# akashsengupta1997/STRAPS-3DHumanShapePose

Hardware: AMD Instinct MI355X
Metric: bodies/sec (higher is better)
Workload: dtype fp32 (encoder convolutions as exact bf16x3 operand splits (six bf16 products per term); in-step SMPL blend contraction and skinning as 3-product fp16 splits (fp16x3_lbs: 22-bit operands); fp32 accumulate throughout)

## Files before the change

include/straps_hip.h:

```cpp
#ifndef STRAPS_HIP_H
#define STRAPS_HIP_H

#include <stddef.h>
#include <stdint.h>

#ifdef __cplusplus
extern "C" {
#endif

#define STRAPS_ABI_VERSION 12

#define STRAPS_OK 0
#define STRAPS_EINVAL 1
#define STRAPS_EHIP 2
#define STRAPS_EUNSUPPORTED 3

int straps_abi_version(void);
int straps_selftest_mfma_peak(const float* seed512, float* out, int blocks, int iters, void* stream);
int straps_selftest_mfma_bf16(float* out, unsigned long long* clk2, int blocks, int iters, void* stream);
int straps_selftest_mfma_bf16_dense(float* out, unsigned long long* clk2, int blocks, int iters, int data, void* stream);
const char* straps_last_error(void);
int straps_device_count(void);
int straps_wall_clock_khz(void);
int straps_set_clock_accumulator(unsigned long long* acc2);


int straps_pack_conv_weight(const float* w_oihw, float* w_krsc, int cout, int cin, int kh, int kw,
                            void* stream);
int straps_pack_conv_weight_dgrad(const float* w_oihw, float* w_crsk, int cout, int cin, int kh,
                                  int kw, void* stream);
typedef struct {
    const float* src;
    float* dst_krsc;
    float* dst_crsk;
    int32_t o, c, r, s;
    long long first;
} straps_pack_desc_t;
int straps_pack_conv_weights_batched(const straps_pack_desc_t* descs, int n, long long total,
                                     void* stream);
int straps_pack_conv_weights_batched_x3(const straps_pack_desc_t* descs, int n, long long total,
                                        unsigned short* krsc_planes, unsigned short* crsk_planes,
                                        long long plane_stride, void* stream);

size_t straps_stem_weight_floats(int cin);
int straps_pack_stem_weight(const float* w_oihw, float* w_frag, int cin, void* stream);

int straps_bn_fold(const float* gamma, const float* beta, const float* mean, const float* var,
                   float eps, float* scale, float* shift, int c, void* stream);
int straps_bn_fold_stats(const float* gamma, const float* beta, const float* mean, const float* var,
                         float eps, float* scale, float* shift, float* save_mean, float* save_invstd,
                         int c, void* stream);

int straps_conv_trace_buffer(long long* trace);

int straps_stem_stat_blocks(int batch, int h, int w);
size_t straps_stem_nzmask_words(int batch, int cin, int h, int w);
int straps_stem_nzmask(const float* x_nchw, uint32_t* mask, int batch, int cin, int h, int w,
                       void* stream);
int straps_stem_fwd(const float* x_nchw, const float* w_frag, const float* scale,
                    const float* shift, int relu, float* y_nhwc, float* stats_partial,
                    const uint32_t* nzmask, int batch, int cin, int h, int w, void* stream);

int straps_conv_stat_blocks(int batch, int ho, int wo, int cout, int kdim , int tile_cfg);
int straps_conv_fwd(const float* x_nhwc, const float* w_krsc, const float* scale,
                    const float* shift, const float* residual, int relu, float* y_nhwc,
                    float* stats_partial, int batch, int h, int w, int cin, int cout, int kh,
                    int kw, int stride, int pad, int tile_cfg, void* stream);

int straps_maxpool_fwd(const float* x_nhwc, float* y_nhwc, int batch, int h, int w, int c,
                       void* stream);
int straps_gap_fwd(const float* x_nhwc, float* y, int batch, int hw, int c, void* stream);

int straps_bn_stats_finalize(const float* stats_partial, int nblocks, int c, long long count,
                             const float* gamma, const float* beta, float eps, float momentum,
                             float* running_mean, float* running_var, float* scale, float* shift,
                             float* save_mean, float* save_invstd, void* stream);
int straps_bn_apply(const float* x, const float* scale, const float* shift, const float* residual,
                    int relu, float* y, long long rows, int c, void* stream);

int straps_linear_fwd(const float* x, int ldx, const float* w, int ldw, const float* bias,
                      const float* addend, float* out, int ldo, int m, int n, int kdim, int relu,
                      void* stream);
int straps_broadcast_rows(const float* row, int cols, float* dst, int ld_dst, int m, void* stream);
int straps_ief_pack(const float* fc1_w, const float* fc3_w, float* w1f, float* w1e, float* w3, int f, int p,
                    int h1, int h2, int ld_e, void* stream);
#define STRAPS_GEMM_MULTI_MAX 8
typedef struct {
    const float* a; long long sam, sak;
    const float* b; long long sbk, sbn;
    float* c; int32_t ldc, accumulate;
    const float* addend; int32_t ldadd, reserved0;
    const float* mask; int32_t ldmask, reserved1;
    float* c2; int32_t ldc2, accumulate2;
    int32_t m, n, k, reserved2;
} straps_gemm_desc_t;
int straps_gemm_multi(const straps_gemm_desc_t* descs_host, int n, void* stream);

int straps_rot6d_fwd(const float* x6, long long ld, int per_row, float* rotmats, long long rows,
                     void* stream);
int straps_rodrigues_fwd(const float* aa, float* rotmats, long long n, void* stream);
int straps_rodrigues_bwd(const float* aa, const float* drotmats, float* daa, long long n, void* stream);
int straps_orthographic_project(const float* points, const float* cam, int ld_cam, float* out,
                                long long batch, int n, void* stream);
int straps_orthographic_project_bwd(const float* points, const float* cam, int ld_cam, const float* dout,
                                    float* dpoints, float* dcam, long long batch, int n, void* stream);
int straps_perspective_project(const float* points, const float* rotation, const float* translation,
                               const float* cam_k, int k_per_body, float* out, long long batch, int n,
                               void* stream);

#define STRAPS_SMPL_V 6890
#define STRAPS_SMPL_VPAD 6912
#define STRAPS_SMPL_TILES 216
#define STRAPS_SMPL_KP 224
#define STRAPS_SMPL_NJ 24
#define STRAPS_SMPL_NEXTRA 45
#define STRAPS_SMPL_NPICK 21
#define STRAPS_SMPL_NJOINTS_OUT 90

typedef struct {
    const float* blend_frag;
    const float* j_template;
    const float* j_shapedirs;
    const int32_t* parents;
    const int32_t* depth;
    int32_t max_depth;
    int32_t skin_k;
    const float* skin_w;
    const int32_t* skin_j;
    const int32_t* vj_ptr;
    int32_t n_tiles;
    int32_t reserved0;
    const int32_t* pick_ids;
    const float* blend_frag_t;
    const int32_t* children;
    const int32_t* jrt_ptr;
    const int32_t* jrt_code;
    const float* jrt_w;
    const int32_t* dj_ptr;
    const int32_t* dj_code;
    const float* dj_w;
    const void* blend_frag_h;
    float blend_h_unscale;
    int32_t reserved1;
    const void* skin_frag_p;
} straps_smpl_model_t;

#define STRAPS_SMPL_KERNEL_WIDE 0x100
#define STRAPS_SMPL_KERNEL_NARROW 0x200
#define STRAPS_SMPL_KERNEL_WIDE_BUILTIN 0x400
#define STRAPS_SMPL_EXACT_F32 0
#define STRAPS_SMPL_SPLIT_F16 1
#define STRAPS_SMPL_SPLIT_F16_LBS 2
#define STRAPS_SMPL_SPLIT_F16_LBS_PD16 3
#define STRAPS_SMPL_SPLIT_F16_LBS_P16 4

size_t straps_smpl_workspace_bytes(const straps_smpl_model_t* model, long long batch);
int straps_smpl_fwd(const straps_smpl_model_t* model, const float* betas, const float* rotmats,
                    float* verts, float* joints, void* workspace, long long batch, int chunks, int mode,
                    void* stream);

size_t straps_smpl_bwd_workspace_bytes(long long batch, int chunks);
int straps_smpl_bwd(const straps_smpl_model_t* model, const float* betas, const float* rotmats,
                    const float* dverts, const float* djoints, float* dbetas, float* drotmats,
                    void* workspace, long long batch, int chunks, void* stream);
int straps_smpl_bwd_aa(const straps_smpl_model_t* model, const float* betas, const float* rotmats,
                       const float* full_pose_aa, const float* dverts, const float* djoints, float* dbetas,
                       float* dfull_pose_aa, float* drotmats, void* workspace, long long batch, int chunks,
                       void* stream);

int straps_conv_dgrad(const float* dy_nhwc, const float* w_crsk, const float* addend,
                      float* dx_nhwc, int batch, int h, int w, int cin, int cout, int kh, int kw,
                      int stride, int pad, int tile_cfg, void* stream);

int straps_split3_bf16(const float* x, unsigned short* planes, long long n, long long plane_stride,
                       void* stream);
int straps_split3_bf16_cm(const float* x, unsigned short* planes, long long rows, int c,
                          long long plane_stride, void* stream);
int straps_conv_x3_stat_blocks(int batch, int h, int w, int cin, int cout, int kh, int kw, int stride,
                               int pad, int tile_cfg);

int straps_conv_x3f_supported(int cin, int cout, int kh, int kw, int stride, int pad);
int straps_conv_fwd_x3f(const float* x, const float* a_scale, const float* a_shift, int a_relu, const unsigned short* w3,
                        long long w_plane_stride, const float* scale, const float* shift, const float* residual, int relu,
                        float* y, float* stats_partial, int batch, int h, int w, int cin, int cout, int kh, int kw, int stride,
                        int pad, int tile_cfg, void* stream);
int straps_conv_x3f_stat_blocks(int batch, int h, int w, int cin, int cout, int kh, int kw, int stride, int pad, int tile_cfg);
int straps_conv_dgrad_x3f(const float* dy, const unsigned short* w3_crsk, long long w_plane_stride, const float* addend,
                          const unsigned* addend_bits, float* dx, int batch, int h, int w, int cin, int cout, int kh, int kw,
                          int stride, int pad, int tile_cfg, const float* bn_raw, const unsigned* bn_out_bits,
                          const float* bn_mask_scale, const float* bn_mask_shift, const float* bn_mean, const float* bn_invstd,
                          double* bn_partials, void* stream);
int straps_conv_dgrad_x3f_bn_blocks(int batch, int h, int w, int cin, int cout, int kh, int kw, int stride, int pad, int tile_cfg);
size_t straps_conv_wgrad_x3f_workspace_bytes(int batch, int h, int w, int cin, int cout, int kh, int kw, int stride, int pad);
int straps_conv_wgrad_x3f(const float* x, const float* a_scale, const float* a_shift, int a_relu, const float* dy, float* dw_oihw,
                          void* workspace, int batch, int h, int w, int cin, int cout, int kh, int kw, int stride, int pad,
                          int accumulate, void* stream);
int straps_conv_fwd_x3(const unsigned short* x3, long long x_plane_stride,
                       const unsigned short* w3_krsc, long long w_plane_stride, const float* scale,
                       const float* shift, const float* residual, int relu, float* y_nhwc,
                       float* stats_partial, int batch, int h, int w, int cin, int cout, int kh,
                       int kw, int stride, int pad, int tile_cfg, void* stream);
int straps_conv_fwd_x3p(const unsigned short* x3, long long x_plane_stride,
                        const unsigned short* w3_krsc, long long w_plane_stride, const float* scale,
                        const float* shift, const float* residual, int relu, float* y_nhwc,
                        unsigned short* y_planes, long long y_plane_stride, int batch, int h, int w,
                        int cin, int cout, int kh, int kw, int stride, int pad, int tile_cfg, void* stream);
int straps_split_bf16_cm(const float* x, unsigned short* plane, long long rows, int c, void* stream);
int straps_pack_conv_weight_bf16(const float* w_oihw, unsigned short* w_plane, int cout, int cin, int kh, int kw, void* stream);
int straps_conv_bf16_tile_choice(int batch, int h, int w, int cin, int cout, int kh, int kw, int stride, int pad);
int straps_conv_fwd_bf16(const unsigned short* x1, const unsigned short* w1_krsc, const float* scale, const float* shift,
                         const float* residual, int relu, float* y_nhwc, unsigned short* y_plane, int batch, int h, int w,
                         int cin, int cout, int kh, int kw, int stride, int pad, int tile_cfg, void* stream);
int straps_conv_dgrad_x3(const unsigned short* dy3, long long dy_plane_stride,
                         const unsigned short* w3_crsk, long long w_plane_stride,
                         const float* addend, float* dx_nhwc, int batch, int h, int w, int cin,
                         int cout, int kh, int kw, int stride, int pad, int tile_cfg, void* stream);
int straps_bn_apply_x3(const float* raw, const float* scale, const float* shift, const float* residual,
                       int relu, float* y, unsigned short* y_planes, long long plane_stride,
                       long long rows, int c, void* stream);
int straps_bn_relu_maxpool_fwd_x3(const float* raw, const float* scale, const float* shift,
                                  float* y_pool, uint8_t* idx, unsigned short* y_planes,
                                  long long plane_stride, int batch, int h, int w, int c, void* stream);
int straps_bn_bwd_x3(const float* dy, const float* yact, const float* raw, const float* save_mean,
                     const float* save_invstd, const float* gamma, const float* mask_scale,
                     const float* mask_shift, float* dgamma, float* dbeta, float* draw, float* dz_out,
                     unsigned short* draw_planes, long long plane_stride, void* workspace,
                     long long rows, int c, int accumulate, void* stream);
int straps_conv_dgrad_x3_bn_blocks(int batch, int h, int w, int cin, int cout, int kh, int kw, int stride,
                                   int pad, int tile_cfg);
int straps_conv_dgrad_x3_bn(const unsigned short* dy3, long long dy_plane_stride,
                            const unsigned short* w3_crsk, long long w_plane_stride, const float* addend,
                            float* dx_nhwc, int batch, int h, int w, int cin, int cout, int kh, int kw,
                            int stride, int pad, int tile_cfg, const float* bn_raw, const float* bn_out,
                            const float* bn_mask_scale, const float* bn_mask_shift, const float* bn_mean,
                            const float* bn_invstd, double* bn_partials, void* stream);
int straps_bn_bwd_finish_x3(const float* dy, const float* yact, const float* raw, const float* save_mean,
                            const float* save_invstd, const float* gamma, const float* mask_scale,
                            const float* mask_shift, float* dgamma, float* dbeta, float* draw, float* dz_out,
                            unsigned short* draw_planes, long long plane_stride, const double* partials,
                            int nblk, void* workspace, long long rows, int c, int accumulate, void* stream);
int straps_bn_apply_bits_x3(const float* raw, const float* scale, const float* shift, const float* residual, float* y,
                            unsigned short* y_planes, long long plane_stride, unsigned* relu_bits, long long rows,
                            int c, void* stream);
int straps_bn_bwd_bits_x3(const float* dy, const unsigned* relu_bits, const float* raw, const float* save_mean,
                          const float* save_invstd, const float* gamma, float* dgamma, float* dbeta, float* draw,
                          unsigned short* draw_planes, long long plane_stride, void* workspace, long long rows, int c,
                          int accumulate, void* stream);
int straps_bn_bwd_finish_bits_x3(const float* dy, const unsigned* relu_bits, const float* raw, const float* save_mean,
                                 const float* save_invstd, const float* gamma, float* dgamma, float* dbeta, float* draw,
                                 unsigned short* draw_planes, long long plane_stride, const double* partials, int nblk,
                                 void* workspace, long long rows, int c, int accumulate, void* stream);
int straps_conv_dgrad_x3_bits(const unsigned short* dy3, long long dy_plane_stride, const unsigned short* w3_crsk,
                              long long w_plane_stride, const float* addend, float* dx_nhwc, int batch, int h, int w,
                              int cin, int cout, int kh, int kw, int stride, int pad, int tile_cfg,
                              const unsigned* addend_bits, void* stream);
int straps_conv_dgrad_x3_bn_bits(const unsigned short* dy3, long long dy_plane_stride,
                                 const unsigned short* w3_crsk, long long w_plane_stride, const float* addend,
                                 float* dx_nhwc, int batch, int h, int w, int cin, int cout, int kh, int kw,
                                 int stride, int pad, int tile_cfg, const float* bn_raw, const float* bn_out,
                                 const float* bn_mask_scale, const float* bn_mask_shift, const float* bn_mean,
                                 const float* bn_invstd, double* bn_partials, const unsigned* addend_bits,
                                 const unsigned* bn_out_bits, void* stream);
int straps_conv_wgrad_x3_on_planes(int batch, int h, int w, int cin, int cout, int kh, int kw,
                                   int stride, int pad);
int straps_conv_wgrad_x3(const float* x_nhwc, const float* dy_nhwc, const unsigned short* x3,
                         long long x_plane_stride, const unsigned short* dy3, long long dy_plane_stride,
                         float* dw_oihw, void* workspace, int batch, int h, int w, int cin, int cout,
                         int kh, int kw, int stride, int pad, int accumulate, void* stream);


size_t straps_conv_wgrad_workspace_bytes(int batch, int h, int w, int cin, int cout, int kh,
                                         int kw, int stride, int pad);
int straps_conv_wgrad(const float* x_nhwc, const float* dy_nhwc, float* dw_oihw, void* workspace,
                      int batch, int h, int w, int cin, int cout, int kh, int kw, int stride,
                      int pad, int accumulate, void* stream);
size_t straps_stem_wgrad_workspace_bytes(int batch, int cin, int h, int w);
int straps_stem_wgrad(const float* x_nchw, const float* dy_nhwc, float* dw_oihw, void* workspace,
                      const uint32_t* nzmask , int batch, int cin,
                      int h, int w, int accumulate, void* stream);
#define STRAPS_STEM_DGRAD_MAX_CIN 64
size_t straps_stem_dgrad_weight_floats(int cin);
int straps_pack_stem_dgrad_weight(const float* w_oihw, float* w_pk, int cin, void* stream);
int straps_stem_dgrad(const float* dy_nhwc, const float* w_pk, float* dx_nchw, int batch, int cin, int h, int w,
                      int accumulate, void* stream);
int straps_bn_bwd_blocks(long long rows, int c);
size_t straps_bn_bwd_workspace_bytes(long long rows, int c);
int straps_bn_bwd(const float* dy, const float* yact, const float* raw, const float* save_mean,
                  const float* save_invstd, const float* gamma, const float* mask_scale,
                  const float* mask_shift, float* dgamma, float* dbeta, float* draw, float* dz_out,
                  void* workspace, long long rows, int c, int accumulate, void* stream);
int straps_bn_relu_maxpool_fwd(const float* raw_nhwc, const float* scale, const float* shift,
                               float* y_pool_nhwc, uint8_t* idx, int batch, int h, int w, int c,
                               void* stream);
int straps_bn_bwd_pooled(const float* dy_pool_nhwc, const uint8_t* idx, const float* raw,
                         const float* save_mean, const float* save_invstd, const float* gamma,
                         const float* mask_scale, const float* mask_shift, float* dgamma, float* dbeta,
                         float* draw, void* workspace, int batch, int h, int w, int c, int accumulate,
                         void* stream);
size_t straps_stem_tiles(int batch, int in_h, int in_w);
int straps_stem_tile_activity(const uint32_t* nzmask, uint8_t* tile_active, int batch, int cin, int in_h,
                              int in_w, void* stream);
int straps_bn_bwd_pooled_sparse(const float* dy_pool_nhwc, const uint8_t* idx, const float* raw,
                                const float* save_mean, const float* save_invstd, const float* gamma,
                                const float* mask_scale, const float* mask_shift, float* dgamma,
                                float* dbeta, float* draw, void* workspace, int batch, int h, int w, int c,
                                int accumulate, const uint8_t* tile_active, void* stream);
int straps_maxpool_fwd_idx(const float* x_nhwc, float* y_nhwc, uint8_t* idx, int batch, int h,
                           int w, int c, void* stream);
int straps_maxpool_bwd(const float* dy_nhwc, const uint8_t* idx, float* dx_nhwc, int batch, int h,
                       int w, int c, void* stream);
int straps_gap_bwd(const float* dfeat, float* dx_nhwc, int batch, int hw, int c, void* stream);
int straps_masked_copy(const float* x, int ldx, const float* mask, int ldmask, float* y, int ldy,
                       int m, int n, int accumulate, void* stream);
int straps_rot6d_bwd(const float* x6, long long ld, int per_row, const float* drot, float* dx6,
                     long long ldd, long long rows, void* stream);

int straps_build_proxy_input(const float* seg, const float* joints2d, float* out_nchw, int batch,
                             int nj, int wh, void* stream);
int straps_build_proxy_input_std(const float* seg, const float* joints2d, float* out_nchw, int batch,
                                 int nj, int wh, int std, void* stream);
int straps_build_proxy_input_nz(const float* seg, const float* joints2d, float* out_nchw, uint32_t* nzmask,
                                int batch, int nj, int wh, int std, void* stream);
size_t straps_loss_workspace_bytes(long long batch);
int straps_loss_fwd_bwd(const float* pred_verts, const float* pred_joints, const float* est,
                        int ld_est, const float* pred_rot, const float* tgt_verts,
                        const float* tgt_joints2d, const float* tgt_joints3d,
                        const float* tgt_shape, const float* tgt_rot, const float* log_vars,
                        float* loss_out, float* dverts, float* djoints, float* dest, float* drot,
                        float* dlogvar, void* workspace, long long batch, int img_wh, void* stream);
int straps_loss_fwd_bwd_gm(const float* pred_verts, const float* pred_joints, const float* est, int ld_est,
                           const float* pred_rot, const float* tgt_verts, const float* tgt_joints2d,
                           const float* tgt_joints3d, const float* tgt_shape, const float* tgt_rot,
                           const float* log_vars, float* loss_out, float* dverts, float* djoints, float* dest,
                           float* drot, float* dlogvar, void* workspace, long long batch, int img_wh,
                           const float* j2d_count_global, float count_scale, void* stream);
int straps_count_visible(const float* tgt_joints2d, float* out_count, long long batch, int nj, int img_wh,
                         void* stream);
int straps_mse_fwd(const float* pred, const float* tgt, const uint8_t* row_mask, long long rows,
                   int cols, float tgt_scale, float tgt_shift, float* out3, void* workspace,
                   void* stream);
int straps_mse_bwd(const float* pred, const float* tgt, const uint8_t* row_mask, long long rows,
                   int cols, float tgt_scale, float tgt_shift, const float* coef, float* grad,
                   void* stream);
int straps_augment_seg(const float* seg, const float* uniforms, const float* remove_prob,
                       float occlude_prob, int box_dim, float* out, int batch, int wh, void* stream);
int straps_philox_fill(unsigned long long seed, const long long* step_dev, long long step_host,
                       unsigned substream, float* out, long long n, int kind, void* stream);
int straps_counter_add(long long* counters, int n, long long delta, void* stream);
int straps_gather_f32(const float* src, const int* index, float* dst, int n, void* stream);
int straps_memset_zero(void* ptr, size_t bytes, void* stream);
int straps_augment_smpl(const float* pose_rows, long long n_rows, const float* u_index,
                        const float* orig_shape, const float* mean_shape, const float* shape_draws,
                        int shape_mode, const float* std_vector, double range_lo, double range_hi,
                        float* out_shape, float* out_rotmats, float* out_pose, long long batch,
                        void* stream);
int straps_augment_cam_t(const float* mean_cam_t, const float* normals_xy, const float* uniform_z,
                         double xy_std, double z_lo, double z_hi, float* out_cam_t, long long batch,
                         void* stream);
int straps_deviate_joints2d(const float* joints2d, const float* uniforms, double lo, double hi,
                            double hip_lo, double hip_hi, float* out, long long batch, void* stream);
int straps_deviate_verts2d(const float* verts, const float* uniforms, double lo, double hi, float* out,
                           long long nverts_total, void* stream);
int straps_project_targets(const float* joints, const float* cam_t, float fx, float fy, float cx,
                           float cy, float* joints2d, float* joints3d, long long batch, void* stream);
size_t straps_rasterize_workspace_bytes(long long batch, int nverts, int wh);
int straps_rasterize_parts(const float* verts, const int32_t* faces, const uint8_t* face_parts,
                           const float* cam_K, const float* cam_R, const float* cam_t, float* parts,
                           float* depth, void* workspace, long long batch, int nverts, int nfaces, int wh,
                           int cam_per_body, float near, float far, const float* vert_noise_u, double noise_lo,
                           double noise_hi, void* stream);
int straps_crop_resize(const float* seg, const float* joints2d, const float* uniforms,
                       double orig_scale_factor, double delta_scale_lo, double delta_scale_hi,
                       double delta_centre_lo, double delta_centre_hi, float* out_seg,
                       float* out_joints2d, int* boxes, int batch, int wh, int out_wh, int nj,
                       void* stream);
int straps_point_metrics(const float* pred, const float* target, float* out3, long long batch,
                         int npoints, void* stream);
int straps_adam_step(float* params, const float* grads, float* exp_avg, float* exp_avg_sq,
                     long long n, int step, float lr, float beta1, float beta2, float eps,
                     float grad_scale, const long long* step_dev, void* stream);

typedef struct {
    int layers;
    int in_channels;
    int ief_iters;
    int precision;
} straps_regressor_desc_t;
size_t straps_regressor_param_floats(const straps_regressor_desc_t* desc);
size_t straps_regressor_prepared_bytes(const straps_regressor_desc_t* desc);
int straps_regressor_prepare(const straps_regressor_desc_t* desc, const float* params, void* prepared, void* stream);
size_t straps_regressor_workspace_bytes(const straps_regressor_desc_t* desc, int batch, int h, int w);
int straps_regressor_fwd_infer(const straps_regressor_desc_t* desc, const void* prepared, const float* x, int batch, int h, int w,
                               float* est, int ld_est, float* rotmats, void* workspace, size_t workspace_bytes, void* stream);

size_t straps_regressor_train_param_floats(const straps_regressor_desc_t* desc);
size_t straps_regressor_bn_state_floats(const straps_regressor_desc_t* desc);
size_t straps_regressor_train_workspace_bytes(const straps_regressor_desc_t* desc, int batch, int h, int w);
int straps_regressor_fwd_train(const straps_regressor_desc_t* desc, const float* params, float* bn_state, const float* init_est,
                               const float* x, int batch, int h, int w, float* est, int ld_est,
                               void* workspace, size_t workspace_bytes, void* stream);
int straps_regressor_bwd(const straps_regressor_desc_t* desc, const float* params, const float* x, int batch, int h, int w,
                         const float* dest, int ld_dest, float* grads, float* dx,
                         void* workspace, size_t workspace_bytes, void* stream);
int straps_regressor_export_infer_params(const straps_regressor_desc_t* desc, const float* params, const float* bn_state,
                                         const float* init_est, float* infer_params, void* stream);

#define STRAPS_COMM_ID_BYTES 128
int straps_comm_unique_id(void* id128);
int straps_comm_init_rank(const void* id128, int nranks, int rank, void** comm);
int straps_comm_destroy(void* comm);
int straps_comm_size(void* comm);
const char* straps_comm_library(void);
int straps_allreduce_grads(float* flat_g, long long n, void* comm, void* stream);

#ifdef __cplusplus
}
#endif
#endif
```

straps-3dhumanshapepose_amd/csrc/common.h:

```cpp
#pragma once
#include <hip/hip_runtime.h>
#include <stdint.h>
#include <stdio.h>

#include "../../include/straps_hip.h"

typedef float f32x4 __attribute__((ext_vector_type(4)));
typedef float f32x16 __attribute__((ext_vector_type(16)));
typedef float f32x2 __attribute__((ext_vector_type(2)));

void straps_set_error(const char* fmt, ...);
unsigned long long* straps_clk_acc_current();

#define STRAPS_REQUIRE(cond, ...)             \
    do {                                      \
        if (!(cond)) {                        \
            straps_set_error(__VA_ARGS__);    \
            return STRAPS_EINVAL;             \
        }                                     \
    } while (0)

#define STRAPS_CHECK_LAUNCH(name)                                                        \
    do {                                                                                 \
        hipError_t e__ = hipGetLastError();                                              \
        if (e__ != hipSuccess) {                                                         \
            straps_set_error("%s: launch failed: %s", name, hipGetErrorString(e__));     \
            return STRAPS_EHIP;                                                          \
        }                                                                                \
    } while (0)

#if defined(__HIP_DEVICE_COMPILE__) && !(defined(STRAPS_TOOLS) && defined(STRAPS_ALLOW_PACKED_FP32))
#define STRAPS_NO_PACKED_FP32 __attribute__((target("no-packed-fp32-ops")))
#else
#define STRAPS_NO_PACKED_FP32
#endif

inline hipError_t straps_raise_dynamic_lds(const void* fn, size_t bytes, unsigned long long& done) {
    int dev = 0;
    hipError_t e = hipGetDevice(&dev);
    if (e != hipSuccess) return e;
    const unsigned long long bit = 1ull << (dev & 63);
    if (done & bit) return hipSuccess;
    e = hipFuncSetAttribute(fn, hipFuncAttributeMaxDynamicSharedMemorySize, (int)bytes);
    if (e == hipSuccess) done |= bit;
    return e;
}
#define STRAPS_RAISE_LDS(fn, bytes, name)                                                                  \
    do {                                                                                                   \
        static unsigned long long done__ = 0;                                                              \
        hipError_t e__ = straps_raise_dynamic_lds((const void*)(fn), (size_t)(bytes), done__);             \
        if (e__ != hipSuccess) {                                                                           \
            straps_set_error("%s: cannot raise dynamic LDS to %zu: %s", name, (size_t)(bytes), hipGetErrorString(e__)); \
            return STRAPS_EHIP;                                                                            \
        }                                                                                                  \
    } while (0)

__device__ __forceinline__ f32x16 mfma32(float a, float b, f32x16 c) {
    return __builtin_amdgcn_mfma_f32_32x32x2f32(a, b, c, 0, 0, 0);
}
__device__ __forceinline__ int mfma_row(int r, int lane) { return (r & 3) + 8 * (r >> 2) + 4 * (lane >> 5); }

__device__ __forceinline__ int xcd_remap(int bid, int nblk) {
    const int q = nblk >> 3, r = nblk & 7, xcd = bid & 7;
    return (xcd < r ? xcd * (q + 1) : r * (q + 1) + (xcd - r) * q) + (bid >> 3);
}

template <typename T>
__device__ __forceinline__ bool bn_partials_sum4(const T* __restrict__ part, int nblocks, int C, double& s1, double& s2, int& c) {
    __shared__ double red[256][2];
    const int cl = threadIdx.x & 3, pl = threadIdx.x >> 2;
    c = blockIdx.x * 4 + cl;
    double a1 = 0.0, a2 = 0.0;
    if (c < C) {
        int k = pl;
        for (; k + 15 * 64 < nblocks; k += 16 * 64) {
            T v0[16], v1[16];
#pragma unroll
            for (int q = 0; q < 16; ++q) {
                const T* v = part + ((long long)(k + q * 64) * C + c) * 2;
                v0[q] = v[0];
                v1[q] = v[1];
            }
#pragma unroll
            for (int q = 0; q < 16; ++q) { a1 += (double)v0[q]; a2 += (double)v1[q]; }
        }
#pragma unroll 8
        for (; k < nblocks; k += 64) {
            const T* v = part + ((long long)k * C + c) * 2;
            a1 += (double)v[0];
            a2 += (double)v[1];
        }
    }
    red[threadIdx.x][0] = a1;
    red[threadIdx.x][1] = a2;
    __syncthreads();
    if (pl != 0 || c >= C) return false;
    s1 = 0.0; s2 = 0.0;
    for (int q = 0; q < 64; ++q) { s1 += red[q * 4 + cl][0]; s2 += red[q * 4 + cl][1]; }
    return true;
}

typedef unsigned short u16;
typedef u16 u16x4 __attribute__((ext_vector_type(4)));
__device__ __forceinline__ u16 bf16_rn(float x) {
    unsigned u = __float_as_uint(x);
    u += 0x7FFFu + ((u >> 16) & 1u);
    return (u16)(u >> 16);
}
__device__ __forceinline__ void split3(float x, u16& b1, u16& b2, u16& b3) {
    b1 = bf16_rn(x);
    const float r1 = (__float_as_uint(x) & 0x7fffffffu) == 0x7f800000u ? 0.f : x - __uint_as_float((unsigned)b1 << 16);
    b2 = bf16_rn(r1);
    const float r2 = r1 - __uint_as_float((unsigned)b2 << 16);
    b3 = bf16_rn(r2);
}
__device__ __forceinline__ void store_planes4(u16* __restrict__ planes, long long ps, long long i, const f32x4& v) {
    u16x4 q1, q2, q3;
#pragma unroll
    for (int e = 0; e < 4; ++e) {
        u16 b1, b2, b3;
        split3(v[e], b1, b2, b3);
        q1[e] = b1; q2[e] = b2; q3[e] = b3;
    }
    *reinterpret_cast<u16x4*>(planes + i) = q1;
    *reinterpret_cast<u16x4*>(planes + ps + i) = q2;
    *reinterpret_cast<u16x4*>(planes + 2 * ps + i) = q3;
}

__device__ __forceinline__ long long cm_index(long long r, int c, long long rows) { return ((long long)(c >> 5) * rows + r) * 32 + (c & 31); }
__device__ __forceinline__ void store_planes4_cm(u16* __restrict__ planes, long long ps, long long r, int c, long long rows, const f32x4& v) {
    store_planes4(planes, ps, cm_index(r, c, rows), v);
}

#ifdef STRAPS_TOOLS
#include <stdlib.h>
#define STRAPS_TOOL_ENV_INT(name, dflt) (getenv(name) ? atoi(getenv(name)) : (dflt))
#else
#define STRAPS_TOOL_ENV_INT(name, dflt) (dflt)
#endif

static inline int cdiv(long long a, long long b) { return (int)((a + b - 1) / b); }

static inline unsigned straps_grid256(long long n) {
    const long long g = (n + 255) / 256;
    return (unsigned)(g > 256 * 16 ? 256 * 16 : (g < 1 ? 1 : g));
}
static inline unsigned straps_grid256_rows(long long n, int C4) {
    unsigned g = straps_grid256(n);
    if (C4 > 0 && (256 % C4) != 0) {
        long long a = C4, b = 256;
        while (b) { const long long t = a % b; a = b; b = t; }
        const long long m = C4 / a;
        if (m <= 256 * 16) { const long long up = ((g + m - 1) / m) * m; g = (unsigned)(up > 256 * 16 ? (256 * 16 / m) * m : up); }
    }
    return g;
}
static inline int straps_bn_tiled(long long rows, int C4) {
    static const int mode = STRAPS_TOOL_ENV_INT("STRAPS_BN_TILED", 1);
    if (!mode || (C4 & 15)) return 0;
    const int ncg = C4 >> 4;
    if (!(ncg == 1 || ncg == 2 || (ncg & 3) == 0) || (mode == 1 && ncg < 4)) return 0;
    const int wcg = ncg < 4 ? ncg : 4;
    return (rows % (16 / wcg)) == 0 ? wcg : 0;
}
static inline unsigned straps_bn_tiled_grid(long long rows, int C4, int wcg) {
    const long long ncb = (C4 >> 4) / wcg, tiles = rows / (16 / wcg) * ncb;
    long long g = tiles < 256 * 16 ? tiles : 256 * 16;
    g = g / ncb * ncb;
    return (unsigned)(g < ncb ? ncb : g);
}
```

straps-3dhumanshapepose_amd/csrc/smpl_bwd.hip:

```cpp
#include "common.h"
#include "rodrigues.h"

namespace {

constexpr int KP = STRAPS_SMPL_KP, KG = KP / 8, NT = STRAPS_SMPL_TILES, NV = STRAPS_SMPL_V, NROUNDS = NT / 4;
constexpr int BT = 32, AS = 292, SS = 193;
constexpr int NJS = STRAPS_SMPL_NPICK + STRAPS_SMPL_NEXTRA;

__global__ __launch_bounds__(256, 1) STRAPS_NO_PACKED_FP32 void smpl_verts_bwd_kernel(straps_smpl_model_t m, const float* __restrict__ F,
                                                                const float* __restrict__ Amat, const float* __restrict__ dverts,
                                                                const float* __restrict__ djoints, float* __restrict__ dFp,
                                                                float* __restrict__ dAp, long long B, int rounds_per_chunk) {
    extern __shared__ __attribute__((aligned(16))) float smem[];
    float* As_ = smem;
    float* stage = As_ + BT * AS;

    const int tid = threadIdx.x, lane = tid & 63, wave = tid >> 6;
    const int h = lane >> 5, bl = lane & 31;
    const int chunk = blockIdx.x;
    const long long b0 = (long long)blockIdx.y * BT;
    const int nb = (int)((B - b0) < BT ? (B - b0) : BT);

    for (int i = tid; i < BT * 72; i += 256) {
        const int b = i / 72, q = i % 72;
        f32x4 v = {0.f, 0.f, 0.f, 0.f};
        if (b < nb) v = *reinterpret_cast<const f32x4*>(Amat + (b0 + b) * 288 + q * 4);
        *reinterpret_cast<f32x4*>(As_ + b * AS + q * 4) = v;
    }
    __syncthreads();

    const int round0 = chunk * rounds_per_chunk;
    const int round1 = min(round0 + rounds_per_chunk, NROUNDS);
    const f32x4* __restrict__ blend = reinterpret_cast<const f32x4*>(m.blend_frag);
    const f32x4* __restrict__ blend_t = reinterpret_cast<const f32x4*>(m.blend_frag_t);
    float* mystage = stage + wave * BT * SS;
    const int KW = m.skin_k;
    const bool vbody = bl < nb;

    float dacc[3][12];
#pragma unroll
    for (int i = 0; i < 3; ++i)
#pragma unroll
        for (int e = 0; e < 12; ++e) dacc[i][e] = 0.f;
    f32x16 accF[7];
#pragma unroll
    for (int f = 0; f < 7; ++f)
#pragma unroll
        for (int q = 0; q < 16; ++q) accF[f][q] = 0.f;

    for (int rd = round0; rd < round1; ++rd) {
        const int tile = rd * 4 + wave;
        f32x16 ax, ay, az;
#pragma unroll
        for (int r = 0; r < 16; ++r) { ax[r] = 0.f; ay[r] = 0.f; az[r] = 0.f; }
        {
            const f32x4* px = blend + ((long long)(tile * 3 + 0) * KG) * 64 + lane;
            const f32x4* py = px + KG * 64;
            const f32x4* pz = py + KG * 64;
            const float* frow = F + (b0 + (vbody ? bl : 0)) * KP + 4 * h;
            f32x4 cx0 = px[0], cy0 = py[0], cz0 = pz[0];
            f32x4 fn = *reinterpret_cast<const f32x4*>(frow);
#pragma unroll 2
            for (int g = 0; g < KG; ++g) {
                f32x4 nx0 = cx0, ny0 = cy0, nz0 = cz0;
                const f32x4 f0 = vbody ? fn : f32x4{0.f, 0.f, 0.f, 0.f};
                if (g + 1 < KG) {
                    nx0 = px[(g + 1) * 64]; ny0 = py[(g + 1) * 64]; nz0 = pz[(g + 1) * 64];
                    fn = *reinterpret_cast<const f32x4*>(frow + 8 * (g + 1));
                }
#pragma unroll
                for (int e = 0; e < 4; ++e) {
                    ax = mfma32(cx0[e], f0[e], ax);
                    ay = mfma32(cy0[e], f0[e], ay);
                    az = mfma32(cz0[e], f0[e], az);
                }
                cx0 = nx0; cy0 = ny0; cz0 = nz0;
            }
        }
        {
            const int ncol = min(96, (NV - tile * 32) * 3);
            for (int i = lane; i < BT * 96; i += 64) {
                const int b = i / 96, c = i - b * 96;
                float v = 0.f;
                if (dverts && b < nb && c < ncol) v = dverts[(b0 + b) * (long long)(NV * 3) + tile * 96 + c];
                mystage[b * SS + (c / 3) * 6 + (c % 3)] = v;
            }
        }
        __syncthreads();
        if (djoints && h == 0 && vbody) {
            const float* dj = djoints + (b0 + bl) * (STRAPS_SMPL_NJOINTS_OUT * 3) + 72;
            const int e0 = m.jrt_ptr[tile], e1 = m.jrt_ptr[tile + 1];
            for (int e = e0; e < e1; ++e) {
                const int code = m.jrt_code[e];
                const float w = m.jrt_w[e];
                float* sv = mystage + bl * SS + (code >> 8) * 6;
                const float* g = dj + (code & 255) * 3;
                sv[0] = fmaf(w, g[0], sv[0]); sv[1] = fmaf(w, g[1], sv[1]); sv[2] = fmaf(w, g[2], sv[2]);
            }
        }
        __syncthreads();
        {
            const float* Ab = As_ + bl * AS;
#pragma unroll
            for (int r = 0; r < 16; ++r) {
                const int vrow = (r & 3) + 8 * (r >> 2) + 4 * h;
                const int v = tile * 32 + vrow;
                float* sv = mystage + bl * SS + vrow * 6;
                const float gx = sv[0], gy = sv[1], gz = sv[2];
                sv[3] = ax[r]; sv[4] = ay[r]; sv[5] = az[r];
                float t00 = 0.f, t01 = 0.f, t02 = 0.f, t10 = 0.f, t11 = 0.f, t12 = 0.f, t20 = 0.f, t21 = 0.f, t22 = 0.f;
                for (int k = 0; k < KW; ++k) {
                    const float w = m.skin_w[v * KW + k];
                    const int jo = m.skin_j[v * KW + k] * 12;
                    const f32x4 a0 = *reinterpret_cast<const f32x4*>(Ab + jo);
                    const f32x4 a1 = *reinterpret_cast<const f32x4*>(Ab + jo + 4);
                    const f32x4 a2 = *reinterpret_cast<const f32x4*>(Ab + jo + 8);
                    t00 += w * a0[0]; t01 += w * a0[1]; t02 += w * a0[2];
                    t10 += w * a1[0]; t11 += w * a1[1]; t12 += w * a1[2];
                    t20 += w * a2[0]; t21 += w * a2[1]; t22 += w * a2[2];
                }
                ax[r] = t00 * gx + t10 * gy + t20 * gz;
                ay[r] = t01 * gx + t11 * gy + t21 * gz;
                az[r] = t02 * gx + t12 * gy + t22 * gz;
            }
        }
        __syncthreads();
#pragma unroll
        for (int i = 0; i < 3; ++i) {
            const int j = wave + 4 * (2 * i + h);
            const int e0 = m.dj_ptr[rd * 24 + j], e1 = m.dj_ptr[rd * 24 + j + 1];
            for (int e = e0; e < e1; ++e) {
                const int code = m.dj_code[e];
                const float w = m.dj_w[e];
                const float* sv = stage + ((code >> 5) * BT + bl) * SS + (code & 31) * 6;
                const float wx = w * sv[0], wy = w * sv[1], wz = w * sv[2];
                const float x = sv[3], y = sv[4], z = sv[5];
                dacc[i][0] = fmaf(wx, x, dacc[i][0]); dacc[i][1] = fmaf(wx, y, dacc[i][1]); dacc[i][2] = fmaf(wx, z, dacc[i][2]); dacc[i][3] += wx;
                dacc[i][4] = fmaf(wy, x, dacc[i][4]); dacc[i][5] = fmaf(wy, y, dacc[i][5]); dacc[i][6] = fmaf(wy, z, dacc[i][6]); dacc[i][7] += wy;
                dacc[i][8] = fmaf(wz, x, dacc[i][8]); dacc[i][9] = fmaf(wz, y, dacc[i][9]); dacc[i][10] = fmaf(wz, z, dacc[i][10]); dacc[i][11] += wz;
            }
        }
        {
            const f32x4* pt = blend_t + ((long long)tile * 3 * 7 * 4) * 64 + lane;
#pragma unroll
            for (int c = 0; c < 3; ++c) {
#pragma unroll
                for (int f = 0; f < 7; ++f) {
#pragma unroll
                    for (int rq = 0; rq < 4; ++rq) {
                        const f32x4 a = pt[((c * 7 + f) * 4 + rq) * 64];
#pragma unroll
                        for (int e = 0; e < 4; ++e) {
                            const float g = c == 0 ? ax[rq * 4 + e] : (c == 1 ? ay[rq * 4 + e] : az[rq * 4 + e]);
                            accF[f] = mfma32(a[e], g, accF[f]);
                        }
                    }
                }
            }
        }
        __syncthreads();
    }
    {
        __syncthreads();
        float* red = smem;
        if (wave >= 2) {
#pragma unroll
            for (int f = 0; f < 7; ++f)
#pragma unroll
                for (int q = 0; q < 16; ++q) red[(wave - 2) * 7168 + (f * 16 + q) * 64 + lane] = accF[f][q];
        }
        __syncthreads();
        if (wave < 2) {
#pragma unroll
            for (int f = 0; f < 7; ++f)
#pragma unroll
                for (int q = 0; q < 16; ++q) accF[f][q] += red[wave * 7168 + (f * 16 + q) * 64 + lane];
        }
        __syncthreads();
        if (wave == 1) {
#pragma unroll
            for (int f = 0; f < 7; ++f)
#pragma unroll
                for (int q = 0; q < 16; ++q) red[(f * 16 + q) * 64 + lane] = accF[f][q];
        }
        __syncthreads();
        if (wave == 0) {
#pragma unroll
            for (int f = 0; f < 7; ++f)
#pragma unroll
                for (int q = 0; q < 16; ++q) accF[f][q] += red[(f * 16 + q) * 64 + lane];
        }
    }
    if (vbody && wave == 0) {
        float* o = dFp + ((long long)chunk * B + b0 + bl) * KP;
#pragma unroll
        for (int f = 0; f < 7; ++f)
#pragma unroll
            for (int q = 0; q < 16; ++q) o[f * 32 + mfma_row(q, lane)] = accF[f][q];
    }
    if (vbody) {
        float* o = dAp + ((long long)chunk * B + b0 + bl) * 288;
#pragma unroll
        for (int i = 0; i < 3; ++i) {
            const int j = wave + 4 * (2 * i + h);
#pragma unroll
            for (int e = 0; e < 12; ++e) o[j * 12 + e] = dacc[i][e];
        }
    }
}

__device__ __forceinline__ float lane_get(float value, int src) { return __shfl(value, src, 64); }
template <bool AA>
__global__ __launch_bounds__(256) STRAPS_NO_PACKED_FP32 void smpl_pose_bwd_kernel(straps_smpl_model_t m, const float* __restrict__ betas,
                                                            const float* __restrict__ rotmats, const float* __restrict__ dFp,
                                                            const float* __restrict__ dAp, const float* __restrict__ djoints,
                                                            float* __restrict__ dbetas, float* __restrict__ drot, long long B,
                                                            int chunks, const float* __restrict__ aa, float* __restrict__ daa) {
    const int lane = threadIdx.x & 63;
    const int j = lane & 31;
    const int base = lane & 32;
    const long long body = ((long long)blockIdx.x * 256 + threadIdx.x) >> 5;
    const bool vb = body < B;
    const bool vj = j < 24;
    const long long bb = vb ? body : 0;
    const int jj = vj ? j : 0;

    float beta[10];
#pragma unroll
    for (int l = 0; l < 10; ++l) beta[l] = betas[bb * 10 + l];
    float R[9];
#pragma unroll
    for (int e = 0; e < 9; ++e) R[e] = rotmats[(bb * 24 + jj) * 9 + e];
    float J[3];
#pragma unroll
    for (int c = 0; c < 3; ++c) {
        float s = m.j_template[jj * 3 + c];
#pragma unroll
        for (int l = 0; l < 10; ++l) s = fmaf(m.j_shapedirs[(jj * 3 + c) * 10 + l], beta[l], s);
        J[c] = s;
    }
    const int par = m.parents[jj];
    const int dep = vj ? m.depth[jj] : -1;
    const int src = base + (par < 0 ? 0 : par);
    float rel[3];
#pragma unroll
    for (int c = 0; c < 3; ++c) {
        const float jp = lane_get(J[c], src);
        rel[c] = (jj > 0) ? J[c] - jp : J[c];
    }
    float G[12], PR[9];
#pragma unroll
    for (int r = 0; r < 3; ++r) {
        G[r * 4 + 0] = R[r * 3 + 0]; G[r * 4 + 1] = R[r * 3 + 1]; G[r * 4 + 2] = R[r * 3 + 2]; G[r * 4 + 3] = rel[r];
    }
#pragma unroll
    for (int e = 0; e < 9; ++e) PR[e] = (e == 0 || e == 4 || e == 8) ? 1.f : 0.f;
    for (int d = 1; d <= m.max_depth; ++d) {
        float P[12];
#pragma unroll
        for (int e = 0; e < 12; ++e) P[e] = lane_get(G[e], src);
        if (dep == d) {
#pragma unroll
            for (int r = 0; r < 3; ++r) {
                const float p0 = P[r * 4 + 0], p1 = P[r * 4 + 1], p2 = P[r * 4 + 2];
                PR[r * 3 + 0] = p0; PR[r * 3 + 1] = p1; PR[r * 3 + 2] = p2;
                G[r * 4 + 0] = p0 * R[0] + p1 * R[3] + p2 * R[6];
                G[r * 4 + 1] = p0 * R[1] + p1 * R[4] + p2 * R[7];
                G[r * 4 + 2] = p0 * R[2] + p1 * R[5] + p2 * R[8];
                G[r * 4 + 3] = p0 * rel[0] + p1 * rel[1] + p2 * rel[2] + P[r * 4 + 3];
            }
        }
    }
    float gA[12];
#pragma unroll
    for (int e = 0; e < 12; ++e) gA[e] = 0.f;
    if (vb && vj)
        for (int c = 0; c < chunks; ++c) {
            const float* p = dAp + (((long long)c * B + body) * 24 + j) * 12;
#pragma unroll
            for (int e = 0; e < 12; ++e) gA[e] += p[e];
        }
    float gGR[9], gGt[3], gJ[3];
#pragma unroll
    for (int r = 0; r < 3; ++r) {
        const float gat = gA[r * 4 + 3];
        gGR[r * 3 + 0] = gA[r * 4 + 0] - gat * J[0];
        gGR[r * 3 + 1] = gA[r * 4 + 1] - gat * J[1];
        gGR[r * 3 + 2] = gA[r * 4 + 2] - gat * J[2];
        gGt[r] = gat + ((vb && vj && djoints) ? djoints[(body * STRAPS_SMPL_NJOINTS_OUT + j) * 3 + r] : 0.f);
    }
#pragma unroll
    for (int c = 0; c < 3; ++c) gJ[c] = -(G[0 * 4 + c] * gA[3] + G[1 * 4 + c] * gA[7] + G[2 * 4 + c] * gA[11]);

    int child[3];
#pragma unroll
    for (int c = 0; c < 3; ++c) child[c] = m.children[jj * 3 + c];
    float gR[9];
#pragma unroll
    for (int e = 0; e < 9; ++e) gR[e] = 0.f;
    for (int d = m.max_depth; d >= 1; --d) {
        float M[15];
        const bool mine = (dep == d);
        float grel[3];
#pragma unroll
        for (int c = 0; c < 3; ++c) grel[c] = PR[0 * 3 + c] * gGt[0] + PR[1 * 3 + c] * gGt[1] + PR[2 * 3 + c] * gGt[2];
#pragma unroll
        for (int r = 0; r < 3; ++r)
#pragma unroll
            for (int c = 0; c < 3; ++c)
                M[r * 3 + c] = mine ? (gGR[r * 3 + 0] * R[c * 3 + 0] + gGR[r * 3 + 1] * R[c * 3 + 1] + gGR[r * 3 + 2] * R[c * 3 + 2] + gGt[r] * rel[c]) : 0.f;
#pragma unroll
        for (int c = 0; c < 3; ++c) { M[9 + c] = mine ? gGt[c] : 0.f; M[12 + c] = mine ? -grel[c] : 0.f; }
        if (mine) {
#pragma unroll
            for (int r = 0; r < 3; ++r)
#pragma unroll
                for (int c = 0; c < 3; ++c)
                    gR[r * 3 + c] = PR[0 * 3 + r] * gGR[0 * 3 + c] + PR[1 * 3 + r] * gGR[1 * 3 + c] + PR[2 * 3 + r] * gGR[2 * 3 + c];
#pragma unroll
            for (int c = 0; c < 3; ++c) gJ[c] += grel[c];
        }
#pragma unroll
        for (int cc = 0; cc < 3; ++cc) {
            const int ch = child[cc];
            const int cs = base + (ch < 0 ? 0 : ch);
            float in[15];
#pragma unroll
            for (int e = 0; e < 15; ++e) in[e] = lane_get(M[e], cs);
            if (vj && ch >= 0) {
#pragma unroll
                for (int e = 0; e < 9; ++e) gGR[e] += in[e];
#pragma unroll
                for (int c = 0; c < 3; ++c) { gGt[c] += in[9 + c]; gJ[c] += in[12 + c]; }
            }
        }
    }
    if (j == 0) {
#pragma unroll
        for (int e = 0; e < 9; ++e) gR[e] = gGR[e];
#pragma unroll
        for (int c = 0; c < 3; ++c) gJ[c] += gGt[c];
    }
    float gbeta_direct = 0.f;
    if (vb && vj) {
        for (int c = 0; c < chunks; ++c) {
            const float* p = dFp + ((long long)c * B + body) * KP;
            if (j >= 1) {
#pragma unroll
                for (int e = 0; e < 9; ++e) gR[e] += p[11 + (j - 1) * 9 + e];
            }
            if (j < 10) gbeta_direct += p[1 + j];
        }
        if (!AA || drot) {
#pragma unroll
            for (int e = 0; e < 9; ++e) drot[(body * 24 + j) * 9 + e] = gR[e];
        }
        if constexpr (AA) {
            float ox, oy, oz;
            const float* r = aa + (body * 24 + j) * 3;
            straps_rodrigues_bwd_one(r[0], r[1], r[2], gR, ox, oy, oz);
            float* o = daa + (body * 24 + j) * 3;
            o[0] = ox; o[1] = oy; o[2] = oz;
        }
    }
#pragma unroll
    for (int l = 0; l < 10; ++l) {
        float s = vj ? (m.j_shapedirs[(jj * 3 + 0) * 10 + l] * gJ[0] + m.j_shapedirs[(jj * 3 + 1) * 10 + l] * gJ[1] +
                        m.j_shapedirs[(jj * 3 + 2) * 10 + l] * gJ[2]) : 0.f;
#pragma unroll
        for (int o = 16; o > 0; o >>= 1) s += __shfl_xor(s, o, 64);
        const float direct = lane_get(gbeta_direct, base + l);
        if (vb && j == l) dbetas[body * 10 + l] = s + direct;
    }
}

inline int resolve_rpc(long long batch, int chunks) {
    if (chunks <= 0) chunks = (batch >= 1024) ? 8 : 54;
    if (chunks > NROUNDS) chunks = NROUNDS;
    return (NROUNDS + chunks - 1) / chunks;
}

}

int straps_smpl_launch_pose(const straps_smpl_model_t* model, const float* betas, const float* rotmats, float* F, float* Amat,
                            float* joints, long long batch, hipStream_t st);

extern "C" size_t straps_smpl_bwd_workspace_bytes(long long batch, int chunks) {
    const int rpc = resolve_rpc(batch, chunks);
    const int nch = (NROUNDS + rpc - 1) / rpc;
    return (size_t)batch * (size_t)(KP + 288 + nch * (KP + 288)) * sizeof(float);
}

namespace {
template <bool AA>
int smpl_bwd_launch(const straps_smpl_model_t* model, const float* betas, const float* rotmats, const float* aa, const float* dverts,
                    const float* djoints, float* dbetas, float* drotmats, float* daa, void* workspace, long long batch, int chunks,
                    void* stream) {
    hipStream_t st = (hipStream_t)stream;
    const int rpc = resolve_rpc(batch, chunks);
    const int nch = (NROUNDS + rpc - 1) / rpc;
    float* F = (float*)workspace;
    float* Amat = F + batch * KP;
    float* dFp = Amat + batch * 288;
    float* dAp = dFp + (long long)nch * batch * KP;
    int rc = straps_smpl_launch_pose(model, betas, rotmats, F, Amat, nullptr, batch, st);
    if (rc != STRAPS_OK) return rc;
    const size_t lds = (size_t)(BT * AS + 4 * BT * SS) * sizeof(float);
    STRAPS_RAISE_LDS((smpl_verts_bwd_kernel), lds, "smpl_verts_bwd_kernel");
    const long long btiles = (batch + BT - 1) / BT;
    if (btiles > 65535) { straps_set_error("straps_smpl_bwd: batch %lld exceeds one launch; split it", batch); return STRAPS_EUNSUPPORTED; }
    hipLaunchKernelGGL(smpl_verts_bwd_kernel, dim3(nch, (unsigned)btiles), dim3(256), lds, st, *model, F, Amat, dverts, djoints, dFp, dAp, batch, rpc);
    STRAPS_CHECK_LAUNCH("smpl_verts_bwd_kernel");
    hipLaunchKernelGGL(smpl_pose_bwd_kernel<AA>, dim3((unsigned)((batch * 32 + 255) / 256)), dim3(256), 0, st, *model, betas, rotmats, dFp, dAp,
                       djoints, dbetas, drotmats, batch, nch, aa, daa);
    STRAPS_CHECK_LAUNCH("smpl_pose_bwd_kernel");
    return STRAPS_OK;
}
}

extern "C" int straps_smpl_bwd(const straps_smpl_model_t* model, const float* betas, const float* rotmats, const float* dverts,
                               const float* djoints, float* dbetas, float* drotmats, void* workspace, long long batch, int chunks,
                               void* stream) {
    STRAPS_REQUIRE(model && betas && rotmats && dbetas && drotmats && workspace, "straps_smpl_bwd: null pointer");
    STRAPS_REQUIRE(model->blend_frag_t && model->children && model->jrt_ptr && model->dj_ptr && model->dj_code && model->dj_w,
                   "straps_smpl_bwd: model lacks the backward tables");
    STRAPS_REQUIRE(batch > 0, "straps_smpl_bwd: batch must be positive");
    return smpl_bwd_launch<false>(model, betas, rotmats, nullptr, dverts, djoints, dbetas, drotmats, nullptr, workspace, batch, chunks, stream);
}

extern "C" int straps_smpl_bwd_aa(const straps_smpl_model_t* model, const float* betas, const float* rotmats, const float* full_pose_aa,
                                  const float* dverts, const float* djoints, float* dbetas, float* dfull_pose_aa, float* drotmats,
                                  void* workspace, long long batch, int chunks, void* stream) {
    STRAPS_REQUIRE(model && betas && rotmats && full_pose_aa && dbetas && dfull_pose_aa && workspace, "straps_smpl_bwd_aa: null pointer");
    STRAPS_REQUIRE(model->blend_frag_t && model->children && model->jrt_ptr && model->dj_ptr && model->dj_code && model->dj_w,
                   "straps_smpl_bwd_aa: model lacks the backward tables");
    STRAPS_REQUIRE(batch > 0, "straps_smpl_bwd_aa: batch must be positive");
    return smpl_bwd_launch<true>(model, betas, rotmats, full_pose_aa, dverts, djoints, dbetas, drotmats, dfull_pose_aa, workspace, batch, chunks,
                                 stream);
}
```

straps-3dhumanshapepose_amd/csrc/train.hip:

```cpp
#include <math.h>

#include "common.h"

namespace {

__constant__ int c_coco[17] = {24, 26, 25, 28, 27, 16, 17, 18, 19, 20, 21, 1, 2, 4, 5, 7, 8};
__constant__ int c_h36m14[14] = {73 + 6, 73 + 5, 73 + 4, 73 + 1, 73 + 2, 73 + 3, 73 + 16, 73 + 15, 73 + 14, 73 + 11, 73 + 12, 73 + 13, 73 + 8, 73 + 10};

__device__ __forceinline__ float heat_value(int x, int y, int jx, int jy, int WH, int size, float step, float two_var) {
    if (!(jx > -size && jy > -size && jx < WH - 1 + size && jy < WH - 1 + size)) return 0.f;
    const int hx0 = max(0, jx - size), hx1 = min(WH - 1, jx + size);
    const int hy0 = max(0, jy - size), hy1 = min(WH - 1, jy + size);
    if (!(x >= hx0 && x < hx1 && y >= hy0 && y < hy1)) return 0.f;
    const int gx = x - hx0 + max(0, size - jx), gy = y - hy0 + max(0, size - jy);
    const float fs = (float)size;
    const float lx = gx < size ? -fs + step * gx : fs - step * (2 * size - 1 - gx);
    const float ly = gy < size ? -fs + step * gy : fs - step * (2 * size - 1 - gy);
    const float d = sqrtf(lx * lx + ly * ly);
    return expf(-(d * d / two_var));
}

__global__ __launch_bounds__(256) void build_proxy_kernel(const float* __restrict__ seg, const float* __restrict__ j2d,
                                                          float* __restrict__ out, int B, int NJ, int WH, int size, float step, float two_var) {
    const int plane = blockIdx.y;
    const int b = plane / (NJ + 1), ch = plane - b * (NJ + 1);
    const int npix = WH * WH;
    float* o = out + (long long)plane * npix;
    int jx = 0, jy = 0;
    if (ch > 0) {
        jx = (int)j2d[((long long)b * NJ + ch - 1) * 2 + 0];
        jy = (int)j2d[((long long)b * NJ + ch - 1) * 2 + 1];
    }
    const float* s = seg + (long long)b * npix;
    const bool vec = (WH & 3) == 0;
    for (int p = (blockIdx.x * 256 + threadIdx.x) * 4; p < npix; p += gridDim.x * 1024) {
        float v[4];
#pragma unroll
        for (int e = 0; e < 4; ++e) {
            const int q = p + e;
            v[e] = 0.f;
            if (q < npix) {
                if (ch == 0) v[e] = s[q] != 0.f ? 1.f : 0.f;
                else {
                    const int y = q / WH, x = q - y * WH;
                    v[e] = heat_value(x, y, jx, jy, WH, size, step, two_var);
                }
            }
        }
        if (vec) *reinterpret_cast<f32x4*>(o + p) = f32x4{v[0], v[1], v[2], v[3]};
        else
            for (int e = 0; e < 4; ++e)
                if (p + e < npix) o[p + e] = v[e];
    }
}

__global__ __launch_bounds__(256) void build_proxy_nz_kernel(const float* __restrict__ seg, const float* __restrict__ j2d, float* __restrict__ out,
                                                             unsigned* __restrict__ mask, long long nwords, int NJ, int WH, int size, float step,
                                                             float two_var) {
    const int lane = threadIdx.x & 63;
    const long long word = (long long)blockIdx.x * 4 + (threadIdx.x >> 6);
    if (word >= nwords) return;
    const int HC = (WH + 3) >> 2, WW = (WH + 255) >> 8;
    const int ww = (int)(word % WW);
    const long long t = word / WW;
    const int hc = (int)(t % HC);
    const int plane = (int)(t / HC);
    const int b = plane / (NJ + 1), ch = plane - b * (NJ + 1);
    const int x0 = ww * 256 + (lane & 31) * 8 + (lane >> 5) * 4, y0 = hc * 4;
    const int npix = WH * WH;
    float* o = out + (long long)plane * npix;
    bool nz = false;
    if (x0 < WH) {
        f32x4 v[4];
#pragma unroll
        for (int r = 0; r < 4; ++r) v[r] = f32x4{0.f, 0.f, 0.f, 0.f};
        if (ch == 0) {
            const float* s = seg + (long long)b * npix;
#pragma unroll
            for (int r = 0; r < 4; ++r)
                if (y0 + r < WH) {
                    const f32x4 a = *reinterpret_cast<const f32x4*>(s + (y0 + r) * WH + x0);
#pragma unroll
                    for (int e = 0; e < 4; ++e) v[r][e] = a[e] != 0.f ? 1.f : 0.f;
                }
        } else {
            const int jx = (int)j2d[((long long)b * NJ + ch - 1) * 2 + 0];
            const int jy = (int)j2d[((long long)b * NJ + ch - 1) * 2 + 1];
            if (x0 + 3 >= jx - size && x0 < jx + size && y0 + 3 >= jy - size && y0 < jy + size) {
#pragma unroll
                for (int r = 0; r < 4; ++r)
                    if (y0 + r < WH)
#pragma unroll
                        for (int e = 0; e < 4; ++e) v[r][e] = heat_value(x0 + e, y0 + r, jx, jy, WH, size, step, two_var);
            }
        }
#pragma unroll
        for (int r = 0; r < 4; ++r)
            if (y0 + r < WH) {
                *reinterpret_cast<f32x4*>(o + (y0 + r) * WH + x0) = v[r];
                nz = nz || v[r][0] != 0.f || v[r][1] != 0.f || v[r][2] != 0.f || v[r][3] != 0.f;
            }
    }
    const unsigned long long m = __ballot(nz);
    if (lane == 0) mask[word] = (unsigned)(m | (m >> 32));
}

constexpr int NVB = 1024;

__global__ __launch_bounds__(256) void loss_verts_partial_kernel(const float* __restrict__ p, const float* __restrict__ t, long long n,
                                                                 float* __restrict__ part) {
    __shared__ float red[4];
    float s = 0.f;
    for (long long i = (long long)blockIdx.x * 256 + threadIdx.x; i < n; i += (long long)gridDim.x * 256) {
        const float d = p[i] - t[i];
        s = fmaf(d, d, s);
    }
#pragma unroll
    for (int o = 32; o > 0; o >>= 1) s += __shfl_xor(s, o, 64);
    if ((threadIdx.x & 63) == 0) red[threadIdx.x >> 6] = s;
    __syncthreads();
    if (threadIdx.x == 0) part[blockIdx.x] = (red[0] + red[1]) + (red[2] + red[3]);
}

__device__ __forceinline__ bool joint_visible(float x, float y, float wh) { return !(x > wh || y > wh || x < 0.f || y < 0.f); }

__global__ __launch_bounds__(256) void loss_heads_kernel(const float* __restrict__ joints, const float* __restrict__ est, int ld_est,
                                                         const float* __restrict__ prot, const float* __restrict__ tj2d,
                                                         const float* __restrict__ tj3d, const float* __restrict__ tshape,
                                                         const float* __restrict__ trot, float* __restrict__ body_sums, long long B,
                                                         float wh) {
    const long long b = (long long)blockIdx.x * 256 + threadIdx.x;
    if (b >= B) return;
    const float* J = joints + b * 270;
    const float* e = est + b * ld_est;
    const float s = e[0], tx = e[1], ty = e[2];
    float sq2 = 0.f, nvis = 0.f, sq3 = 0.f, sqs = 0.f, sqr = 0.f;
    for (int k = 0; k < 17; ++k) {
        const float lx = tj2d[(b * 17 + k) * 2 + 0], ly = tj2d[(b * 17 + k) * 2 + 1];
        if (joint_visible(lx, ly, wh)) {
            const float* pj = J + c_coco[k] * 3;
            const float u = s * (pj[0] + tx), v = s * (pj[1] + ty);
            const float du = u - ((2.0f * lx) / wh - 1.0f), dv = v - ((2.0f * ly) / wh - 1.0f);
            sq2 += du * du + dv * dv;
            nvis += 1.f;
        }
    }
    for (int k = 0; k < 14; ++k) {
        const float* pj = J + c_h36m14[k] * 3;
        const float* tj = tj3d + (b * 14 + k) * 3;
        for (int c = 0; c < 3; ++c) { const float d = pj[c] - tj[c]; sq3 += d * d; }
    }
    for (int l = 0; l < 10; ++l) { const float d = e[147 + l] - tshape[b * 10 + l]; sqs += d * d; }
    for (int q = 0; q < 216; ++q) { const float d = prot[b * 216 + q] - trot[b * 216 + q]; sqr += d * d; }
    float* o = body_sums + b * 8;
    o[0] = sq2; o[1] = nvis; o[2] = sq3; o[3] = sqs; o[4] = sqr;
}

__global__ __launch_bounds__(256) void loss_finalize_kernel(const float* __restrict__ vpart, const float* __restrict__ body_sums,
                                                            const float* __restrict__ log_vars, float* __restrict__ loss_out,
                                                            float* __restrict__ dlogvar, float* __restrict__ coef, long long B,
                                                            const float* __restrict__ j2d_count, float count_scale) {
    __shared__ double red[256][6];
    double a[6] = {0, 0, 0, 0, 0, 0};
    for (int i = threadIdx.x; i < NVB; i += 256) a[0] += (double)vpart[i];
    for (long long b = threadIdx.x; b < B; b += 256) {
        const float* o = body_sums + b * 8;
        a[1] += o[0]; a[2] += o[1]; a[3] += o[2]; a[4] += o[3]; a[5] += o[4];
    }
    for (int q = 0; q < 6; ++q) red[threadIdx.x][q] = a[q];
    __syncthreads();
    if (threadIdx.x == 0) {
        double t[6] = {0, 0, 0, 0, 0, 0};
        for (int i = 0; i < 256; ++i)
            for (int q = 0; q < 6; ++q) t[q] += red[i][q];
        const double nvis = t[2];
        const double n2 = j2d_count ? (double)j2d_count[0] * (double)count_scale : nvis;
        const double cnt[5] = {(double)B * 20670.0, n2 * 2.0, (double)B * 42.0, (double)B * 10.0, (double)B * 216.0};
        const double sq[5] = {t[0], t[1], t[3], t[4], t[5]};
        double total = 0.0;
        for (int k = 0; k < 5; ++k) {
            const double mse = sq[k] / cnt[k];
            const double s = (double)log_vars[k];
            const double w = exp(-s);
            loss_out[1 + k] = (float)(mse * w);
            loss_out[6 + k] = (float)mse;
            total += mse * w + s;
            dlogvar[k] = (float)(-mse * w + 1.0);
            coef[k] = (float)(2.0 * w / cnt[k]);
        }
        loss_out[0] = (float)total;
        loss_out[11] = (float)nvis;
    }
}

__global__ __launch_bounds__(256) void loss_grad_verts_kernel(const float* __restrict__ p, const float* __restrict__ t,
                                                              const float* __restrict__ coef, float* __restrict__ g, long long n) {
    const float c = coef[0];
    for (long long i = (long long)blockIdx.x * 256 + threadIdx.x; i < n; i += (long long)gridDim.x * 256) g[i] = c * (p[i] - t[i]);
}

__global__ __launch_bounds__(64) STRAPS_NO_PACKED_FP32 void loss_grad_heads_kernel(const float* __restrict__ joints, const float* __restrict__ est, int ld_est,
                                                             const float* __restrict__ prot, const float* __restrict__ tj2d,
                                                             const float* __restrict__ tj3d, const float* __restrict__ tshape,
                                                             const float* __restrict__ trot, const float* __restrict__ coef,
                                                             float* __restrict__ djoints, float* __restrict__ dest,
                                                             float* __restrict__ drot, long long B, float wh) {
    const long long b = blockIdx.x;
    const int lane = threadIdx.x;
    const float* J = joints + b * 270;
    const float* e = est + b * ld_est;
    float* dJ = djoints + b * 270;
    float* dE = dest + b * ld_est;
    const float c2 = coef[1], c3 = coef[2], cs = coef[3], cr = coef[4];
    for (int i = lane; i < 270; i += 64) dJ[i] = 0.f;
    for (int i = lane; i < ld_est; i += 64) dE[i] = (i >= 147 && i < 157) ? cs * (e[i] - tshape[b * 10 + i - 147]) : 0.f;
    for (int i = lane; i < 216; i += 64) drot[b * 216 + i] = cr * (prot[b * 216 + i] - trot[b * 216 + i]);
    __builtin_amdgcn_s_waitcnt(0);
    __syncthreads();
    const float s = e[0], tx = e[1], ty = e[2];
    float gs = 0.f, gtx = 0.f, gty = 0.f;
    if (lane < 17) {
        const float lx = tj2d[(b * 17 + lane) * 2 + 0], ly = tj2d[(b * 17 + lane) * 2 + 1];
        if (joint_visible(lx, ly, wh)) {
            const float* pj = J + c_coco[lane] * 3;
            const float u = s * (pj[0] + tx), v = s * (pj[1] + ty);
            const float du = c2 * (u - ((2.0f * lx) / wh - 1.0f)), dv = c2 * (v - ((2.0f * ly) / wh - 1.0f));
            dJ[c_coco[lane] * 3 + 0] = du * s;
            dJ[c_coco[lane] * 3 + 1] = dv * s;
            gs = du * (pj[0] + tx) + dv * (pj[1] + ty);
            gtx = du * s;
            gty = dv * s;
        }
    } else if (lane >= 32 && lane < 46) {
        const int k = lane - 32;
        const float* pj = J + c_h36m14[k] * 3;
        const float* tj = tj3d + (b * 14 + k) * 3;
        for (int c = 0; c < 3; ++c) dJ[c_h36m14[k] * 3 + c] = c3 * (pj[c] - tj[c]);
    }
#pragma unroll
    for (int o = 16; o > 0; o >>= 1) {
        gs += __shfl_xor(gs, o, 64);
        gtx += __shfl_xor(gtx, o, 64);
        gty += __shfl_xor(gty, o, 64);
    }
    if (lane == 0) { dE[0] = gs; dE[1] = gtx; dE[2] = gty; }
}

__global__ __launch_bounds__(256) void adam_kernel(float* __restrict__ p, const float* __restrict__ g, float* __restrict__ m,
                                                   float* __restrict__ v, long long n, float b1, float b2, float eps, float step_size,
                                                   float inv_sqrt_bc2, float gscale, float lr, const long long* __restrict__ step_dev) {
    if (step_dev) {
        const double t = (double)step_dev[0];
        step_size = (float)((double)lr / (1.0 - pow((double)b1, t)));
        inv_sqrt_bc2 = (float)(1.0 / sqrt(1.0 - pow((double)b2, t)));
    }
    for (long long i = (long long)blockIdx.x * 256 + threadIdx.x; i < n; i += (long long)gridDim.x * 256) {
        const float gi = g[i] * gscale;
        const float mi = b1 * m[i] + (1.f - b1) * gi;
        const float vi = b2 * v[i] + (1.f - b2) * gi * gi;
        m[i] = mi;
        v[i] = vi;
        p[i] -= step_size * mi / (sqrtf(vi) * inv_sqrt_bc2 + eps);
    }
}

inline unsigned capped_grid(long long n, int cap = 4096) {
    long long g = (n + 255) / 256;
    return (unsigned)(g > cap ? cap : (g < 1 ? 1 : g));
}

}

extern "C" int straps_build_proxy_input_std(const float* seg, const float* joints2d, float* out_nchw, int batch, int nj, int wh, int std,
                                            void* stream) {
    STRAPS_REQUIRE(seg && joints2d && out_nchw && batch > 0 && nj > 0 && wh > 16, "straps_build_proxy_input: bad arguments");
    STRAPS_REQUIRE(std >= 1 && 4 * std <= wh, "straps_build_proxy_input: std must be an integer in [1, wh / 4] (got %d)", std);
    STRAPS_REQUIRE((long long)batch * (nj + 1) <= 65535 && wh <= 16384, "straps_build_proxy_input: batch*(nj+1) must be <= 65535 per call");
    const int gx = (wh * wh / 4 + 255) / 256;
    const int size = 2 * std;
    const float step = (float)(2 * size) / (float)(2 * size - 1);
    const float two_var = (float)(2.0 * std * std);
    hipLaunchKernelGGL(build_proxy_kernel, dim3(gx < 64 ? gx : 64, batch * (nj + 1)), dim3(256), 0, (hipStream_t)stream, seg, joints2d, out_nchw, batch, nj, wh,
                       size, step, two_var);
    STRAPS_CHECK_LAUNCH("build_proxy_kernel");
    return STRAPS_OK;
}

extern "C" int straps_build_proxy_input_nz(const float* seg, const float* joints2d, float* out_nchw, uint32_t* nzmask, int batch, int nj, int wh,
                                           int std, void* stream) {
    STRAPS_REQUIRE(seg && joints2d && out_nchw && nzmask && batch > 0 && nj > 0 && wh > 16, "straps_build_proxy_input_nz: bad arguments");
    STRAPS_REQUIRE(std >= 1 && 4 * std <= wh, "straps_build_proxy_input_nz: std must be an integer in [1, wh / 4] (got %d)", std);
    STRAPS_REQUIRE((wh & 7) == 0 && wh <= 16384, "straps_build_proxy_input_nz: wh must be a multiple of 8 (got %d)", wh);
    const long long nwords = (long long)batch * (nj + 1) * ((wh + 3) / 4) * ((wh + 255) / 256);
    STRAPS_REQUIRE((nwords + 3) / 4 < (1LL << 31) && (long long)batch * (nj + 1) * wh * wh < (1LL << 40), "straps_build_proxy_input_nz: input too large for one launch");
    const int size = 2 * std;
    const float step = (float)(2 * size) / (float)(2 * size - 1);
    const float two_var = (float)(2.0 * std * std);
    hipLaunchKernelGGL(build_proxy_nz_kernel, dim3((unsigned)((nwords + 3) / 4)), dim3(256), 0, (hipStream_t)stream, seg, joints2d, out_nchw, nzmask, nwords, nj,
                       wh, size, step, two_var);
    STRAPS_CHECK_LAUNCH("build_proxy_nz_kernel");
    return STRAPS_OK;
}

extern "C" int straps_build_proxy_input(const float* seg, const float* joints2d, float* out_nchw, int batch, int nj, int wh,
                                        void* stream) {
    return straps_build_proxy_input_std(seg, joints2d, out_nchw, batch, nj, wh, 4, stream);
}

extern "C" size_t straps_loss_workspace_bytes(long long batch) { return (size_t)(NVB + batch * 8 + 16) * sizeof(float); }

__global__ __launch_bounds__(256) void count_visible_kernel(const float* __restrict__ tj2d, float* __restrict__ out, long long n, float wh) {
    __shared__ int red[4];
    int c = 0;
    for (long long i = threadIdx.x; i < n; i += 256) c += joint_visible(tj2d[i * 2], tj2d[i * 2 + 1], wh) ? 1 : 0;
#pragma unroll
    for (int o = 32; o > 0; o >>= 1) c += __shfl_xor(c, o, 64);
    if ((threadIdx.x & 63) == 0) red[threadIdx.x >> 6] = c;
    __syncthreads();
    if (threadIdx.x == 0) out[0] = (float)(red[0] + red[1] + red[2] + red[3]);
}

extern "C" int straps_count_visible(const float* tgt_joints2d, float* out_count, long long batch, int nj, int img_wh, void* stream) {
    STRAPS_REQUIRE(tgt_joints2d && out_count && batch > 0 && nj > 0, "straps_count_visible: bad arguments");
    hipLaunchKernelGGL(count_visible_kernel, dim3(1), dim3(256), 0, (hipStream_t)stream, tgt_joints2d, out_count, batch * nj, (float)img_wh);
    STRAPS_CHECK_LAUNCH("count_visible_kernel");
    return STRAPS_OK;
}

extern "C" int straps_loss_fwd_bwd(const float* pred_verts, const float* pred_joints, const float* est, int ld_est, const float* pred_rot,
                                   const float* tgt_verts, const float* tgt_joints2d, const float* tgt_joints3d, const float* tgt_shape,
                                   const float* tgt_rot, const float* log_vars, float* loss_out, float* dverts, float* djoints,
                                   float* dest, float* drot, float* dlogvar, void* workspace, long long batch, int img_wh, void* stream) {
    return straps_loss_fwd_bwd_gm(pred_verts, pred_joints, est, ld_est, pred_rot, tgt_verts, tgt_joints2d, tgt_joints3d, tgt_shape, tgt_rot, log_vars, loss_out,
                                  dverts, djoints, dest, drot, dlogvar, workspace, batch, img_wh, nullptr, 1.0f, stream);
}

extern "C" int straps_loss_fwd_bwd_gm(const float* pred_verts, const float* pred_joints, const float* est, int ld_est, const float* pred_rot,
                                      const float* tgt_verts, const float* tgt_joints2d, const float* tgt_joints3d, const float* tgt_shape,
                                      const float* tgt_rot, const float* log_vars, float* loss_out, float* dverts, float* djoints,
                                      float* dest, float* drot, float* dlogvar, void* workspace, long long batch, int img_wh,
                                      const float* j2d_count_global, float count_scale, void* stream) {
    STRAPS_REQUIRE(pred_verts && pred_joints && est && pred_rot && tgt_verts && tgt_joints2d && tgt_joints3d && tgt_shape && tgt_rot &&
                       log_vars && loss_out && workspace,
                   "straps_loss_fwd_bwd: null pointer");
    STRAPS_REQUIRE(batch > 0 && ld_est >= 157, "straps_loss_fwd_bwd: bad shape batch=%lld ld_est=%d", batch, ld_est);
    const bool want_grad = dverts || djoints || dest || drot || dlogvar;
    STRAPS_REQUIRE(!want_grad || (dverts && djoints && dest && drot && dlogvar), "straps_loss_fwd_bwd: give all gradient outputs or none");
    hipStream_t st = (hipStream_t)stream;
    float* vpart = (float*)workspace;
    float* body = vpart + NVB;
    float* coef = body + batch * 8;
    float* dlv = dlogvar ? dlogvar : coef + 8;
    const long long nv = batch * 20670LL;
    hipLaunchKernelGGL(loss_verts_partial_kernel, dim3(NVB), dim3(256), 0, st, pred_verts, tgt_verts, nv, vpart);
    STRAPS_CHECK_LAUNCH("loss_verts_partial_kernel");
    hipLaunchKernelGGL(loss_heads_kernel, dim3((unsigned)((batch + 255) / 256)), dim3(256), 0, st, pred_joints, est, ld_est, pred_rot,
                       tgt_joints2d, tgt_joints3d, tgt_shape, tgt_rot, body, batch, (float)img_wh);
    STRAPS_CHECK_LAUNCH("loss_heads_kernel");
    hipLaunchKernelGGL(loss_finalize_kernel, dim3(1), dim3(256), 0, st, vpart, body, log_vars, loss_out, dlv, coef, batch, j2d_count_global, count_scale);
    STRAPS_CHECK_LAUNCH("loss_finalize_kernel");
    if (want_grad) {
        hipLaunchKernelGGL(loss_grad_verts_kernel, dim3(capped_grid(nv)), dim3(256), 0, st, pred_verts, tgt_verts, coef, dverts, nv);
        STRAPS_CHECK_LAUNCH("loss_grad_verts_kernel");
        hipLaunchKernelGGL(loss_grad_heads_kernel, dim3((unsigned)batch), dim3(64), 0, st, pred_joints, est, ld_est, pred_rot, tgt_joints2d,
                           tgt_joints3d, tgt_shape, tgt_rot, coef, djoints, dest, drot, batch, (float)img_wh);
        STRAPS_CHECK_LAUNCH("loss_grad_heads_kernel");
    }
    return STRAPS_OK;
}

extern "C" int straps_adam_step(float* params, const float* grads, float* exp_avg, float* exp_avg_sq, long long n, int step, float lr,
                                float beta1, float beta2, float eps, float grad_scale, const long long* step_dev, void* stream) {
    STRAPS_REQUIRE(params && grads && exp_avg && exp_avg_sq && n > 0 && (step >= 1 || step_dev), "straps_adam_step: bad arguments");
    if (step < 1) step = 1;
    const double bc1 = 1.0 - pow((double)beta1, (double)step);
    const double bc2 = 1.0 - pow((double)beta2, (double)step);
    hipLaunchKernelGGL(adam_kernel, dim3(capped_grid(n)), dim3(256), 0, (hipStream_t)stream, params, grads, exp_avg, exp_avg_sq, n, beta1, beta2,
                       eps, (float)((double)lr / bc1), (float)(1.0 / sqrt(bc2)), grad_scale, lr, step_dev);
    STRAPS_CHECK_LAUNCH("adam_kernel");
    return STRAPS_OK;
}

namespace {

__global__ __launch_bounds__(256) void mse_sum_kernel(const float* __restrict__ p, const float* __restrict__ t, const uint8_t* __restrict__ mask,
                                                      long long rows, int cols, float ts, float tb, float* __restrict__ part) {
    __shared__ float red[4][2];
    float s = 0.f, c = 0.f;
    const long long n = rows * cols;
    for (long long i = (long long)blockIdx.x * 256 + threadIdx.x; i < n; i += (long long)gridDim.x * 256) {
        if (mask && !mask[i / cols]) continue;
        const float d = p[i] - (t[i] * ts + tb);
        s = fmaf(d, d, s);
        c += 1.f;
    }
#pragma unroll
    for (int o = 32; o > 0; o >>= 1) { s += __shfl_xor(s, o, 64); c += __shfl_xor(c, o, 64); }
    if ((threadIdx.x & 63) == 0) { red[threadIdx.x >> 6][0] = s; red[threadIdx.x >> 6][1] = c; }
    __syncthreads();
    if (threadIdx.x == 0) {
        part[blockIdx.x * 2 + 0] = (red[0][0] + red[1][0]) + (red[2][0] + red[3][0]);
        part[blockIdx.x * 2 + 1] = (red[0][1] + red[1][1]) + (red[2][1] + red[3][1]);
    }
}

__global__ __launch_bounds__(64) void mse_finalize_kernel(const float* __restrict__ part, int nblk, float* __restrict__ out) {
    double s = 0.0, c = 0.0;
    for (int i = threadIdx.x; i < nblk; i += 64) { s += part[i * 2]; c += part[i * 2 + 1]; }
#pragma unroll
    for (int o = 32; o > 0; o >>= 1) { s += __shfl_xor(s, o, 64); c += __shfl_xor(c, o, 64); }
    if (threadIdx.x == 0) { out[0] = (float)s; out[1] = (float)c; out[2] = (float)(s / c); }
}

__global__ __launch_bounds__(256) void mse_grad_kernel(const float* __restrict__ p, const float* __restrict__ t, const uint8_t* __restrict__ mask,
                                                       long long rows, int cols, float ts, float tb, const float* __restrict__ coef,
                                                       float* __restrict__ g) {
    const long long n = rows * cols;
    const float c = coef[0];
    for (long long i = (long long)blockIdx.x * 256 + threadIdx.x; i < n; i += (long long)gridDim.x * 256)
        g[i] = (mask && !mask[i / cols]) ? 0.f : c * (p[i] - (t[i] * ts + tb));
}

}

extern "C" int straps_mse_fwd(const float* pred, const float* tgt, const uint8_t* row_mask, long long rows, int cols, float tgt_scale,
                              float tgt_shift, float* out3, void* workspace, void* stream) {
    STRAPS_REQUIRE(pred && tgt && out3 && workspace && rows > 0 && cols > 0, "straps_mse_fwd: bad arguments");
    float* part = (float*)workspace;
    hipLaunchKernelGGL(mse_sum_kernel, dim3(256), dim3(256), 0, (hipStream_t)stream, pred, tgt, row_mask, rows, cols, tgt_scale, tgt_shift, part);
    STRAPS_CHECK_LAUNCH("mse_sum_kernel");
    hipLaunchKernelGGL(mse_finalize_kernel, dim3(1), dim3(64), 0, (hipStream_t)stream, part, 256, out3);
    STRAPS_CHECK_LAUNCH("mse_finalize_kernel");
    return STRAPS_OK;
}

extern "C" int straps_mse_bwd(const float* pred, const float* tgt, const uint8_t* row_mask, long long rows, int cols, float tgt_scale,
                              float tgt_shift, const float* coef, float* grad, void* stream) {
    STRAPS_REQUIRE(pred && tgt && coef && grad && rows > 0 && cols > 0, "straps_mse_bwd: bad arguments");
    hipLaunchKernelGGL(mse_grad_kernel, dim3(capped_grid(rows * cols)), dim3(256), 0, (hipStream_t)stream, pred, tgt, row_mask, rows, cols,
                       tgt_scale, tgt_shift, coef, grad);
    STRAPS_CHECK_LAUNCH("mse_grad_kernel");
    return STRAPS_OK;
}

namespace {
__global__ __launch_bounds__(256) void project_targets_kernel(const float* __restrict__ joints, const float* __restrict__ cam_t, float fx,
                                                              float fy, float cx, float cy, float* __restrict__ j2d,
                                                              float* __restrict__ j3d, long long B) {
    const long long i = (long long)blockIdx.x * 256 + threadIdx.x;
    if (i >= B * 31) return;
    const long long b = i / 31;
    const int k = (int)(i - b * 31);
    const float* J = joints + b * 270;
    if (k < 17) {
        const float* p = J + c_coco[k] * 3;
        const float x = p[0] + cam_t[b * 3 + 0], y = p[1] + cam_t[b * 3 + 1], z = p[2] + cam_t[b * 3 + 2];
        j2d[(b * 17 + k) * 2 + 0] = fx * (x / z) + cx;
        j2d[(b * 17 + k) * 2 + 1] = fy * (y / z) + cy;
    } else {
        const float* p = J + c_h36m14[k - 17] * 3;
        float* o = j3d + (b * 14 + (k - 17)) * 3;
        o[0] = p[0]; o[1] = p[1]; o[2] = p[2];
    }
}
}

extern "C" int straps_project_targets(const float* joints, const float* cam_t, float fx, float fy, float cx, float cy, float* joints2d,
                                      float* joints3d, long long batch, void* stream) {
    STRAPS_REQUIRE(joints && cam_t && joints2d && joints3d && batch > 0, "straps_project_targets: bad arguments");
    hipLaunchKernelGGL(project_targets_kernel, dim3((unsigned)((batch * 31 + 255) / 256)), dim3(256), 0, (hipStream_t)stream, joints, cam_t, fx,
                       fy, cx, cy, joints2d, joints3d, batch);
    STRAPS_CHECK_LAUNCH("project_targets_kernel");
    return STRAPS_OK;
}
```

straps-3dhumanshapepose_amd/hipabi.py:

```python
import ctypes as C
import os
import subprocess

_HERE = os.path.dirname(os.path.abspath(__file__))
CSRC = os.path.join(_HERE, 'csrc')
LIB_PATH = os.path.join(CSRC, 'libstraps_hip.so')
HEADER = os.path.join(os.path.dirname(_HERE), 'include', 'straps_hip.h')
SOURCES = ['abi.hip', 'augment.hip', 'pose.hip', 'ief.hip', 'elementwise.hip', 'conv.hip', 'conv_x3.hip', 'conv_x3_lean.hip', 'conv_bf16.hip', 'conv_x3f.hip', 'conv_wgrad_x3f.hip', 'stem.hip', 'stem_dgrad.hip', 'smpl.hip',
           'smpl_bwd.hip', 'backward.hip', 'train.hip', 'metrics.hip', 'image.hip', 'raster.hip', 'exchange.hip',
           'regressor.hip', 'regressor_train.hip']

_lib = None
LINK_LIBS = ['-ldl']
EXTRA_FLAGS = {'smpl.hip': ['-fno-slp-vectorize']}


def _existing_sources():
    return [os.path.join(CSRC, s) for s in SOURCES if os.path.isfile(os.path.join(CSRC, s))]


TOOLS_LIB_PATH = os.path.join(os.path.dirname(_HERE), 'tools', 'bin', 'libstraps_hip_tools.so')


def build(force=False, verbose=False, tools=False):
    srcs = _existing_sources()
    lib_path = TOOLS_LIB_PATH if tools else LIB_PATH
    if tools and not force and os.environ.get('STRAPS_TOOLS_NO_BUILD') == '1' and os.path.isfile(lib_path):
        import sys
        import time
        print('hipabi.build(tools=True): STRAPS_TOOLS_NO_BUILD=1 -- reusing %s (built %s)' % (lib_path, time.strftime('%Y-%m-%d %H:%M:%S', time.localtime(os.path.getmtime(lib_path)))),
              file=sys.stderr)
        return lib_path
    import glob
    hdrs = sorted(glob.glob(os.path.join(CSRC, '*.h'))) + [HEADER]
    deps = srcs + hdrs
    if not force and os.path.isfile(lib_path) and all(os.path.getmtime(lib_path) > os.path.getmtime(d) for d in deps):
        if not tools:
            _audit(lib_path, 'hipabi.build (library up to date)')
        return lib_path
    hipcc = os.environ.get('HIPCC', '/opt/rocm/bin/hipcc')
    flags = ['--offload-arch=gfx950', '-O3', '-std=c++17', '-fPIC'] + (['-DSTRAPS_TOOLS'] if tools else [])
    extra = dict(EXTRA_FLAGS)
    if tools and os.environ.get('STRAPS_TOOLS_SMPL_FLAGS'):
        extra['smpl.hip'] = extra.get('smpl.hip', []) + os.environ['STRAPS_TOOLS_SMPL_FLAGS'].split()
    if tools and os.environ.get('STRAPS_TOOLS_SMPL_BWD_FLAGS'):
        extra['smpl_bwd.hip'] = extra.get('smpl_bwd.hip', []) + os.environ['STRAPS_TOOLS_SMPL_BWD_FLAGS'].split()
    if tools and os.environ.get('STRAPS_TOOLS_RASTER_FLAGS'):
        extra['raster.hip'] = extra.get('raster.hip', []) + os.environ['STRAPS_TOOLS_RASTER_FLAGS'].split()
    objdir = os.path.join(os.path.dirname(TOOLS_LIB_PATH), 'build') if tools else os.path.join(CSRC, 'build')
    os.makedirs(objdir, exist_ok=True)
    jobs = []
    for s in srcs:
        o = os.path.join(objdir, os.path.basename(s)[:-4] + '.o')
        if force or not os.path.isfile(o) or any(os.path.getmtime(o) <= os.path.getmtime(d) for d in [s] + hdrs):
            cmd = [hipcc] + flags + extra.get(os.path.basename(s), []) + ['-c', s, '-o', o]
            if verbose:
                print(' '.join(cmd))
            jobs.append((cmd, subprocess.Popen(cmd, cwd=CSRC)))
    for cmd, p in jobs:
        if p.wait() != 0:
            raise subprocess.CalledProcessError(p.returncode, cmd)
    objs = [os.path.join(objdir, os.path.basename(s)[:-4] + '.o') for s in srcs]
    cmd = [hipcc, '--offload-arch=gfx950', '-fPIC', '-shared', '-o', lib_path] + objs + LINK_LIBS
    if verbose:
        print(' '.join(cmd))
    subprocess.run(cmd, check=True, cwd=CSRC)
    if not tools:
        _audit(lib_path, 'hipabi.build', fresh=True)
    return lib_path


def _audit(lib_path, what, fresh=False):
    from . import isa_audit
    if not fresh and isa_audit.stamp_ok(lib_path):
        return
    if not isa_audit.enforce(lib_path, what):
        import warnings
        warnings.warn('%s: llvm-objdump not found under %s -- the packed-operand-select audit of %s (DESIGN section 1: wrong results in lanes 48..63 on '
                      'MI355X) did NOT run; set STRAPS_LLVM_BIN or audit the library where it was built (tools/audit_packed_fp32.py)'
                      % (what, isa_audit.LLVM_BIN, lib_path), RuntimeWarning, stacklevel=3)


class SmplModelStruct(C.Structure):
    _fields_ = [('blend_frag', C.c_void_p), ('j_template', C.c_void_p), ('j_shapedirs', C.c_void_p),
                ('parents', C.c_void_p), ('depth', C.c_void_p), ('max_depth', C.c_int32), ('skin_k', C.c_int32),
                ('skin_w', C.c_void_p), ('skin_j', C.c_void_p), ('vj_ptr', C.c_void_p), ('n_tiles', C.c_int32),
                ('reserved0', C.c_int32), ('pick_ids', C.c_void_p), ('blend_frag_t', C.c_void_p), ('children', C.c_void_p),
                ('jrt_ptr', C.c_void_p), ('jrt_code', C.c_void_p), ('jrt_w', C.c_void_p), ('dj_ptr', C.c_void_p), ('dj_code', C.c_void_p),
                ('dj_w', C.c_void_p), ('blend_frag_h', C.c_void_p), ('blend_h_unscale', C.c_float), ('reserved1', C.c_int32), ('skin_frag_p', C.c_void_p)]


class PackDesc(C.Structure):
    _fields_ = [('src', C.c_void_p), ('dst_krsc', C.c_void_p), ('dst_crsk', C.c_void_p), ('o', C.c_int32), ('c', C.c_int32),
                ('r', C.c_int32), ('s', C.c_int32), ('first', C.c_longlong)]


class GemmDesc(C.Structure):
    _fields_ = [('a', C.c_void_p), ('sam', C.c_longlong), ('sak', C.c_longlong), ('b', C.c_void_p), ('sbk', C.c_longlong), ('sbn', C.c_longlong),
                ('c', C.c_void_p), ('ldc', C.c_int32), ('accumulate', C.c_int32), ('addend', C.c_void_p), ('ldadd', C.c_int32), ('reserved0', C.c_int32),
                ('mask', C.c_void_p), ('ldmask', C.c_int32), ('reserved1', C.c_int32), ('c2', C.c_void_p), ('ldc2', C.c_int32), ('accumulate2', C.c_int32),
                ('m', C.c_int32), ('n', C.c_int32), ('k', C.c_int32), ('reserved2', C.c_int32)]


def gemm_desc(a, sam, sak, b, sbk, sbn, c, ldc, m, n, k, accumulate=0, addend=None, ldadd=0, mask=None, ldmask=0, c2=None, ldc2=0, accumulate2=0):
    adr = lambda t: None if t is None else (t if isinstance(t, int) else t.data_ptr())
    return GemmDesc(adr(a), sam, sak, adr(b), sbk, sbn, adr(c), ldc, accumulate, adr(addend), ldadd, 0, adr(mask), ldmask, 0, adr(c2), ldc2, accumulate2,
                    m, n, k, 0)


def gemm_multi(descs):
    arr = (GemmDesc * len(descs))(*descs)
    check(lib().straps_gemm_multi(arr, len(descs), stream_ptr()), 'straps_gemm_multi')


class RegressorDesc(C.Structure):
    _fields_ = [('layers', C.c_int32), ('in_channels', C.c_int32), ('ief_iters', C.c_int32), ('precision', C.c_int32)]


_P, _I, _L, _F, _Z, _D = C.c_void_p, C.c_int, C.c_longlong, C.c_float, C.c_size_t, C.c_double

ABI_VERSION = 12
SIGNATURES = {
    'straps_abi_version': (_I, []),
    'straps_last_error': (C.c_char_p, []),
    'straps_device_count': (_I, []),
    'straps_wall_clock_khz': (_I, []),
    'straps_set_clock_accumulator': (_I, [_P]),
    'straps_selftest_mfma_peak': (_I, [_P, _P, _I, _I, _P]),
    'straps_selftest_mfma_bf16': (_I, [_P, _P, _I, _I, _P]),
    'straps_selftest_mfma_bf16_dense': (_I, [_P, _P, _I, _I, _I, _P]),
    'straps_pack_conv_weight': (_I, [_P, _P, _I, _I, _I, _I, _P]),
    'straps_pack_conv_weight_dgrad': (_I, [_P, _P, _I, _I, _I, _I, _P]),
    'straps_pack_conv_weights_batched': (_I, [_P, _I, _L, _P]),
    'straps_pack_conv_weights_batched_x3': (_I, [_P, _I, _L, _P, _P, _L, _P]),
    'straps_stem_weight_floats': (_Z, [_I]),
    'straps_pack_stem_weight': (_I, [_P, _P, _I, _P]),
    'straps_bn_fold': (_I, [_P, _P, _P, _P, _F, _P, _P, _I, _P]),
    'straps_bn_fold_stats': (_I, [_P, _P, _P, _P, _F, _P, _P, _P, _P, _I, _P]),
    'straps_stem_stat_blocks': (_I, [_I, _I, _I]),
    'straps_stem_nzmask_words': (_Z, [_I, _I, _I, _I]),
    'straps_stem_nzmask': (_I, [_P, _P, _I, _I, _I, _I, _P]),
    'straps_stem_fwd': (_I, [_P, _P, _P, _P, _I, _P, _P, _P, _I, _I, _I, _I, _P]),
    'straps_conv_trace_buffer': (_I, [_P]),
    'straps_split3_bf16': (_I, [_P, _P, _L, _L, _P]),
    'straps_split3_bf16_cm': (_I, [_P, _P, _L, _I, _L, _P]),
    'straps_conv_fwd_x3': (_I, [_P, _L, _P, _L, _P, _P, _P, _I, _P, _P, _I, _I, _I, _I, _I, _I, _I, _I, _I, _I, _P]),
    'straps_conv_fwd_x3p': (_I, [_P, _L, _P, _L, _P, _P, _P, _I, _P, _P, _L, _I, _I, _I, _I, _I, _I, _I, _I, _I, _I, _P]),
    'straps_conv_dgrad_x3': (_I, [_P, _L, _P, _L, _P, _P, _I, _I, _I, _I, _I, _I, _I, _I, _I, _I, _P]),
    'straps_split_bf16_cm': (_I, [_P, _P, _L, _I, _P]),
    'straps_pack_conv_weight_bf16': (_I, [_P, _P, _I, _I, _I, _I, _P]),
    'straps_conv_bf16_tile_choice': (_I, [_I] * 9),
    'straps_conv_fwd_bf16': (_I, [_P, _P, _P, _P, _P, _I, _P, _P] + [_I] * 10 + [_P]),
    'straps_conv_x3_stat_blocks': (_I, [_I] * 10),
    'straps_conv_x3f_supported': (_I, [_I] * 6),
    'straps_conv_fwd_x3f': (_I, [_P, _P, _P, _I, _P, _L, _P, _P, _P, _I, _P, _P] + [_I] * 10 + [_P]),
    'straps_conv_x3f_stat_blocks': (_I, [_I] * 10),
    'straps_conv_dgrad_x3f': (_I, [_P, _P, _L, _P, _P, _P] + [_I] * 10 + [_P] * 8),
    'straps_conv_dgrad_x3f_bn_blocks': (_I, [_I] * 10),
    'straps_conv_wgrad_x3f_workspace_bytes': (_Z, [_I] * 9),
    'straps_conv_wgrad_x3f': (_I, [_P, _P, _P, _I, _P, _P, _P] + [_I] * 10 + [_P]),
    'straps_bn_apply_x3': (_I, [_P, _P, _P, _P, _I, _P, _P, _L, _L, _I, _P]),
    'straps_bn_relu_maxpool_fwd_x3': (_I, [_P, _P, _P, _P, _P, _P, _L, _I, _I, _I, _I, _P]),
    'straps_conv_wgrad_x3_on_planes': (_I, [_I] * 9),
    'straps_conv_dgrad_x3_bn_blocks': (_I, [_I] * 10),
    'straps_conv_dgrad_x3_bn': (_I, [_P, _L, _P, _L, _P, _P, _I, _I, _I, _I, _I, _I, _I, _I, _I, _I, _P, _P, _P, _P, _P, _P, _P, _P]),
    'straps_bn_bwd_finish_x3': (_I, [_P] * 13 + [_L, _P, _I, _P, _L, _I, _I, _P]),
    'straps_conv_wgrad_x3': (_I, [_P, _P, _P, _L, _P, _L, _P, _P, _I, _I, _I, _I, _I, _I, _I, _I, _I, _I, _P]),
    'straps_bn_bwd_x3': (_I, [_P] * 13 + [_L, _P, _L, _I, _I, _P]),
    'straps_bn_apply_bits_x3': (_I, [_P, _P, _P, _P, _P, _P, _L, _P, _L, _I, _P]),
    'straps_bn_bwd_bits_x3': (_I, [_P] * 10 + [_L, _P, _L, _I, _I, _P]),
    'straps_bn_bwd_finish_bits_x3': (_I, [_P] * 10 + [_L, _P, _I, _P, _L, _I, _I, _P]),
    'straps_conv_dgrad_x3_bits': (_I, [_P, _L, _P, _L, _P, _P, _I, _I, _I, _I, _I, _I, _I, _I, _I, _I, _P, _P]),
    'straps_conv_dgrad_x3_bn_bits': (_I, [_P, _L, _P, _L, _P, _P, _I, _I, _I, _I, _I, _I, _I, _I, _I, _I, _P, _P, _P, _P, _P, _P, _P, _P, _P, _P]),
    'straps_conv_stat_blocks': (_I, [_I, _I, _I, _I, _I, _I]),
    'straps_conv_fwd': (_I, [_P, _P, _P, _P, _P, _I, _P, _P, _I, _I, _I, _I, _I, _I, _I, _I, _I, _I, _P]),
    'straps_maxpool_fwd': (_I, [_P, _P, _I, _I, _I, _I, _P]),
    'straps_gap_fwd': (_I, [_P, _P, _I, _I, _I, _P]),
    'straps_bn_stats_finalize': (_I, [_P, _I, _I, _L, _P, _P, _F, _F, _P, _P, _P, _P, _P, _P, _P]),
    'straps_bn_apply': (_I, [_P, _P, _P, _P, _I, _P, _L, _I, _P]),
    'straps_linear_fwd': (_I, [_P, _I, _P, _I, _P, _P, _P, _I, _I, _I, _I, _I, _P]),
    'straps_broadcast_rows': (_I, [_P, _I, _P, _I, _I, _P]),
    'straps_ief_pack': (_I, [_P, _P, _P, _P, _P, _I, _I, _I, _I, _I, _P]),
    'straps_gemm_multi': (_I, [C.POINTER(GemmDesc), _I, _P]),
    'straps_rot6d_fwd': (_I, [_P, _L, _I, _P, _L, _P]),
    'straps_rodrigues_fwd': (_I, [_P, _P, _L, _P]),
    'straps_rodrigues_bwd': (_I, [_P, _P, _P, _L, _P]),
    'straps_orthographic_project': (_I, [_P, _P, _I, _P, _L, _I, _P]),
    'straps_orthographic_project_bwd': (_I, [_P, _P, _I, _P, _P, _P, _L, _I, _P]),
    'straps_perspective_project': (_I, [_P, _P, _P, _P, _I, _P, _L, _I, _P]),
    'straps_smpl_workspace_bytes': (_Z, [C.POINTER(SmplModelStruct), _L]),
    'straps_smpl_fwd': (_I, [C.POINTER(SmplModelStruct), _P, _P, _P, _P, _P, _L, _I, _I, _P]),
    'straps_smpl_bwd_workspace_bytes': (_Z, [_L, _I]),
    'straps_smpl_bwd': (_I, [C.POINTER(SmplModelStruct), _P, _P, _P, _P, _P, _P, _P, _L, _I, _P]),
    'straps_smpl_bwd_aa': (_I, [C.POINTER(SmplModelStruct), _P, _P, _P, _P, _P, _P, _P, _P, _P, _L, _I, _P]),
    'straps_conv_dgrad': (_I, [_P, _P, _P, _P, _I, _I, _I, _I, _I, _I, _I, _I, _I, _I, _P]),
    'straps_conv_wgrad_workspace_bytes': (_Z, [_I, _I, _I, _I, _I, _I, _I, _I, _I]),
    'straps_conv_wgrad': (_I, [_P, _P, _P, _P, _I, _I, _I, _I, _I, _I, _I, _I, _I, _I, _P]),
    'straps_stem_wgrad_workspace_bytes': (_Z, [_I, _I, _I, _I]),
    'straps_stem_wgrad': (_I, [_P, _P, _P, _P, _P, _I, _I, _I, _I, _I, _P]),
    'straps_stem_dgrad_weight_floats': (_Z, [_I]),
    'straps_pack_stem_dgrad_weight': (_I, [_P, _P, _I, _P]),
    'straps_stem_dgrad': (_I, [_P, _P, _P, _I, _I, _I, _I, _I, _P]),
    'straps_bn_bwd_blocks': (_I, [_L, _I]),
    'straps_bn_bwd_workspace_bytes': (_Z, [_L, _I]),
    'straps_bn_bwd': (_I, [_P, _P, _P, _P, _P, _P, _P, _P, _P, _P, _P, _P, _P, _L, _I, _I, _P]),
    'straps_bn_relu_maxpool_fwd': (_I, [_P, _P, _P, _P, _P, _I, _I, _I, _I, _P]),
    'straps_bn_bwd_pooled': (_I, [_P, _P, _P, _P, _P, _P, _P, _P, _P, _P, _P, _P, _I, _I, _I, _I, _I, _P]),
    'straps_bn_bwd_pooled_sparse': (_I, [_P, _P, _P, _P, _P, _P, _P, _P, _P, _P, _P, _P, _I, _I, _I, _I, _I, _P, _P]),
    'straps_stem_tiles': (_Z, [_I, _I, _I]),
    'straps_stem_tile_activity': (_I, [_P, _P, _I, _I, _I, _I, _P]),
    'straps_maxpool_fwd_idx': (_I, [_P, _P, _P, _I, _I, _I, _I, _P]),
    'straps_maxpool_bwd': (_I, [_P, _P, _P, _I, _I, _I, _I, _P]),
    'straps_gap_bwd': (_I, [_P, _P, _I, _I, _I, _P]),
    'straps_masked_copy': (_I, [_P, _I, _P, _I, _P, _I, _I, _I, _I, _P]),
    'straps_rot6d_bwd': (_I, [_P, _L, _I, _P, _P, _L, _L, _P]),
    'straps_build_proxy_input': (_I, [_P, _P, _P, _I, _I, _I, _P]),
    'straps_build_proxy_input_std': (_I, [_P, _P, _P, _I, _I, _I, _I, _P]),
    'straps_build_proxy_input_nz': (_I, [_P, _P, _P, _P, _I, _I, _I, _I, _P]),
    'straps_loss_workspace_bytes': (_Z, [_L]),
    'straps_loss_fwd_bwd': (_I, [_P, _P, _P, _I, _P, _P, _P, _P, _P, _P, _P, _P, _P, _P, _P, _P, _P, _P, _L, _I, _P]),
    'straps_loss_fwd_bwd_gm': (_I, [_P, _P, _P, _I, _P, _P, _P, _P, _P, _P, _P, _P, _P, _P, _P, _P, _P, _P, _L, _I, _P, _F, _P]),
    'straps_count_visible': (_I, [_P, _P, _L, _I, _I, _P]),
    'straps_adam_step': (_I, [_P, _P, _P, _P, _L, _I, _F, _F, _F, _F, _F, _P, _P]),
    'straps_mse_fwd': (_I, [_P, _P, _P, _L, _I, _F, _F, _P, _P, _P]),
    'straps_mse_bwd': (_I, [_P, _P, _P, _L, _I, _F, _F, _P, _P, _P]),
    'straps_augment_seg': (_I, [_P, _P, _P, _F, _I, _P, _I, _I, _P]),
    'straps_rasterize_workspace_bytes': (_Z, [_L, _I, _I]),
    'straps_rasterize_parts': (_I, [_P, _P, _P, _P, _P, _P, _P, _P, _P, _L, _I, _I, _I, _I, _F, _F, _P, _D, _D, _P]),
    'straps_philox_fill': (_I, [C.c_ulonglong, _P, _L, C.c_uint, _P, _L, _I, _P]),
    'straps_counter_add': (_I, [_P, _I, _L, _P]),
    'straps_gather_f32': (_I, [_P, _P, _P, _I, _P]),
    'straps_memset_zero': (_I, [_P, _Z, _P]),
    'straps_augment_smpl': (_I, [_P, _L, _P, _P, _P, _P, _I, _P, _D, _D, _P, _P, _P, _L, _P]),
    'straps_augment_cam_t': (_I, [_P, _P, _P, _D, _D, _D, _P, _L, _P]),
    'straps_deviate_verts2d': (_I, [_P, _P, _D, _D, _P, _L, _P]),
    'straps_deviate_joints2d': (_I, [_P, _P, _D, _D, _D, _D, _P, _L, _P]),
    'straps_project_targets': (_I, [_P, _P, _F, _F, _F, _F, _P, _P, _L, _P]),
    'straps_point_metrics': (_I, [_P, _P, _P, _L, _I, _P]),
    'straps_crop_resize': (_I, [_P, _P, _P, _D, _D, _D, _D, _D, _P, _P, _P, _I, _I, _I, _I, _P]),
    'straps_comm_unique_id': (_I, [_P]),
    'straps_comm_init_rank': (_I, [_P, _I, _I, C.POINTER(C.c_void_p)]),
    'straps_comm_destroy': (_I, [_P]),
    'straps_comm_size': (_I, [_P]),
    'straps_comm_library': (C.c_char_p, []),
    'straps_allreduce_grads': (_I, [_P, _L, _P, _P]),
    'straps_regressor_param_floats': (_Z, [C.POINTER(RegressorDesc)]),
    'straps_regressor_prepared_bytes': (_Z, [C.POINTER(RegressorDesc)]),
    'straps_regressor_prepare': (_I, [C.POINTER(RegressorDesc), _P, _P, _P]),
    'straps_regressor_workspace_bytes': (_Z, [C.POINTER(RegressorDesc), _I, _I, _I]),
    'straps_regressor_fwd_infer': (_I, [C.POINTER(RegressorDesc), _P, _P, _I, _I, _I, _P, _I, _P, _P, _Z, _P]),
    'straps_regressor_train_param_floats': (_Z, [C.POINTER(RegressorDesc)]),
    'straps_regressor_bn_state_floats': (_Z, [C.POINTER(RegressorDesc)]),
    'straps_regressor_train_workspace_bytes': (_Z, [C.POINTER(RegressorDesc), _I, _I, _I]),
    'straps_regressor_fwd_train': (_I, [C.POINTER(RegressorDesc), _P, _P, _P, _P, _I, _I, _I, _P, _I, _P, _Z, _P]),
    'straps_regressor_bwd': (_I, [C.POINTER(RegressorDesc), _P, _P, _I, _I, _I, _P, _I, _P, _P, _P, _Z, _P]),
    'straps_regressor_export_infer_params': (_I, [C.POINTER(RegressorDesc), _P, _P, _P, _P, _P]),
}


def load(path=None):
    global _lib
    if _lib is not None and path is None:
        return _lib
    p = path or LIB_PATH
    if not os.path.isfile(p):
        raise RuntimeError('libstraps_hip.so is not built (%s missing): run `python -c "import __graft_entry__ as g; '
                           'g.build()"` -- this package has no CPU fallback' % p)
    if os.path.abspath(p) != os.path.abspath(TOOLS_LIB_PATH):
        _audit(p, 'hipabi.load')
    lib = C.CDLL(p)
    if hasattr(lib, 'straps_abi_version'):
        lib.straps_abi_version.restype = C.c_int
        got = lib.straps_abi_version()
        if got != ABI_VERSION:
            raise RuntimeError('%s is ABI version %d, this package binds version %d: rebuild it (`python -c "import __graft_entry__ as g; g.build()"`)'
                               % (p, got, ABI_VERSION))
    for name, (res, args) in SIGNATURES.items():
        if not hasattr(lib, name):
            continue
        fn = getattr(lib, name)
        fn.restype = res
        fn.argtypes = args
    if path is None:
        _lib = lib
    return lib


def lib():
    return load()


def use_library(path):
    global _lib
    _lib = load(path)
    return _lib


_TRACE = os.environ.get('STRAPS_TRACE_CALLS')
_trace_fh = None


def check(rc, what):
    if rc != 0:
        raise RuntimeError('%s failed (code %d): %s' % (what, rc, lib().straps_last_error().decode()))
    if _TRACE:
        import torch
        global _trace_fh
        if _trace_fh is None:
            _trace_fh = open(_TRACE, 'a', buffering=1)
        if not torch.cuda.is_current_stream_capturing():
            _trace_fh.write(what + '\n')
            _trace_fh.flush()
            os.fsync(_trace_fh.fileno())
            torch.cuda.synchronize()


def stream_ptr():
    import torch
    return C.c_void_p(torch.cuda.current_stream().cuda_stream)


def _first_cuda_tensor(values):
    import torch
    for v in values:
        if isinstance(v, torch.Tensor):
            if v.is_cuda:
                return v
        elif isinstance(v, dict):
            t = _first_cuda_tensor(v.values())
            if t is not None:
                return t
    return None


def on_tensor_device(fn):
    import functools

    @functools.wraps(fn)
    def wrapper(*a, **k):
        import torch
        t = _first_cuda_tensor(list(a) + list(k.values()))
        if t is None or t.device.index == torch.cuda.current_device():
            return fn(*a, **k)
        with torch.cuda.device(t.device):
            return fn(*a, **k)
    return wrapper


def ptr(t):
    return C.c_void_p(0 if t is None else t.data_ptr())


def require_gpu_tensor(t, name, dtype=None):
    import torch
    if not isinstance(t, torch.Tensor) or not t.is_cuda:
        raise RuntimeError('%s must be a GPU tensor: the STRAPS hot path runs only through the HIP library '
                           '(no CPU fallback)' % name)
    if dtype is not None and t.dtype != dtype:
        raise RuntimeError('%s must have dtype %s (got %s)' % (name, dtype, t.dtype))
    if t.device.index != torch.cuda.current_device():
        raise RuntimeError('%s lives on %s but the current device is cuda:%d: kernels are launched on the current device\'s '
                           'stream -- call torch.cuda.set_device(%d) or wrap the call in `with torch.cuda.device(...)`'
                           % (name, t.device, torch.cuda.current_device(), t.device.index))
    return t
```

straps-3dhumanshapepose_amd/smpl.py:

```python
import ctypes as C
from collections import namedtuple

import numpy as np
import torch
import torch.nn as nn

from . import hipabi
from .synthetic_smpl import load_smpl_model

ModelOutput = namedtuple('ModelOutput', ['vertices', 'joints', 'full_pose', 'betas', 'global_orient', 'body_pose'])
ModelOutput.__new__.__defaults__ = (None,) * len(ModelOutput._fields)

V, VPAD, TILES, KP = 6890, 6912, 216, 224
PRECISIONS = {'fp32': 0, 'fp16x3': 1, 'fp16x3_lbs': 2, 'fp16x3_lbs_pd16': 3, 'fp16x3_lbs_p16': 4}
KERNELS = {'auto': 0, 'wide': 0x100, 'narrow': 0x200, 'wide_builtin': 0x100 | 0x400}


def pack_smpl_model(model):
    vt = np.asarray(model['v_template'], np.float64)
    sd = np.asarray(model['shapedirs'], np.float64)
    pd = np.asarray(model['posedirs'], np.float64)
    Jr = np.asarray(model['J_regressor'], np.float64)
    W = np.asarray(model['weights'], np.float32)
    assert vt.shape == (V, 3) and sd.shape == (V, 3, 10) and pd.shape == (207, V * 3) and W.shape == (V, 24)
    D = np.zeros((KP, VPAD, 3), np.float32)
    D[0, :V] = vt
    D[1:11, :V] = np.transpose(sd, (2, 0, 1))
    D[11:218, :V] = pd.reshape(207, V, 3)
    R45 = np.concatenate([np.asarray(model[n], np.float64) for n in
                          ('J_regressor_extra', 'J_regressor_cocoplus', 'J_regressor_h36m')], axis=0)
    assert R45.shape == (45, V)
    D64 = np.zeros((V, 218, 3), np.float64)
    D64[:, 0] = vt
    D64[:, 1:11] = np.transpose(sd, (0, 2, 1))
    D64[:, 11:] = pd.reshape(207, V, 3).transpose(1, 0, 2)
    D64 = D64.reshape(V, 218 * 3)
    W64 = W.astype(np.float64)
    vdirs, vs_, vk_, vjn = [], [], [], np.zeros(45, np.int64)
    for j in range(45):
        cols = np.nonzero(R45[j])[0]
        if cols.size == 0:
            continue
        Cj = R45[j, cols, None] * W64[cols]
        for kb in np.nonzero(np.any(Cj != 0, axis=0))[0]:
            c = Cj[:, kb]
            parts = [c] if abs(c.sum()) >= 0.25 * np.abs(c).sum() else [np.where(c > 0, c, 0.0), np.where(c < 0, c, 0.0)]
            for cp in parts:
                s_ = cp.sum()
                if s_ == 0:
                    continue
                vdirs.append((cp @ D64[cols]) / s_)
                vs_.append(s_)
                vk_.append(kb)
                vjn[j] += 1
    nvirt = len(vs_)
    vj_ptr = np.concatenate([[0], np.cumsum(vjn)]).astype(np.int32)
    n_tiles = ((TILES + (nvirt + 31) // 32 + 7) // 8) * 8
    Dall = np.zeros((KP, n_tiles * 32, 3), np.float32)
    Dall[:, :VPAD] = D
    if nvirt:
        Dall[:218, VPAD:VPAD + nvirt] = np.asarray(vdirs).reshape(nvirt, 218, 3).transpose(1, 0, 2)
    frag = Dall.reshape(28, 2, 4, n_tiles, 32, 3).transpose(3, 5, 0, 1, 4, 2).copy()
    dmax = float(np.abs(Dall).max())
    sd_exp = 14 if dmax == 0 else int(min(14, np.floor(np.log2(32768.0 / dmax))))
    Ds = Dall.astype(np.float32) * np.float32(2.0 ** sd_exp)
    Dh = Ds.astype(np.float16)
    Dl = (Ds - Dh.astype(np.float32)).astype(np.float16)
    assert np.isfinite(Dh.astype(np.float32)).all()
    frag_h = np.stack([Dh, Dl], axis=0).reshape(2, KP // 16, 2, 8, n_tiles, 32, 3).transpose(4, 1, 6, 0, 2, 5, 3).copy()
    parents = np.asarray(model['parents'], np.int32).copy()
    depth = np.zeros(24, np.int32)
    for j in range(1, 24):
        assert 0 <= parents[j] < j, 'parents must be topologically ordered'
        depth[j] = depth[parents[j]] + 1
    nnz = (W != 0).sum(1)
    k = int(max(1, nnz.max()))
    order = np.argsort(-(W != 0).astype(np.int8), axis=1, kind='stable')[:, :k]
    sw = np.zeros((n_tiles * 32, k), np.float32)
    sj = np.zeros((n_tiles * 32, k), np.int32)
    sw[:V] = np.take_along_axis(W, order, axis=1)
    sj[:V] = np.where(sw[:V] != 0, order, 0)
    if nvirt:
        sw[VPAD:VPAD + nvirt, 0] = np.asarray(vs_, np.float32)
        sj[VPAD:VPAD + nvirt, 0] = np.asarray(vk_, np.int32)
    Wd = np.zeros((n_tiles * 32, 32), np.float32)
    np.add.at(Wd, (np.repeat(np.arange(n_tiles * 32), k), sj.reshape(-1)), sw.reshape(-1))
    assert float(np.abs(Wd).max()) < 3.9, 'skinning weight too large for the fp16 split (|w| * 2^14 must stay below 65504)'
    Ws = Wd * np.float32(2.0 ** 14)
    Wh = Ws.astype(np.float16)
    Wl = (Ws - Wh.astype(np.float32)).astype(np.float16)
    Wp = np.concatenate([Wh[:, :24], Wh[:, :24], Wl[:, :24], np.zeros((n_tiles * 32, 8), np.float16)], axis=1)
    skin_frag_p = Wp.reshape(n_tiles, 32, 5, 2, 8).transpose(0, 2, 3, 1, 4).copy()
    jj, vv = np.nonzero(R45)
    o = np.lexsort((vv, jj))
    jj, vv = jj[o], vv[o]
    r_ = np.arange(16)
    rows = (r_[None, :] & 3) + 8 * (r_[None, :] >> 2) + 4 * np.arange(2)[:, None]
    Dk = D.reshape(7, 32, TILES, 32, 3)
    Dt = Dk[:, :, :, rows, :]
    frag_t = Dt.reshape(7, 32, TILES, 2, 4, 4, 3).transpose(2, 6, 0, 4, 3, 1, 5).copy()
    children = -np.ones((24, 3), np.int32)
    for j in range(1, 24):
        slot = int((children[parents[j]] >= 0).sum())
        assert slot < 3, 'a joint with more than 3 children is not supported'
        children[parents[j], slot] = j
    pj = np.arange(21)
    pv = np.asarray(model['extra_vertex_ids'], np.int64)
    src = np.concatenate([pj, 21 + jj])
    vs = np.concatenate([pv, vv])
    ws = np.concatenate([np.ones(21, np.float32), R45[jj, vv].astype(np.float32)])
    o2 = np.lexsort((src, vs))
    src, vs, ws = src[o2], vs[o2], ws[o2]
    jrt_ptr = np.zeros(TILES + 1, np.int32)
    np.add.at(jrt_ptr, vs // 32 + 1, 1)
    jrt_ptr = np.cumsum(jrt_ptr).astype(np.int32)
    dv, dk = np.nonzero(sw[:VPAD])
    dj, dw = sj[:VPAD][dv, dk], sw[:VPAD][dv, dk]
    o3 = np.lexsort((dv, dj, dv // 128))
    dv, dj, dw = dv[o3], dj[o3], dw[o3]
    dj_ptr = np.zeros(54 * 24 + 1, np.int32)
    np.add.at(dj_ptr, (dv // 128) * 24 + dj + 1, 1)
    dj_ptr = np.cumsum(dj_ptr).astype(np.int32)
    dj_code = ((((dv % 128) // 32) << 5) | (dv % 32)).astype(np.int32)
    return {
        'dj_ptr': dj_ptr, 'dj_code': dj_code, 'dj_w': dw.astype(np.float32),
        'blend_frag_t': frag_t.reshape(-1), 'children': children,
        'jrt_ptr': jrt_ptr, 'jrt_code': (((vs % 32) << 8) | src).astype(np.int32), 'jrt_w': ws,
        'blend_frag': frag.reshape(-1),
        'blend_frag_h': frag_h.reshape(-1), 'blend_h_unscale': float(2.0 ** -(sd_exp + 6)),         'skin_frag_p': skin_frag_p.reshape(-1),
        'j_template': (Jr @ vt).astype(np.float32),
        'j_shapedirs': np.einsum('jv,vcl->jcl', Jr, sd).astype(np.float32),
        'parents': parents, 'depth': depth, 'max_depth': int(depth.max()), 'skin_k': k,
        'skin_w': sw, 'skin_j': sj,
        'vj_ptr': vj_ptr, 'n_tiles': int(n_tiles),
        'pick_ids': np.asarray(model['extra_vertex_ids'], np.int32),
    }


class SMPL(nn.Module):

    NUM_BODY_JOINTS = 23

    def __init__(self, model_path, batch_size=1, gender='neutral', extra_regressor_paths=None, **kwargs):
        super().__init__()
        model = model_path if isinstance(model_path, dict) else load_smpl_model(model_path, gender, extra_regressor_paths)
        self.batch_size = batch_size
        self.faces = None if model.get('faces') is None else np.asarray(model['faces'])
        self.face_parts = None if model.get('face_parts') is None else np.asarray(model['face_parts'])
        packed = pack_smpl_model(model)
        self.max_depth, self.skin_k, self.n_tiles = packed.pop('max_depth'), packed.pop('skin_k'), packed.pop('n_tiles')
        self.blend_h_unscale = packed.pop('blend_h_unscale')
        precision = kwargs.pop('precision', 'fp32')
        if precision not in PRECISIONS:
            raise ValueError("SMPL: precision must be one of %s" % (sorted(PRECISIONS),))
        self.precision = precision
        for name, arr in packed.items():
            self.register_buffer('_k_' + name, torch.from_numpy(np.ascontiguousarray(arr)), persistent=False)
        self.register_buffer('v_template', torch.tensor(model['v_template'], dtype=torch.float32))
        self.register_buffer('shapedirs', torch.tensor(model['shapedirs'], dtype=torch.float32))
        self.register_buffer('posedirs', torch.tensor(model['posedirs'], dtype=torch.float32))
        self.register_buffer('J_regressor', torch.tensor(model['J_regressor'], dtype=torch.float32))
        self.register_buffer('lbs_weights', torch.tensor(model['weights'], dtype=torch.float32))
        self.register_buffer('parents', torch.tensor(model['parents'], dtype=torch.long))
        self.register_buffer('J_regressor_extra', torch.tensor(model['J_regressor_extra'], dtype=torch.float32))
        self.register_buffer('J_regressor_cocoplus', torch.tensor(model['J_regressor_cocoplus'], dtype=torch.float32))
        self.register_buffer('J_regressor_h36m', torch.tensor(model['J_regressor_h36m'], dtype=torch.float32))
        self.betas = nn.Parameter(torch.zeros(batch_size, 10))
        self.global_orient = nn.Parameter(torch.zeros(batch_size, 3))
        self.body_pose = nn.Parameter(torch.zeros(batch_size, self.NUM_BODY_JOINTS * 3))
        self.transl = nn.Parameter(torch.zeros(batch_size, 3))
        self._struct = None
        self._struct_key = None

    def _model_struct(self):
        key = self._k_blend_frag.data_ptr()
        if self._struct_key != key:
            s = hipabi.SmplModelStruct()
            for f in ('blend_frag', 'blend_frag_h', 'skin_frag_p', 'j_template', 'j_shapedirs', 'parents', 'depth', 'skin_w', 'skin_j', 'vj_ptr',
                      'pick_ids', 'blend_frag_t', 'children', 'jrt_ptr', 'jrt_code', 'jrt_w', 'dj_ptr', 'dj_code', 'dj_w'):
                setattr(s, f, getattr(self, '_k_' + f).data_ptr())
            s.max_depth, s.skin_k, s.n_tiles = self.max_depth, self.skin_k, self.n_tiles
            s.blend_h_unscale = self.blend_h_unscale
            self._struct, self._struct_key = s, key
        return self._struct

    @hipabi.on_tensor_device
    def forward_arrays(self, betas, rotmats, want_joints=True, chunks=0, out_verts=None, out_joints=None, precision=None, kernel='auto'):
        if kernel not in KERNELS:
            raise ValueError("SMPL.forward_arrays: kernel must be one of %s" % (sorted(KERNELS),))
        hipabi.require_gpu_tensor(betas, 'betas', torch.float32)
        hipabi.require_gpu_tensor(rotmats, 'rotmats', torch.float32)
        hipabi.require_gpu_tensor(self._k_blend_frag, 'SMPL model buffers (call .to(device))')
        B = betas.shape[0]
        if tuple(betas.shape) != (B, 10) or tuple(rotmats.shape) != (B, 24, 3, 3):
            raise RuntimeError('SMPL: expected betas [B,10] and rotmats [B,24,3,3], got %s and %s'
                               % (tuple(betas.shape), tuple(rotmats.shape)))
        betas, rotmats = betas.contiguous(), rotmats.contiguous()
        L = hipabi.lib()
        verts = torch.empty(B, V, 3, device=betas.device, dtype=torch.float32) if out_verts is None else out_verts
        joints = None
        if want_joints:
            joints = torch.empty(B, 90, 3, device=betas.device, dtype=torch.float32) if out_joints is None else out_joints
        for t, shp, nm in ((verts, (B, V, 3), 'out_verts'), (joints, (B, 90, 3), 'out_joints')):
            if t is not None and (tuple(t.shape) != shp or not t.is_contiguous() or t.dtype != torch.float32 or t.device != betas.device):
                raise RuntimeError('SMPL: %s must be a contiguous fp32 %s tensor on %s' % (nm, shp, betas.device))
        ws = torch.empty(L.straps_smpl_workspace_bytes(C.byref(self._model_struct()), B) // 4, device=betas.device, dtype=torch.float32)
        hipabi.check(L.straps_smpl_fwd(C.byref(self._model_struct()), hipabi.ptr(betas), hipabi.ptr(rotmats),
                                       hipabi.ptr(verts), hipabi.ptr(joints), hipabi.ptr(ws), B, chunks,
                                       PRECISIONS[self.precision if precision is None else precision] | KERNELS[kernel], hipabi.stream_ptr()), 'straps_smpl_fwd')
        return verts, joints

    @hipabi.on_tensor_device
    def forward(self, betas=None, body_pose=None, global_orient=None, transl=None, pose2rot=True, **kwargs):
        from .rigid_transform_utils import batch_rodrigues
        betas = self.betas if betas is None else betas
        body_pose = self.body_pose if body_pose is None else body_pose
        global_orient = self.global_orient if global_orient is None else global_orient
        B = max(betas.shape[0], body_pose.shape[0], global_orient.shape[0])
        if betas.shape[0] != B:
            betas = betas.expand(B, -1)
        if pose2rot:
            full_pose = torch.cat([global_orient.reshape(-1, 3).expand(B, -1) if global_orient.shape[0] != B
                                   else global_orient.reshape(B, 3), body_pose.reshape(body_pose.shape[0], -1).expand(B, -1)],
                                  dim=1)
            if torch.is_grad_enabled() and (betas.requires_grad or full_pose.requires_grad):
                from .autograd_ops import smpl_aa_forward_autograd
                verts, joints = smpl_aa_forward_autograd(self, betas, full_pose)
            else:
                rotmats = batch_rodrigues(full_pose.detach().reshape(-1, 3)).view(B, 24, 3, 3)
                verts, joints = self.forward_arrays(betas.detach().float(), rotmats)
        else:
            full_pose = torch.cat([global_orient.reshape(-1, 1, 3, 3), body_pose.reshape(-1, 23, 3, 3)], dim=1)
            rotmats = full_pose
            if torch.is_grad_enabled() and (betas.requires_grad or rotmats.requires_grad):
                from .autograd_ops import smpl_forward_autograd
                verts, joints = smpl_forward_autograd(self, betas, rotmats)
            else:
                verts, joints = self.forward_arrays(betas.detach().float(), rotmats.detach().float())
        tr = self.transl if transl is None else transl
        if transl is not None:
            verts = verts + tr[:, None]
            joints = joints + tr[:, None]
        return ModelOutput(vertices=verts, joints=joints, full_pose=full_pose if pose2rot else None, betas=betas,
                           global_orient=global_orient, body_pose=body_pose)
```

straps-3dhumanshapepose_amd/train_step.py:

```python
import ctypes as C
import sys

import numpy as np
import torch

from . import config, hipabi
from .autograd_ops import encoder_backward, ief_backward
from .encoder_exec import encoder_forward
from .ief_module import EST_LD
from .multi_task_loss import TASKS

SMPL_AUGMENT_PARAMS = {'augment_shape': True, 'delta_betas_distribution': 'normal', 'delta_betas_std_vector': [1.5] * 10,
                       'delta_betas_range': [-3., 3.]}
CAM_AUGMENT_PARAMS = {'xy_std': 0.05, 'delta_z_range': [-5, 5]}
BBOX_AUGMENT_PARAMS = {'crop_input': True, 'mean_scale_factor': 1.2, 'delta_scale_range': [-0.2, 0.2], 'delta_centre_range': [-5, 5]}
PROXY_REP_AUGMENT_PARAMS = {'remove_appendages': True, 'deviate_joints2D': True, 'deviate_verts2D': True, 'occlude_seg': True,
                            'remove_appendages_classes': [1, 2, 3, 4, 5, 6],
                            'remove_appendages_probabilities': [0.1, 0.1, 0.1, 0.1, 0.05, 0.05],
                            'delta_j2d_dev_range': [-8, 8], 'delta_j2d_hip_dev_range': [-8, 8], 'delta_verts2d_dev_range': [-0.01, 0.01],
                            'occlude_probability': 0.5, 'occlude_box_dim': 48}
H36M14 = [73 + i for i in config.H36M_TO_J14]


def flatten_parameters(params, device):
    total = sum(p.numel() for p in params)
    flat_p = torch.empty(total, device=device, dtype=torch.float32)
    flat_g = torch.zeros(total, device=device, dtype=torch.float32)
    views, off = {}, 0
    for p in params:
        n = p.numel()
        flat_p[off:off + n].copy_(p.detach().reshape(-1))
        p.data = flat_p[off:off + n].view(p.shape)
        views[p] = flat_g[off:off + n].view(p.shape)
        off += n
    return flat_p, flat_g, views


def allreduce_gradients(flat_g, world_size, group=None):
    if world_size > 1:
        import torch.distributed as dist
        dist.all_reduce(flat_g, op=dist.ReduceOp.SUM, group=group)
    return 1.0 / world_size


def allreduce_visible_count(count, world_size, group=None, async_op=False):
    if world_size > 1:
        import torch.distributed as dist
        return dist.all_reduce(count, op=dist.ReduceOp.SUM, group=group, async_op=async_op)
    return None


_FUSED_PROXY_NZ = True

class GradientExchange:

    def __init__(self, flat_g, split_off, world_size, group=None, force=False, backend='torch', rank=0):
        self.flat_g, self.split_off, self.world, self.group = flat_g, int(split_off), world_size, group
        self.active = world_size > 1 or bool(force)
        self.backend = backend
        self._work = None
        self._comm, self._stream, self._started = None, None, False
        if backend not in ('torch', 'rccl'):
            raise ValueError("GradientExchange: backend must be 'torch' or 'rccl' (got %r)" % (backend,))
        if self.active and backend == 'rccl':
            self._init_rccl(rank)

    def _init_rccl(self, rank):
        if not self.flat_g.is_cuda:
            raise RuntimeError("GradientExchange(backend='rccl') needs the gradient buffer on a GPU")
        L = hipabi.lib()
        grank = rank
        if self.world > 1:
            import torch.distributed as dist
            grank = dist.get_rank(self.group)
            if grank < 0:
                raise RuntimeError("GradientExchange(backend='rccl'): this process is not a member of the group it was given")
            if dist.get_world_size(self.group) != self.world:
                raise RuntimeError("GradientExchange(backend='rccl'): world_size %d != size of the process group %d" % (self.world, dist.get_world_size(self.group)))
        idbuf = (C.c_char * 128)()
        if grank == 0:
            hipabi.check(L.straps_comm_unique_id(idbuf), 'straps_comm_unique_id')
        if self.world > 1:
            box = [bytes(idbuf) if grank == 0 else None]
            dist.broadcast_object_list(box, src=dist.get_global_rank(self.group, 0) if self.group is not None else 0, group=self.group)
            idbuf = (C.c_char * 128).from_buffer_copy(box[0])
        comm = C.c_void_p()
        with torch.cuda.device(self.flat_g.device):
            hipabi.check(L.straps_comm_init_rank(idbuf, self.world, grank, C.byref(comm)), 'straps_comm_init_rank')
            self._stream = torch.cuda.Stream(device=self.flat_g.device)
        self._comm = comm
        if L.straps_comm_size(comm) != self.world:
            n = L.straps_comm_size(comm)
            self.close()
            raise RuntimeError("GradientExchange(backend='rccl'): the communicator reports %d ranks, expected %d" % (n, self.world))

    def close(self):
        if self._comm is not None:
            comm, self._comm = self._comm, None
            torch.cuda.synchronize(self.flat_g.device)
            hipabi.check(hipabi.lib().straps_comm_destroy(comm), 'straps_comm_destroy')

    def __del__(self):
        if sys is None or sys.is_finalizing():
            return
        try:
            self.close()
        except Exception:
            pass

    def _rccl_allreduce(self, lo, hi):
        cur = torch.cuda.current_stream(self.flat_g.device)
        self._stream.wait_stream(cur)
        hipabi.check(hipabi.lib().straps_allreduce_grads(C.c_void_p(self.flat_g.data_ptr() + 4 * lo), hi - lo, self._comm,
                                                          C.c_void_p(self._stream.cuda_stream)), 'straps_allreduce_grads')

    def start_tail(self):
        if not self.active:
            return
        if self.backend == 'rccl':
            if not self._started:
                self._rccl_allreduce(self.split_off, self.flat_g.numel())
                self._started = True
        elif self._work is None:
            import torch.distributed as dist
            self._work = dist.all_reduce(self.flat_g[self.split_off:], op=dist.ReduceOp.SUM, group=self.group, async_op=True)

    def finish(self):
        if self.active:
            self.start_tail()
            if self.backend == 'rccl':
                if self.split_off > 0:
                    self._rccl_allreduce(0, self.split_off)
                torch.cuda.current_stream(self.flat_g.device).wait_stream(self._stream)
                self._started = False
            else:
                import torch.distributed as dist
                self._work.wait()
                self._work = None
                if self.split_off > 0:
                    dist.all_reduce(self.flat_g[:self.split_off], op=dist.ReduceOp.SUM, group=self.group)
        return 1.0 / self.world


class TrainStep:
    def __init__(self, regressor, smpl, criterion, batch_size, lr=1e-4, rank=0, world_size=1, seed=1234, group=None,
                 mean_shape=None, mean_cam_t=(0., 0.2, 42.), pose_pool=None, use_graph=False, overlap_wgrad=False,
                 renderer=None, track_metrics=False, comm_overlap=None, pipeline_data=True, smpl_augment_params=None,
                 cam_augment_params=None, bbox_augment_params=None, proxy_rep_augment_params=None, global_masked_mean=False,
                 force_exchange=False, exchange_backend='torch'):
        if getattr(regressor.image_encoder, 'conv_precision', 'fp32') == 'bf16':
            raise RuntimeError("TrainStep: conv_precision='bf16' is an inference-only route (no gradients): train on 'bf16x3' or 'fp32'")
        p0 = next(regressor.parameters())
        if not (isinstance(p0, torch.Tensor) and p0.is_cuda):
            raise RuntimeError('TrainStep: regressor parameters must be GPU tensors (call .to(device) first): the STRAPS hot path runs only '
                               'through the HIP library (no CPU fallback)')
        self.dev = p0.device
        self._force_exchange, self._exchange_backend = bool(force_exchange), exchange_backend
        with torch.cuda.device(self.dev):
            self._init(regressor, smpl, criterion, batch_size, lr, rank, world_size, seed, group, mean_shape, mean_cam_t, pose_pool, use_graph,
                       overlap_wgrad, renderer, track_metrics, comm_overlap, pipeline_data, smpl_augment_params, cam_augment_params,
                       bbox_augment_params, proxy_rep_augment_params)
            self.global_masked_mean = bool(global_masked_mean) and world_size > 1
            self._vis_work = {}
            if self.global_masked_mean and use_graph and not pipeline_data:
                raise NotImplementedError('global_masked_mean with hipGraph capture needs the data pipeline (the count exchange cannot sit inside a captured graph)')

    def _init(self, regressor, smpl, criterion, batch_size, lr, rank, world_size, seed, group, mean_shape, mean_cam_t, pose_pool, use_graph,
              overlap_wgrad, renderer, track_metrics, comm_overlap, pipeline_data, smpl_augment_params, cam_augment_params, bbox_augment_params,
              proxy_rep_augment_params):
        self.reg, self.smpl, self.crit = regressor, smpl, criterion
        if getattr(criterion, 'reduction', 'mean') != 'mean':
            raise NotImplementedError("TrainStep: the fused loss kernel implements reduction='mean' (run_train.py:196); use the criterion "
                                      "module with autograd for 'sum'")
        self.B, self.lr, self.rank, self.world, self.group = batch_size, lr, rank, world_size, group
        self.params = list(regressor.parameters()) + list(criterion.parameters())
        self.flat_p, self.flat_g, self.gviews = flatten_parameters(self.params, self.dev)
        self.exp_avg = torch.zeros_like(self.flat_p)
        self.exp_avg_sq = torch.zeros_like(self.flat_p)
        self.steps = 0
        self.n_reg = sum(p.numel() for p in regressor.parameters())
        if comm_overlap is None:
            import os
            comm_overlap = (world_size > 1 or self._force_exchange) and os.environ.get('STRAPS_NO_COMM_OVERLAP', '0') != '1'
        self.comm_overlap = bool(comm_overlap)
        split_off, off = 0, 0
        for n_, p_ in regressor.named_parameters():
            if n_.startswith('image_encoder.layer3.'):
                split_off = off
                break
            off += p_.numel()
        self.tail_offset = split_off
        self.exchange = GradientExchange(self.flat_g, split_off if self.comm_overlap else 0, world_size, group, force=self._force_exchange,
                                         backend=self._exchange_backend, rank=rank)
        self.time_exchange, self.exchange_events = False, []
        self.logvar_params = [getattr(criterion, n + '_log_var') for n in TASKS]
        self._lv_index = None
        if all(p.requires_grad and p in self.gviews for p in self.logvar_params):
            offs = [(self.gviews[p].data_ptr() - self.flat_g.data_ptr()) // 4 for p in self.logvar_params]
            base = min(offs)
            if sorted(o - base for o in offs) == list(range(5)):
                rel = [o - base for o in offs]
                inv = [rel.index(i) for i in range(5)]
                self._lv_index = torch.tensor(rel, dtype=torch.int32, device=self.dev)
                self._lv_index_inv = torch.tensor(inv, dtype=torch.int32, device=self.dev)
                self._lv_params_flat = self.flat_p[base:base + 5]
                self._lv_grads_flat = self.flat_g[base:base + 5]
        from .device_rng import DeviceDraws
        self.draws = DeviceDraws(seed + rank, self.dev)
        self.smpl_augment_params = dict(SMPL_AUGMENT_PARAMS if smpl_augment_params is None else smpl_augment_params)
        self.cam_augment_params = dict(CAM_AUGMENT_PARAMS if cam_augment_params is None else cam_augment_params)
        self.bbox_augment_params = dict(BBOX_AUGMENT_PARAMS if bbox_augment_params is None else bbox_augment_params)
        self.proxy_rep_augment_params = dict(PROXY_REP_AUGMENT_PARAMS if proxy_rep_augment_params is None else proxy_rep_augment_params)
        assert self.smpl_augment_params['delta_betas_distribution'] in ['uniform', 'normal']
        self.step_t = torch.zeros(1, dtype=torch.int64, device=self.dev)
        self.use_graph, self.graph, self.graph_tail, self._warm, self._g_loss = use_graph, None, None, 0, None
        self.side_stream = torch.cuda.Stream(device=self.dev) if overlap_wgrad else None
        d = self.dev
        self.mean_shape = torch.zeros(10, device=d) if mean_shape is None else torch.as_tensor(mean_shape, dtype=torch.float32, device=d)
        self.mean_cam_t = torch.tensor(mean_cam_t, device=d).expand(batch_size, 3).contiguous()
        self._eye = torch.eye(3, device=d).expand(batch_size, 24, 3, 3).contiguous()
        K = np.array([[config.FOCAL_LENGTH, 0., config.REGRESSOR_IMG_WH / 2.0], [0., config.FOCAL_LENGTH, config.REGRESSOR_IMG_WH / 2.0],
                      [0., 0., 1.]], dtype=np.float32)
        self.cam_K = torch.from_numpy(K).to(d)
        from .augmentation import remove_probabilities
        self.remove_prob = remove_probabilities(self.proxy_rep_augment_params, d)
        std = self.smpl_augment_params.get('delta_betas_std_vector')
        self._std_vector = None if std is None else torch.as_tensor(std, dtype=torch.float32, device=d).expand(10).contiguous()
        self.pool_shape = self.mean_shape[None].expand(batch_size, 10).contiguous()
        if renderer is None:
            if smpl.faces is None or smpl.face_parts is None:
                raise RuntimeError('TrainStep: the SMPL model carries no faces / face_parts; pass renderer=NMRRenderer(...)')
            from .nmr_renderer import NMRRenderer
            renderer = NMRRenderer(batch_size, self.cam_K.cpu(), torch.eye(3), config.REGRESSOR_IMG_WH, rend_parts_seg=True,
                                   faces=smpl.faces, face_parts=smpl.face_parts).to(d)
        self.renderer = renderer
        self.metrics = None
        if track_metrics:
            from .metrics import BatchMetrics
            self.metrics = BatchMetrics(self.dev)
        self._coco = torch.tensor(config.ALL_JOINTS_TO_COCO_MAP, device=d)
        self._h36m14 = torch.tensor([config.ALL_JOINTS_TO_H36M_MAP[k] for k in config.H36M_TO_J14], device=d)
        bns = [m for m in regressor.image_encoder.modules() if isinstance(m, torch.nn.BatchNorm2d) and m.track_running_stats
               and m.num_batches_tracked is not None]
        self.nbt_flat = torch.stack([m.num_batches_tracked.detach().to(d) for m in bns]) if bns else None
        for k, m in enumerate(bns):
            m.num_batches_tracked = self.nbt_flat[k]
        regressor.image_encoder._nbt_flat = self.nbt_flat
        if pose_pool is None:
            g = torch.Generator().manual_seed(seed)
            pose_pool = torch.randn(4096, 72, generator=g) * 0.2
            pose_pool[:, :3] = 0
            pose_pool[:, 1] = (torch.rand(4096, generator=g) * 2 - 1) * np.pi * 0.5
        self.pose_pool = pose_pool.to(d)
        self.last = {}
        self.pipeline = bool(pipeline_data)
        self.data_stream = torch.cuda.Stream(device=d) if self.pipeline else None
        self._bufs = [self._new_buffers() for _ in range(2)] if self.pipeline else None
        self._cur, self._primed = 0, False
        self._last_by_parity = {}

    def _new_buffers(self):
        d, B = self.dev, self.B
        return dict(input=torch.empty(B, 18, 256, 256, device=d), verts=torch.empty(B, 6890, 3, device=d),
                    joints2d=torch.empty(B, 17, 2, device=d), joints3d=torch.empty(B, 14, 3, device=d),
                    shape=torch.empty(B, 10, device=d), rot=torch.empty(B, 24, 3, 3, device=d),
                    reposed=torch.empty(B, 6890, 3, device=d), cam_t=torch.empty(B, 3, device=d), vis_count=torch.zeros(1, device=d),
                    nzmask=torch.empty(hipabi.lib().straps_stem_nzmask_words(B, 18, 256, 256), device=d, dtype=torch.int32))

    def draw_layout(self):
        B = self.B
        u, off = {}, 0
        for name, n in (('pose_index', B), ('cam_z', B), ('crop', 3 * B), ('seg', 9 * B), ('joints2d', 34 * B), ('shape_uniform', 10 * B),
                        ('verts2d', 2 * 6890 * B)):
            u[name] = (off, n)
            off += (n + 3) // 4 * 4
        n_shape = (10 * B + 3) // 4 * 4
        return {'uniform': u, 'n_uniform': off, 'normal': {'shape': (0, 10 * B), 'cam_xy': (n_shape, 2 * B)}, 'n_normal': n_shape + 2 * B}

    def make_batch(self, out=None, keep=None):
        L, st, d, B = hipabi.lib(), hipabi.stream_ptr(), self.dev, self.B
        out = self._new_buffers() if out is None else out
        lay = self.draw_layout()
        U = self.draws.fill(torch.empty(lay['n_uniform'], device=d), 0, 0)
        N = self.draws.fill(torch.empty(lay['n_normal'], device=d), 1, 1)
        self.draws.advance()

        def useg(name):
            o, n = lay['uniform'][name]
            return U[o:o + n]

        def nseg(name):
            o, n = lay['normal'][name]
            return N[o:o + n]
        sp, cp, bp, pp = self.smpl_augment_params, self.cam_augment_params, self.bbox_augment_params, self.proxy_rep_augment_params
        mode = 0
        if sp['augment_shape']:
            mode = 1 if sp['delta_betas_distribution'] == 'normal' else 2
        sdraws = nseg('shape') if mode == 1 else useg('shape_uniform')
        rng = sp['delta_betas_range'] if mode == 2 else (0.0, 0.0)
        tgt_shape, tgt_rot = out['shape'], out['rot']
        hipabi.check(L.straps_augment_smpl(hipabi.ptr(self.pose_pool), self.pose_pool.shape[0], hipabi.ptr(useg('pose_index')),
                                           hipabi.ptr(self.pool_shape), hipabi.ptr(self.mean_shape), hipabi.ptr(sdraws), mode, hipabi.ptr(self._std_vector),
                                           float(rng[0]), float(rng[1]), hipabi.ptr(tgt_shape), hipabi.ptr(tgt_rot), None, B, st),
                     'straps_augment_smpl')
        cam_t = out['cam_t']
        hipabi.check(L.straps_augment_cam_t(hipabi.ptr(self.mean_cam_t), hipabi.ptr(nseg('cam_xy')), hipabi.ptr(useg('cam_z')), float(cp['xy_std']),
                                            float(cp['delta_z_range'][0]), float(cp['delta_z_range'][1]), hipabi.ptr(cam_t), B, st),
                     'straps_augment_cam_t')
        tgt_verts, tgt_joints = self.smpl.forward_arrays(tgt_shape, tgt_rot, out_verts=out['verts'])
        self.smpl.forward_arrays(tgt_shape, self._eye, want_joints=False, out_verts=out['reposed'])
        j2d_full = torch.empty(B, 17, 2, device=d)
        wh = float(config.REGRESSOR_IMG_WH)
        hipabi.check(L.straps_project_targets(hipabi.ptr(tgt_joints), hipabi.ptr(cam_t), config.FOCAL_LENGTH, config.FOCAL_LENGTH, wh / 2, wh / 2,
                                              hipabi.ptr(j2d_full), hipabi.ptr(out['joints3d']), B, st), 'straps_project_targets')
        noise = useg('verts2d') if pp['deviate_verts2D'] else None
        seg = self.renderer.render_arrays(tgt_verts, cam_t, vert_noise_u=noise, noise_range=pp['delta_verts2d_dev_range'])
        if bp['crop_input']:
            from .image_utils import batch_crop_and_resize
            seg_c, tgt_j2d, boxes = batch_crop_and_resize(seg, j2d_full, config.REGRESSOR_IMG_WH, bp['mean_scale_factor'], bp['delta_scale_range'],
                                                          bp['delta_centre_range'], uniforms=useg('crop'), jout=out['joints2d'])
        else:
            seg_c, boxes = seg, None
            tgt_j2d = out['joints2d']
            hipabi.check(L.straps_masked_copy(hipabi.ptr(j2d_full), 34, None, 0, hipabi.ptr(tgt_j2d), 34, B, 34, 0, st), 'joints2d copy')
        seg_aug = torch.empty_like(seg_c)
        hipabi.check(L.straps_augment_seg(hipabi.ptr(seg_c), hipabi.ptr(useg('seg')), hipabi.ptr(self.remove_prob),
                                          float(pp['occlude_probability']) if pp['occlude_seg'] else 0.0, int(pp['occlude_box_dim']),
                                          hipabi.ptr(seg_aug), B, 256, st), 'straps_augment_seg')
        j2d_in = tgt_j2d
        if pp['deviate_joints2D']:
            j2d_in = torch.empty(B, 17, 2, device=d)
            r, hr = pp['delta_j2d_dev_range'], pp['delta_j2d_hip_dev_range']
            hipabi.check(L.straps_deviate_joints2d(hipabi.ptr(tgt_j2d), hipabi.ptr(useg('joints2d')), float(r[0]), float(r[1]), float(hr[0]),
                                                   float(hr[1]), hipabi.ptr(j2d_in), B, st), 'straps_deviate_joints2d')
        x = out['input']
        if _FUSED_PROXY_NZ:
            hipabi.check(L.straps_build_proxy_input_nz(hipabi.ptr(seg_aug), hipabi.ptr(j2d_in), hipabi.ptr(x), hipabi.ptr(out['nzmask']), B, 17, 256, 4, st),
                         'straps_build_proxy_input_nz')
        else:
            hipabi.check(L.straps_build_proxy_input(hipabi.ptr(seg_aug), hipabi.ptr(j2d_in), hipabi.ptr(x), B, 17, 256, st), 'straps_build_proxy_input')
            hipabi.check(L.straps_stem_nzmask(hipabi.ptr(x), hipabi.ptr(out['nzmask']), B, 18, 256, 256, st), 'straps_stem_nzmask')
        hipabi.check(L.straps_count_visible(hipabi.ptr(tgt_j2d), hipabi.ptr(out['vis_count']), B, 17, config.REGRESSOR_IMG_WH, st), 'straps_count_visible')
        if keep is not None:
            keep.update(uniforms=U, normals=N, joints=tgt_joints, joints2d_uncropped=j2d_full, seg=seg, seg_cropped=seg_c, boxes=boxes,
                        seg_aug=seg_aug, joints2d_input=j2d_in)
        return out

    def forward_backward(self, batch, after_layer3=None):
        L, st, d, B = hipabi.lib(), hipabi.stream_ptr(), self.dev, self.B
        reg, smpl = self.reg, self.smpl
        assert reg.training, 'TrainStep needs the regressor in .train() mode'
        hipabi.check(L.straps_memset_zero(hipabi.ptr(self.flat_g), self.flat_g.numel() * 4, st), 'straps_memset_zero(flat gradient)')
        enc_tape, ief_tape = {}, []
        reg.image_encoder.prepack(with_dgrad=True)
        if self.nbt_flat is not None:
            hipabi.check(L.straps_counter_add(hipabi.ptr(self.nbt_flat), self.nbt_flat.numel(), 1, st), 'straps_counter_add(num_batches_tracked)')
        feat = encoder_forward(reg.image_encoder, batch['input'], enc_tape, nzmask=batch.get('nzmask'))
        est = reg.ief_module.forward_estimate(feat, ief_tape)
        pose6d = est[:, 3:147]
        R = torch.empty(B, 24, 3, 3, device=d)
        hipabi.check(L.straps_rot6d_fwd(hipabi.ptr(pose6d), EST_LD, 24, hipabi.ptr(R), B, st), 'straps_rot6d_fwd')
        pred_shape = torch.empty(B, 10, device=d)
        hipabi.check(L.straps_masked_copy(C.c_void_p(est.data_ptr() + 4 * 147), EST_LD, None, 0, hipabi.ptr(pred_shape), 10, B, 10, 0, st), 'pred_shape')
        verts, joints = smpl.forward_arrays(pred_shape, R)
        eye = self._eye
        reposed, _ = smpl.forward_arrays(pred_shape, eye, want_joints=False)
        if self._lv_index is not None:
            lv = torch.empty(5, device=d)
            hipabi.check(L.straps_gather_f32(hipabi.ptr(self._lv_params_flat), hipabi.ptr(self._lv_index), hipabi.ptr(lv), 5, st), 'log-var gather')
        else:
            lv = self.crit.log_var_vector()
        loss = torch.empty(12, device=d)
        dverts, djoints = torch.empty_like(verts), torch.empty_like(joints)
        dest, drot = torch.empty(B, EST_LD, device=d), torch.empty(B, 24, 3, 3, device=d)
        dlv = torch.empty(5, device=d)
        ws = torch.empty(L.straps_loss_workspace_bytes(B) // 4, device=d)
        gm = getattr(self, 'global_masked_mean', False)
        hipabi.check(L.straps_loss_fwd_bwd_gm(hipabi.ptr(verts), hipabi.ptr(joints), hipabi.ptr(est), EST_LD, hipabi.ptr(R), hipabi.ptr(batch['verts']),
                                              hipabi.ptr(batch['joints2d']), hipabi.ptr(batch['joints3d']), hipabi.ptr(batch['shape']),
                                              hipabi.ptr(batch['rot']), hipabi.ptr(lv), hipabi.ptr(loss), hipabi.ptr(dverts), hipabi.ptr(djoints),
                                              hipabi.ptr(dest), hipabi.ptr(drot), hipabi.ptr(dlv), hipabi.ptr(ws), B, config.REGRESSOR_IMG_WH,
                                              hipabi.ptr(batch['vis_count'] if gm else None), 1.0 / self.world, st),
                     'straps_loss_fwd_bwd')
        dbetas, drot2 = torch.empty(B, 10, device=d), torch.empty(B, 24, 3, 3, device=d)
        ws2 = torch.empty(L.straps_smpl_bwd_workspace_bytes(B, 0) // 4, device=d)
        hipabi.check(L.straps_smpl_bwd(C.byref(smpl._model_struct()), hipabi.ptr(pred_shape), hipabi.ptr(R), hipabi.ptr(dverts), hipabi.ptr(djoints),
                                       hipabi.ptr(dbetas), hipabi.ptr(drot2), hipabi.ptr(ws2), B, 0, st), 'straps_smpl_bwd')
        hipabi.check(L.straps_masked_copy(hipabi.ptr(drot2), 216, None, 0, hipabi.ptr(drot), 216, B, 216, 1, st), 'drot sum')
        hipabi.check(L.straps_masked_copy(hipabi.ptr(dbetas), 10, None, 0, C.c_void_p(dest.data_ptr() + 4 * 147), EST_LD, B, 10, 1, st), 'dshape sum')
        hipabi.check(L.straps_rot6d_bwd(hipabi.ptr(pose6d), EST_LD, 24, hipabi.ptr(drot), C.c_void_p(dest.data_ptr() + 4 * 3), EST_LD, B, st),
                     'straps_rot6d_bwd')
        dfeat, _ = ief_backward(reg.ief_module, feat, ief_tape, dest, self.gviews)
        if self._lv_index is not None:
            hipabi.check(L.straps_gather_f32(hipabi.ptr(dlv), hipabi.ptr(self._lv_index_inv), hipabi.ptr(self._lv_grads_flat), 5, st), 'log-var gradient scatter')
        else:
            for k, p in enumerate(self.logvar_params):
                if p.requires_grad:
                    self.gviews[p].copy_(dlv[k])
        encoder_backward(reg.image_encoder, enc_tape, dfeat, self.gviews, self.side_stream, after_layer3)
        self.last = dict(loss=loss, verts=verts, joints=joints, est=est, reposed=reposed, rot=R, ief_tape=ief_tape,
                         enc_tape=enc_tape if getattr(self, 'keep_enc_tape', False) else None,
                         bwd=dict(dverts=dverts, djoints=djoints, dlv=dlv, dbetas=dbetas, drot_smpl=drot2, dest=dest, dfeat=dfeat)
                         if getattr(self, 'keep_bwd', False) else None)
        if self.metrics is not None:
            from .cam_utils import orthographic_project_torch
            pred = {'verts': verts, 'joints3D': joints.index_select(1, self._h36m14), 'shape_params': pred_shape,
                    'pose_params_rot_matrices': R,
                    'joints2D': orthographic_project_torch(joints.index_select(1, self._coco), est[:, :3])}
            tgt = {'verts': batch['verts'], 'joints3D': batch['joints3d'], 'shape_params': batch['shape'],
                   'pose_params_rot_matrices': batch['rot'], 'joints2D': batch['joints2d']}
            self.metrics.update(pred, tgt, pred_reposed_vertices=reposed, target_reposed_vertices=batch['reposed'])
        return loss

    def metrics_summary(self):
        if self.metrics is None:
            raise RuntimeError('TrainStep was built with track_metrics=False')
        self.metrics.n = self.steps * self.B
        return self.metrics.summary()

    def optimise(self):
        if self.time_exchange and self.exchange.active:
            e0, e1 = torch.cuda.Event(enable_timing=True), torch.cuda.Event(enable_timing=True)
            e0.record()
            gscale = self.exchange.finish()
            e1.record()
            self.exchange_events.append((e0, e1))
        else:
            gscale = self.exchange.finish()
        self.steps += 1
        hipabi.check(hipabi.lib().straps_counter_add(hipabi.ptr(self.step_t), 1, 1, hipabi.stream_ptr()), 'straps_counter_add(adam step)')
        hipabi.check(hipabi.lib().straps_adam_step(hipabi.ptr(self.flat_p), hipabi.ptr(self.flat_g), hipabi.ptr(self.exp_avg),
                                                   hipabi.ptr(self.exp_avg_sq), self.flat_p.numel(), self.steps, self.lr, 0.9, 0.999, 1e-8,
                                                   gscale, hipabi.ptr(self.step_t), hipabi.stream_ptr()), 'straps_adam_step')
        self.reg.image_encoder._cache.clear()
        self.reg.ief_module._cache = {}

    def _run(self, after_layer3):
        if not self.pipeline:
            b = self.make_batch()
            if self.global_masked_mean:
                allreduce_visible_count(b['vis_count'], self.world, self.group)
            return self.forward_backward(b, after_layer3)
        if not self._primed:
            self.make_batch(out=self._bufs[self._cur])
            self._primed = True
        cur, nxt = self._bufs[self._cur], self._bufs[1 - self._cur]
        main, side = torch.cuda.current_stream(), self.data_stream
        side.wait_stream(main)
        with torch.cuda.stream(side):
            self.make_batch(out=nxt)
        state = {'joined': False}

        def join():
            if not state['joined']:
                main.wait_stream(side)
                state['joined'] = True

        def hook():
            join()
            after_layer3()

        loss = self.forward_backward(cur, hook if after_layer3 is not None else None)
        join()
        return loss

    def step(self):
        with torch.cuda.device(self.dev), torch.no_grad():
            start_tail = self.exchange.start_tail if self.comm_overlap else None
            gm = self.global_masked_mean and self.pipeline
            if gm:
                if not self._primed:
                    self.make_batch(out=self._bufs[self._cur])
                    self._primed = True
                w = self._vis_work.pop(self._cur, None)
                if w is None:
                    allreduce_visible_count(self._bufs[self._cur]['vis_count'], self.world, self.group)
                else:
                    w.wait()

            def count_next():
                if gm:
                    self._vis_work[self._cur] = allreduce_visible_count(self._bufs[self._cur]['vis_count'], self.world, self.group, async_op=True)

            def eager():
                loss = self._run(start_tail)
                self._cur ^= 1
                count_next()
                self.optimise()
                return loss
            if not self.use_graph or self._warm < 2:
                self._warm += 1
                return eager()
            if self.graph is None:
                self._capture()
                if not self.use_graph:
                    return eager()
            par = self._cur if self.pipeline else 0
            g1, g2, loss = self.graph[par]
            self.last = self._last_by_parity[par]
            g1.replay()
            if g2 is not None:
                self.exchange.start_tail()
                g2.replay()
            self._cur ^= 1
            count_next()
            self.optimise()
            return loss

    def _capture_one(self):
        if not self.comm_overlap:
            g = torch.cuda.CUDAGraph()
            with torch.cuda.graph(g, pool=self._pool, capture_error_mode='thread_local'):
                loss = self._run(None)
            if self._pool is None:
                self._pool = g.pool()
            return g, None, loss
        g1, g2 = torch.cuda.CUDAGraph(), torch.cuda.CUDAGraph()
        s = torch.cuda.Stream(device=self.dev)
        s.wait_stream(torch.cuda.current_stream())
        state = {'second': False}

        def switch():
            g1.capture_end()
            if self._pool is None:
                self._pool = g1.pool()
            g2.capture_begin(pool=self._pool, capture_error_mode='thread_local')
            state['second'] = True

        with torch.cuda.stream(s):
            if self._pool is None:
                g1.capture_begin(capture_error_mode='thread_local')
            else:
                g1.capture_begin(pool=self._pool, capture_error_mode='thread_local')
            try:
                loss = self._run(switch)
            finally:
                (g2 if state['second'] else g1).capture_end()
        torch.cuda.current_stream().wait_stream(s)
        if not state['second']:
            raise RuntimeError('the backward pass never reached the split point')
        return g1, g2, loss

    def _capture(self):
        torch.cuda.synchronize()
        self._pool = None
        start, last0, by_parity0 = self._cur, self.last, dict(self._last_by_parity)
        try:
            graphs = {}
            for par in ((start, 1 - start) if self.pipeline else (0,)):
                self._cur = par
                self.reg.image_encoder._cache.clear()
                self.reg.ief_module._cache = {}
                graphs[par] = self._capture_one()
                self._last_by_parity[par] = self.last
            self._cur = start
            self.graph = graphs
            self.graph_tail = next(iter(graphs.values()))[1]
            ok, why = True, ''
        except Exception as e:
            ok, why = False, str(e)
        if self.world > 1:
            import torch.distributed as dist
            flag = torch.tensor([1.0 if ok else 0.0], device=self.dev)
            dist.all_reduce(flag, op=dist.ReduceOp.MIN, group=self.group)
            if ok and float(flag.item()) < 1.0:
                ok, why = False, 'capture failed on another rank'
        if not ok:
            import warnings
            warnings.warn('hipGraph capture of the training step failed (%s); continuing with eager launches' % (why,))
            self.use_graph, self.graph, self.graph_tail = False, None, None
            self._cur, self.last, self._last_by_parity = start, last0, by_parity0
            self.reg.image_encoder._cache.clear()
            self.reg.ief_module._cache = {}
            torch.cuda.synchronize()

    def close(self):
        ex = getattr(self, 'exchange', None)
        if ex is not None:
            ex.close()

    def __del__(self):
        if sys is None or sys.is_finalizing():
            return
        try:
            self.close()
        except Exception:
            pass

    def state_dict(self):
        state, off = {}, 0
        for i, p in enumerate(self.params):
            n = p.numel()
            state[i] = {'step': torch.tensor(float(self.steps)), 'exp_avg': self.exp_avg[off:off + n].view(p.shape).clone(),
                        'exp_avg_sq': self.exp_avg_sq[off:off + n].view(p.shape).clone()}
            off += n
        group = {'lr': self.lr, 'betas': (0.9, 0.999), 'eps': 1e-8, 'weight_decay': 0, 'amsgrad': False, 'maximize': False,
                 'foreach': None, 'capturable': False, 'differentiable': False, 'fused': None, 'params': list(range(len(self.params)))}
        return {'state': state, 'param_groups': [group]}

    def data_state(self):
        return self.draws.step() - (1 if self.pipeline and self._primed else 0)

    def set_data_state(self, step):
        with torch.cuda.device(self.dev):
            torch.cuda.synchronize()
            self.draws.set_step(step)
            self._primed = False
            for w in getattr(self, '_vis_work', {}).values():
                w.wait()
            self._vis_work = {}
            if self.graph is not None:
                self.graph, self.graph_tail, self._warm, self._last_by_parity = None, None, 0, {}

    def load_state_dict(self, sd):
        groups = sd.get('param_groups', [])
        if len(groups) != 1:
            raise ValueError('TrainStep.load_state_dict: expected one parameter group (run_train.py:200), got %d' % len(groups))
        g = groups[0]
        if len(g['params']) != len(self.params):
            raise ValueError('TrainStep.load_state_dict: the state covers %d parameters, this step has %d' % (len(g['params']), len(self.params)))
        if tuple(g.get('betas', (0.9, 0.999))) != (0.9, 0.999) or g.get('eps', 1e-8) != 1e-8 or g.get('weight_decay', 0) != 0 \
                or g.get('amsgrad', False):
            raise ValueError('TrainStep.load_state_dict: only torch.optim.Adam defaults (betas (0.9, 0.999), eps 1e-8, no weight decay, '
                             'no amsgrad) are implemented by straps_adam_step')
        self.lr = float(g.get('lr', self.lr))
        state = sd.get('state', {})
        steps = set()
        with torch.cuda.device(self.dev), torch.no_grad():
            off = 0
            for i, p in zip(g['params'], self.params):
                n = p.numel()
                st = state.get(i, state.get(str(i)))
                if st is None:
                    self.exp_avg[off:off + n].zero_()
                    self.exp_avg_sq[off:off + n].zero_()
                else:
                    if tuple(st['exp_avg'].shape) != tuple(p.shape):
                        raise ValueError('TrainStep.load_state_dict: parameter %d has shape %s, the state %s' % (i, tuple(p.shape), tuple(st['exp_avg'].shape)))
                    self.exp_avg[off:off + n].copy_(st['exp_avg'].reshape(-1).to(self.dev, torch.float32))
                    self.exp_avg_sq[off:off + n].copy_(st['exp_avg_sq'].reshape(-1).to(self.dev, torch.float32))
                    steps.add(int(float(st['step'])))
                off += n
            if len(steps) > 1:
                raise ValueError('TrainStep.load_state_dict: per-parameter step counts differ (%s); one fused Adam launch keeps one count' % sorted(steps))
            self.steps = steps.pop() if steps else 0
            self.step_t.fill_(self.steps)
```

Measured before the change: 8226.

## Stage SMPL backward tables in LDS, fuse loss kernels, skip unused reposed forward

The SMPL vertex backward kernel gets a templated path that copies the per-round skinning weights, joint-regressor and dJ tables into LDS. It also prefetches the dverts stage and batches the scatter loops to hide latency, with a KW==4 vectorised skinning specialisation. The loss partial-sum and gradient kernels are each merged into one launch, with per-wave barriers and bpermute reductions in place of block syncs. The reposed SMPL forward now runs only when metrics are requested. In exchange the kernel uses more LDS and more complex control flow, and any table longer than the LDS cap falls back to global memory.

```diff
diff --git a/include/straps_hip.h b/include/straps_hip.h
--- a/include/straps_hip.h
+++ b/include/straps_hip.h
@@ -129,7 +129,7 @@
     const int32_t* skin_j;
     const int32_t* vj_ptr;
     int32_t n_tiles;
-    int32_t reserved0;
+    int32_t bwd_jrt_round_max;
     const int32_t* pick_ids;
     const float* blend_frag_t;
     const int32_t* children;
diff --git a/straps-3dhumanshapepose_amd/csrc/common.h b/straps-3dhumanshapepose_amd/csrc/common.h
--- a/straps-3dhumanshapepose_amd/csrc/common.h
+++ b/straps-3dhumanshapepose_amd/csrc/common.h
@@ -34,6 +34,13 @@
 #else
 #define STRAPS_NO_PACKED_FP32
 #endif
+#define STRAPS_WG_BARRIER()                                    \
+    do {                                                       \
+        __builtin_amdgcn_fence(__ATOMIC_RELEASE, "workgroup"); \
+        __builtin_amdgcn_s_barrier();                          \
+        __builtin_amdgcn_fence(__ATOMIC_ACQUIRE, "workgroup"); \
+    } while (0)
+#define STRAPS_LANE_XOR(value, mask, lane) __builtin_bit_cast(float, __builtin_amdgcn_ds_bpermute(((lane) ^ (mask)) << 2, __builtin_bit_cast(int, (float)(value))))
 
 inline hipError_t straps_raise_dynamic_lds(const void* fn, size_t bytes, unsigned long long& done) {
     int dev = 0;
diff --git a/straps-3dhumanshapepose_amd/csrc/smpl_bwd.hip b/straps-3dhumanshapepose_amd/csrc/smpl_bwd.hip
--- a/straps-3dhumanshapepose_amd/csrc/smpl_bwd.hip
+++ b/straps-3dhumanshapepose_amd/csrc/smpl_bwd.hip
@@ -6,7 +6,70 @@
 constexpr int KP = STRAPS_SMPL_KP, KG = KP / 8, NT = STRAPS_SMPL_TILES, NV = STRAPS_SMPL_V, NROUNDS = NT / 4;
 constexpr int BT = 32, AS = 292, SS = 193;
 constexpr int NJS = STRAPS_SMPL_NPICK + STRAPS_SMPL_NEXTRA;
-
+constexpr int TAB_KW_MAX = 8, TAB_SKIN = 128 * TAB_KW_MAX, TAB_JRT_MAX = 1280, TAB_WORDS = 4 * TAB_SKIN + 2 * TAB_JRT_MAX;
+constexpr int TAB_QS = TAB_SKIN / 256, TAB_QJ = TAB_JRT_MAX / 256;
+constexpr int OWN_NB = 8, JRT_NB = 4;
+typedef int i32x4 __attribute__((ext_vector_type(4)));
+
+#ifdef STRAPS_TOOLS
+__device__ long long g_smpl_bwd_phase[8];
+#define PHASE_MARK(k)                                                  \
+    do {                                                               \
+        if (ph_on) {                                                   \
+            __builtin_amdgcn_sched_barrier(0);                         \
+            const long long now__ = clock64();                         \
+            __builtin_amdgcn_sched_barrier(0);                         \
+            ph[k] += now__ - ph_t;                                     \
+            ph_t = now__;                                              \
+        }                                                              \
+    } while (0)
+#else
+#define PHASE_MARK(k) do { } while (0)
+#endif
+
+template <int KWC>
+__device__ __forceinline__ void skin_bwd_rows(const float* __restrict__ Ab, const float* tsw, const int* tsj, float* svb, int h, int kw, f32x16& ax,
+                                              f32x16& ay, f32x16& az) {
+#pragma unroll
+    for (int r = 0; r < 16; ++r) {
+        const int vrow = (r & 3) + 8 * (r >> 2) + 4 * h;
+        float* sv = svb + vrow * 6;
+        const float gx = sv[0], gy = sv[1], gz = sv[2];
+        sv[3] = ax[r]; sv[4] = ay[r]; sv[5] = az[r];
+        float t00 = 0.f, t01 = 0.f, t02 = 0.f, t10 = 0.f, t11 = 0.f, t12 = 0.f, t20 = 0.f, t21 = 0.f, t22 = 0.f;
+        if constexpr (KWC == 4) {
+            const f32x4 w4 = *reinterpret_cast<const f32x4*>(tsw + vrow * 4);
+            const i32x4 j4 = *reinterpret_cast<const i32x4*>(tsj + vrow * 4);
+#pragma unroll
+            for (int k = 0; k < 4; ++k) {
+                const float w = w4[k];
+                const int jo = j4[k] * 12;
+                const f32x4 a0 = *reinterpret_cast<const f32x4*>(Ab + jo);
+                const f32x4 a1 = *reinterpret_cast<const f32x4*>(Ab + jo + 4);
+                const f32x4 a2 = *reinterpret_cast<const f32x4*>(Ab + jo + 8);
+                t00 = fmaf(w, a0[0], t00); t01 = fmaf(w, a0[1], t01); t02 = fmaf(w, a0[2], t02);
+                t10 = fmaf(w, a1[0], t10); t11 = fmaf(w, a1[1], t11); t12 = fmaf(w, a1[2], t12);
+                t20 = fmaf(w, a2[0], t20); t21 = fmaf(w, a2[1], t21); t22 = fmaf(w, a2[2], t22);
+            }
+        } else {
+            for (int k = 0; k < kw; ++k) {
+                const float w = tsw[vrow * kw + k];
+                const int jo = tsj[vrow * kw + k] * 12;
+                const f32x4 a0 = *reinterpret_cast<const f32x4*>(Ab + jo);
+                const f32x4 a1 = *reinterpret_cast<const f32x4*>(Ab + jo + 4);
+                const f32x4 a2 = *reinterpret_cast<const f32x4*>(Ab + jo + 8);
+                t00 = fmaf(w, a0[0], t00); t01 = fmaf(w, a0[1], t01); t02 = fmaf(w, a0[2], t02);
+                t10 = fmaf(w, a1[0], t10); t11 = fmaf(w, a1[1], t11); t12 = fmaf(w, a1[2], t12);
+                t20 = fmaf(w, a2[0], t20); t21 = fmaf(w, a2[1], t21); t22 = fmaf(w, a2[2], t22);
+            }
+        }
+        ax[r] = fmaf(t20, gz, fmaf(t00, gx, __fmul_rn(t10, gy)));
+        ay[r] = fmaf(t21, gz, fmaf(t01, gx, __fmul_rn(t11, gy)));
+        az[r] = fmaf(t22, gz, fmaf(t02, gx, __fmul_rn(t12, gy)));
+    }
+}
+
+template <bool TAB>
 __global__ __launch_bounds__(256, 1) STRAPS_NO_PACKED_FP32 void smpl_verts_bwd_kernel(straps_smpl_model_t m, const float* __restrict__ F,
                                                                 const float* __restrict__ Amat, const float* __restrict__ dverts,
                                                                 const float* __restrict__ djoints, float* __restrict__ dFp,
@@ -14,6 +77,12 @@
     extern __shared__ __attribute__((aligned(16))) float smem[];
     float* As_ = smem;
     float* stage = As_ + BT * AS;
+    float* tab_sw = stage + 4 * BT * SS;
+    int* tab_sj = reinterpret_cast<int*>(tab_sw + TAB_SKIN);
+    int* tab_dc = tab_sj + TAB_SKIN;
+    float* tab_dw = reinterpret_cast<float*>(tab_dc + TAB_SKIN);
+    int* tab_jc = reinterpret_cast<int*>(tab_dw + TAB_SKIN);
+    float* tab_jw = reinterpret_cast<float*>(tab_jc + TAB_JRT_MAX);
 
     const int tid = threadIdx.x, lane = tid & 63, wave = tid >> 6;
     const int h = lane >> 5, bl = lane & 31;
@@ -27,7 +96,7 @@
         if (b < nb) v = *reinterpret_cast<const f32x4*>(Amat + (b0 + b) * 288 + q * 4);
         *reinterpret_cast<f32x4*>(As_ + b * AS + q * 4) = v;
     }
-    __syncthreads();
+    STRAPS_WG_BARRIER();
 
     const int round0 = chunk * rounds_per_chunk;
     const int round1 = min(round0 + rounds_per_chunk, NROUNDS);
@@ -36,6 +105,11 @@
     float* mystage = stage + wave * BT * SS;
     const int KW = m.skin_k;
     const bool vbody = bl < nb;
+#ifdef STRAPS_TOOLS
+    const bool ph_on = blockIdx.x == 0 && blockIdx.y == 0 && wave == 0;
+    long long ph[8] = {0, 0, 0, 0, 0, 0, 0, 0};
+    long long ph_t = ph_on ? clock64() : 0;
+#endif
 
     float dacc[3][12];
 #pragma unroll
@@ -50,6 +124,75 @@
 
     for (int rd = round0; rd < round1; ++rd) {
         const int tile = rd * 4 + wave;
+        [[maybe_unused]] int dj0 = 0, jr0 = 0, jp0 = 0, jp1 = 0, op0[3] = {0, 0, 0}, op1[3] = {0, 0, 0};
+        if constexpr (TAB) {
+            unsigned tq[4 * TAB_QS + 2 * TAB_QJ];
+            dj0 = m.dj_ptr[rd * 24]; jr0 = m.jrt_ptr[rd * 4];
+            const int ndj = min(m.dj_ptr[rd * 24 + 24] - dj0, TAB_SKIN), njr = min(m.jrt_ptr[rd * 4 + 4] - jr0, TAB_JRT_MAX);
+            const int nsk = 128 * KW;
+            const unsigned* gsw = reinterpret_cast<const unsigned*>(m.skin_w) + (long long)rd * nsk;
+            const unsigned* gsj = reinterpret_cast<const unsigned*>(m.skin_j) + (long long)rd * nsk;
+            const unsigned* gdc = reinterpret_cast<const unsigned*>(m.dj_code) + dj0;
+            const unsigned* gdw = reinterpret_cast<const unsigned*>(m.dj_w) + dj0;
+            const unsigned* gjc = reinterpret_cast<const unsigned*>(m.jrt_code) + jr0;
+            const unsigned* gjw = reinterpret_cast<const unsigned*>(m.jrt_w) + jr0;
+#pragma unroll
+            for (int q = 0; q < TAB_QS; ++q) {
+                const int i = q * 256 + tid;
+                tq[q] = i < nsk ? gsw[i] : 0u;
+                tq[TAB_QS + q] = i < nsk ? gsj[i] : 0u;
+                tq[2 * TAB_QS + q] = i < ndj ? gdc[i] : 0u;
+                tq[3 * TAB_QS + q] = i < ndj ? gdw[i] : 0u;
+            }
+#pragma unroll
+            for (int q = 0; q < TAB_QJ; ++q) {
+                const int i = q * 256 + tid;
+                tq[4 * TAB_QS + q] = i < njr ? gjc[i] : 0u;
+                tq[4 * TAB_QS + TAB_QJ + q] = i < njr ? gjw[i] : 0u;
+            }
+            jp0 = m.jrt_ptr[tile] - jr0; jp1 = m.jrt_ptr[tile + 1] - jr0;
+#pragma unroll
+            for (int i = 0; i < 3; ++i) {
+                const int j = wave + 4 * (2 * i + h);
+                op0[i] = m.dj_ptr[rd * 24 + j] - dj0; op1[i] = m.dj_ptr[rd * 24 + j + 1] - dj0;
+            }
+#pragma unroll
+            for (int q = 0; q < TAB_QS; ++q) {
+                const int i = q * 256 + tid;
+                reinterpret_cast<unsigned*>(tab_sw)[i] = tq[q];
+                reinterpret_cast<unsigned*>(tab_sj)[i] = tq[TAB_QS + q];
+                reinterpret_cast<unsigned*>(tab_dc)[i] = tq[2 * TAB_QS + q];
+                reinterpret_cast<unsigned*>(tab_dw)[i] = tq[3 * TAB_QS + q];
+            }
+#pragma unroll
+            for (int q = 0; q < TAB_QJ; ++q) {
+                const int i = q * 256 + tid;
+                reinterpret_cast<unsigned*>(tab_jc)[i] = tq[4 * TAB_QS + q];
+                reinterpret_cast<unsigned*>(tab_jw)[i] = tq[4 * TAB_QS + TAB_QJ + q];
+            }
+            {
+                const int ncol = min(96, (NV - tile * 32) * 3);
+                const int c0 = lane, c1 = 64 + bl;
+                const bool k0 = dverts && c0 < ncol, k1 = dverts && h == 0 && c1 < ncol;
+                const float* drow = dverts ? dverts + b0 * (long long)(NV * 3) + tile * 96 : nullptr;
+                float* st0 = mystage + (c0 / 3) * 6 + (c0 % 3);
+                float* st1 = mystage + (c1 / 3) * 6 + (c1 % 3);
+#pragma unroll
+                for (int hb = 0; hb < BT; hb += 16) {
+                    float v0[16], v1[16];
+#pragma unroll
+                    for (int q = 0; q < 16; ++q) {
+                        v0[q] = (k0 && hb + q < nb) ? drow[(hb + q) * (long long)(NV * 3) + c0] : 0.f;
+                        v1[q] = (k1 && hb + q < nb) ? drow[(hb + q) * (long long)(NV * 3) + c1] : 0.f;
+                    }
+#pragma unroll
+                    for (int q = 0; q < 16; ++q) {
+                        st0[(hb + q) * SS] = v0[q];
+                        if (h == 0) st1[(hb + q) * SS] = v1[q];
+                    }
+                }
+            }
+        }
         f32x16 ax, ay, az;
 #pragma unroll
         for (int r = 0; r < 16; ++r) { ax[r] = 0.f; ay[r] = 0.f; az[r] = 0.f; }
@@ -77,69 +220,140 @@
                 cx0 = nx0; cy0 = ny0; cz0 = nz0;
             }
         }
-        {
-            const int ncol = min(96, (NV - tile * 32) * 3);
-            for (int i = lane; i < BT * 96; i += 64) {
-                const int b = i / 96, c = i - b * 96;
-                float v = 0.f;
-                if (dverts && b < nb && c < ncol) v = dverts[(b0 + b) * (long long)(NV * 3) + tile * 96 + c];
-                mystage[b * SS + (c / 3) * 6 + (c % 3)] = v;
-            }
-        }
-        __syncthreads();
-        if (djoints && h == 0 && vbody) {
-            const float* dj = djoints + (b0 + bl) * (STRAPS_SMPL_NJOINTS_OUT * 3) + 72;
-            const int e0 = m.jrt_ptr[tile], e1 = m.jrt_ptr[tile + 1];
-            for (int e = e0; e < e1; ++e) {
-                const int code = m.jrt_code[e];
-                const float w = m.jrt_w[e];
-                float* sv = mystage + bl * SS + (code >> 8) * 6;
-                const float* g = dj + (code & 255) * 3;
-                sv[0] = fmaf(w, g[0], sv[0]); sv[1] = fmaf(w, g[1], sv[1]); sv[2] = fmaf(w, g[2], sv[2]);
-            }
-        }
-        __syncthreads();
-        {
-            const float* Ab = As_ + bl * AS;
-#pragma unroll
-            for (int r = 0; r < 16; ++r) {
-                const int vrow = (r & 3) + 8 * (r >> 2) + 4 * h;
-                const int v = tile * 32 + vrow;
-                float* sv = mystage + bl * SS + vrow * 6;
-                const float gx = sv[0], gy = sv[1], gz = sv[2];
-                sv[3] = ax[r]; sv[4] = ay[r]; sv[5] = az[r];
-                float t00 = 0.f, t01 = 0.f, t02 = 0.f, t10 = 0.f, t11 = 0.f, t12 = 0.f, t20 = 0.f, t21 = 0.f, t22 = 0.f;
-                for (int k = 0; k < KW; ++k) {
-                    const float w = m.skin_w[v * KW + k];
-                    const int jo = m.skin_j[v * KW + k] * 12;
-                    const f32x4 a0 = *reinterpret_cast<const f32x4*>(Ab + jo);
-                    const f32x4 a1 = *reinterpret_cast<const f32x4*>(Ab + jo + 4);
-                    const f32x4 a2 = *reinterpret_cast<const f32x4*>(Ab + jo + 8);
-                    t00 += w * a0[0]; t01 += w * a0[1]; t02 += w * a0[2];
-                    t10 += w * a1[0]; t11 += w * a1[1]; t12 += w * a1[2];
-                    t20 += w * a2[0]; t21 += w * a2[1]; t22 += w * a2[2];
-                }
-                ax[r] = t00 * gx + t10 * gy + t20 * gz;
-                ay[r] = t01 * gx + t11 * gy + t21 * gz;
-                az[r] = t02 * gx + t12 * gy + t22 * gz;
-            }
-        }
-        __syncthreads();
-#pragma unroll
-        for (int i = 0; i < 3; ++i) {
-            const int j = wave + 4 * (2 * i + h);
-            const int e0 = m.dj_ptr[rd * 24 + j], e1 = m.dj_ptr[rd * 24 + j + 1];
-            for (int e = e0; e < e1; ++e) {
-                const int code = m.dj_code[e];
-                const float w = m.dj_w[e];
-                const float* sv = stage + ((code >> 5) * BT + bl) * SS + (code & 31) * 6;
-                const float wx = w * sv[0], wy = w * sv[1], wz = w * sv[2];
-                const float x = sv[3], y = sv[4], z = sv[5];
-                dacc[i][0] = fmaf(wx, x, dacc[i][0]); dacc[i][1] = fmaf(wx, y, dacc[i][1]); dacc[i][2] = fmaf(wx, z, dacc[i][2]); dacc[i][3] += wx;
-                dacc[i][4] = fmaf(wy, x, dacc[i][4]); dacc[i][5] = fmaf(wy, y, dacc[i][5]); dacc[i][6] = fmaf(wy, z, dacc[i][6]); dacc[i][7] += wy;
-                dacc[i][8] = fmaf(wz, x, dacc[i][8]); dacc[i][9] = fmaf(wz, y, dacc[i][9]); dacc[i][10] = fmaf(wz, z, dacc[i][10]); dacc[i][11] += wz;
-            }
-        }
+        PHASE_MARK(0);
+        if constexpr (TAB) {
+            STRAPS_WG_BARRIER();
+            PHASE_MARK(1);
+            if (djoints && h == 0 && vbody) {
+                const float* dj = djoints + (b0 + bl) * (STRAPS_SMPL_NJOINTS_OUT * 3) + 72;
+                for (int e = jp0; e < jp1; e += JRT_NB) {
+                    int code[JRT_NB];
+                    float w[JRT_NB], g[JRT_NB][3];
+#pragma unroll
+                    for (int q = 0; q < JRT_NB; ++q) {
+                        const int ee = min(e + q, jp1 - 1);
+                        code[q] = ee < TAB_JRT_MAX ? tab_jc[ee] : m.jrt_code[jr0 + ee];
+                        w[q] = ee < TAB_JRT_MAX ? tab_jw[ee] : m.jrt_w[jr0 + ee];
+                    }
+#pragma unroll
+                    for (int q = 0; q < JRT_NB; ++q) {
+                        const float* gp = dj + (code[q] & 255) * 3;
+                        g[q][0] = gp[0]; g[q][1] = gp[1]; g[q][2] = gp[2];
+                    }
+#pragma unroll
+                    for (int q = 0; q < JRT_NB; ++q)
+                        if (e + q < jp1) {
+                            float* sv = mystage + bl * SS + (code[q] >> 8) * 6;
+                            sv[0] = fmaf(w[q], g[q][0], sv[0]); sv[1] = fmaf(w[q], g[q][1], sv[1]); sv[2] = fmaf(w[q], g[q][2], sv[2]);
+                        }
+                }
+            }
+            STRAPS_WG_BARRIER();
+            PHASE_MARK(2);
+            int hr = h;
+            asm volatile("" : "+v"(hr));
+            if (KW == 4) skin_bwd_rows<4>(As_ + bl * AS, tab_sw + wave * 32 * 4, tab_sj + wave * 32 * 4, mystage + bl * SS, hr, 4, ax, ay, az);
+            else skin_bwd_rows<0>(As_ + bl * AS, tab_sw + wave * 32 * KW, tab_sj + wave * 32 * KW, mystage + bl * SS, hr, KW, ax, ay, az);
+            STRAPS_WG_BARRIER();
+            PHASE_MARK(3);
+#pragma unroll
+            for (int i = 0; i < 3; ++i) {
+                const int e1 = op1[i];
+                for (int e = op0[i]; e < e1; e += OWN_NB) {
+                    float w[OWN_NB], s6[OWN_NB][6];
+                    int code[OWN_NB];
+#pragma unroll
+                    for (int q = 0; q < OWN_NB; ++q) {
+                        const int ee = min(e + q, e1 - 1);
+                        code[q] = ee < TAB_SKIN ? tab_dc[ee] : m.dj_code[dj0 + ee];
+                        w[q] = ee < TAB_SKIN ? tab_dw[ee] : m.dj_w[dj0 + ee];
+                    }
+#pragma unroll
+                    for (int q = 0; q < OWN_NB; ++q) {
+                        const float* sv = stage + ((code[q] >> 5) * BT + bl) * SS + (code[q] & 31) * 6;
+#pragma unroll
+                        for (int c = 0; c < 6; ++c) s6[q][c] = sv[c];
+                    }
+#pragma unroll
+                    for (int q = 0; q < OWN_NB; ++q)
+                        if (e + q < e1) {
+                            const float wx = w[q] * s6[q][0], wy = w[q] * s6[q][1], wz = w[q] * s6[q][2];
+                            const float x = s6[q][3], y = s6[q][4], z = s6[q][5];
+                            dacc[i][0] = fmaf(wx, x, dacc[i][0]); dacc[i][1] = fmaf(wx, y, dacc[i][1]); dacc[i][2] = fmaf(wx, z, dacc[i][2]); dacc[i][3] += wx;
+                            dacc[i][4] = fmaf(wy, x, dacc[i][4]); dacc[i][5] = fmaf(wy, y, dacc[i][5]); dacc[i][6] = fmaf(wy, z, dacc[i][6]); dacc[i][7] += wy;
+                            dacc[i][8] = fmaf(wz, x, dacc[i][8]); dacc[i][9] = fmaf(wz, y, dacc[i][9]); dacc[i][10] = fmaf(wz, z, dacc[i][10]); dacc[i][11] += wz;
+                        }
+                }
+            }
+        } else {
+            {
+                const int ncol = min(96, (NV - tile * 32) * 3);
+                for (int i = lane; i < BT * 96; i += 64) {
+                    const int b = i / 96, c = i - b * 96;
+                    float v = 0.f;
+                    if (dverts && b < nb && c < ncol) v = dverts[(b0 + b) * (long long)(NV * 3) + tile * 96 + c];
+                    mystage[b * SS + (c / 3) * 6 + (c % 3)] = v;
+                }
+            }
+            STRAPS_WG_BARRIER();
+            PHASE_MARK(1);
+            if (djoints && h == 0 && vbody) {
+                const float* dj = djoints + (b0 + bl) * (STRAPS_SMPL_NJOINTS_OUT * 3) + 72;
+                const int e0 = m.jrt_ptr[tile], e1 = m.jrt_ptr[tile + 1];
+                for (int e = e0; e < e1; ++e) {
+                    const int code = m.jrt_code[e];
+                    const float w = m.jrt_w[e];
+                    float* sv = mystage + bl * SS + (code >> 8) * 6;
+                    const float* g = dj + (code & 255) * 3;
+                    sv[0] = fmaf(w, g[0], sv[0]); sv[1] = fmaf(w, g[1], sv[1]); sv[2] = fmaf(w, g[2], sv[2]);
+                }
+            }
+            STRAPS_WG_BARRIER();
+            PHASE_MARK(2);
+            {
+                const float* Ab = As_ + bl * AS;
+    #pragma unroll
+                for (int r = 0; r < 16; ++r) {
+                    const int vrow = (r & 3) + 8 * (r >> 2) + 4 * h;
+                    const int v = tile * 32 + vrow;
+                    float* sv = mystage + bl * SS + vrow * 6;
+                    const float gx = sv[0], gy = sv[1], gz = sv[2];
+                    sv[3] = ax[r]; sv[4] = ay[r]; sv[5] = az[r];
+                    float t00 = 0.f, t01 = 0.f, t02 = 0.f, t10 = 0.f, t11 = 0.f, t12 = 0.f, t20 = 0.f, t21 = 0.f, t22 = 0.f;
+                    for (int k = 0; k < KW; ++k) {
+                        const float w = m.skin_w[v * KW + k];
+                        const int jo = m.skin_j[v * KW + k] * 12;
+                        const f32x4 a0 = *reinterpret_cast<const f32x4*>(Ab + jo);
+                        const f32x4 a1 = *reinterpret_cast<const f32x4*>(Ab + jo + 4);
+                        const f32x4 a2 = *reinterpret_cast<const f32x4*>(Ab + jo + 8);
+                        t00 = fmaf(w, a0[0], t00); t01 = fmaf(w, a0[1], t01); t02 = fmaf(w, a0[2], t02);
+                        t10 = fmaf(w, a1[0], t10); t11 = fmaf(w, a1[1], t11); t12 = fmaf(w, a1[2], t12);
+                        t20 = fmaf(w, a2[0], t20); t21 = fmaf(w, a2[1], t21); t22 = fmaf(w, a2[2], t22);
+                    }
+                    ax[r] = fmaf(t20, gz, fmaf(t00, gx, __fmul_rn(t10, gy)));
+                    ay[r] = fmaf(t21, gz, fmaf(t01, gx, __fmul_rn(t11, gy)));
+                    az[r] = fmaf(t22, gz, fmaf(t02, gx, __fmul_rn(t12, gy)));
+                }
+            }
+            STRAPS_WG_BARRIER();
+            PHASE_MARK(3);
+    #pragma unroll
+            for (int i = 0; i < 3; ++i) {
+                const int j = wave + 4 * (2 * i + h);
+                const int e0 = m.dj_ptr[rd * 24 + j], e1 = m.dj_ptr[rd * 24 + j + 1];
+                for (int e = e0; e < e1; ++e) {
+                    const int code = m.dj_code[e];
+                    const float w = m.dj_w[e];
+                    const float* sv = stage + ((code >> 5) * BT + bl) * SS + (code & 31) * 6;
+                    const float wx = w * sv[0], wy = w * sv[1], wz = w * sv[2];
+                    const float x = sv[3], y = sv[4], z = sv[5];
+                    dacc[i][0] = fmaf(wx, x, dacc[i][0]); dacc[i][1] = fmaf(wx, y, dacc[i][1]); dacc[i][2] = fmaf(wx, z, dacc[i][2]); dacc[i][3] += wx;
+                    dacc[i][4] = fmaf(wy, x, dacc[i][4]); dacc[i][5] = fmaf(wy, y, dacc[i][5]); dacc[i][6] = fmaf(wy, z, dacc[i][6]); dacc[i][7] += wy;
+                    dacc[i][8] = fmaf(wz, x, dacc[i][8]); dacc[i][9] = fmaf(wz, y, dacc[i][9]); dacc[i][10] = fmaf(wz, z, dacc[i][10]); dacc[i][11] += wz;
+                }
+            }
+        }
+        PHASE_MARK(4);
         {
             const f32x4* pt = blend_t + ((long long)tile * 3 * 7 * 4) * 64 + lane;
 #pragma unroll
@@ -158,10 +372,14 @@
                 }
             }
         }
-        __syncthreads();
+        STRAPS_WG_BARRIER();
+        PHASE_MARK(5);
+#ifdef STRAPS_TOOLS
+        ph[7] += 1;
+#endif
     }
     {
-        __syncthreads();
+        STRAPS_WG_BARRIER();
         float* red = smem;
         if (wave >= 2) {
 #pragma unroll
@@ -169,21 +387,21 @@
 #pragma unroll
                 for (int q = 0; q < 16; ++q) red[(wave - 2) * 7168 + (f * 16 + q) * 64 + lane] = accF[f][q];
         }
-        __syncthreads();
+        STRAPS_WG_BARRIER();
         if (wave < 2) {
 #pragma unroll
             for (int f = 0; f < 7; ++f)
 #pragma unroll
                 for (int q = 0; q < 16; ++q) accF[f][q] += red[wave * 7168 + (f * 16 + q) * 64 + lane];
         }
-        __syncthreads();
+        STRAPS_WG_BARRIER();
         if (wave == 1) {
 #pragma unroll
             for (int f = 0; f < 7; ++f)
 #pragma unroll
                 for (int q = 0; q < 16; ++q) red[(f * 16 + q) * 64 + lane] = accF[f][q];
         }
-        __syncthreads();
+        STRAPS_WG_BARRIER();
         if (wave == 0) {
 #pragma unroll
             for (int f = 0; f < 7; ++f)
@@ -207,9 +425,45 @@
             for (int e = 0; e < 12; ++e) o[j * 12 + e] = dacc[i][e];
         }
     }
+#ifdef STRAPS_TOOLS
+    __builtin_amdgcn_s_waitcnt(0);
+    PHASE_MARK(6);
+    if (ph_on && lane == 0)
+        for (int k = 0; k < 8; ++k) g_smpl_bwd_phase[k] = ph[k];
+#endif
 }
 
 __device__ __forceinline__ float lane_get(float value, int src) { return __shfl(value, src, 64); }
+template <int N>
+__device__ __forceinline__ void add_dA_rows(const float* __restrict__ p, long long stride, float (&gA)[12]) {
+    float v[N][12];
+#pragma unroll
+    for (int q = 0; q < N; ++q)
+#pragma unroll
+        for (int e = 0; e < 12; ++e) v[q][e] = p[q * stride + e];
+#pragma unroll
+    for (int q = 0; q < N; ++q)
+#pragma unroll
+        for (int e = 0; e < 12; ++e) gA[e] += v[q][e];
+}
+template <int N>
+__device__ __forceinline__ void add_dF_rows(const float* __restrict__ p, long long stride, int j, float (&gR)[9], float& gbeta_direct) {
+    float v[N][9], d[N];
+#pragma unroll
+    for (int q = 0; q < N; ++q) {
+#pragma unroll
+        for (int e = 0; e < 9; ++e) v[q][e] = (j >= 1) ? p[q * stride + 11 + (j - 1) * 9 + e] : 0.f;
+        d[q] = (j < 10) ? p[q * stride + 1 + j] : 0.f;
+    }
+#pragma unroll
+    for (int q = 0; q < N; ++q) {
+        if (j >= 1) {
+#pragma unroll
+            for (int e = 0; e < 9; ++e) gR[e] += v[q][e];
+        }
+        if (j < 10) gbeta_direct += d[q];
+    }
+}
 template <bool AA>
 __global__ __launch_bounds__(256) STRAPS_NO_PACKED_FP32 void smpl_pose_bwd_kernel(straps_smpl_model_t m, const float* __restrict__ betas,
                                                             const float* __restrict__ rotmats, const float* __restrict__ dFp,
@@ -274,12 +528,12 @@
     float gA[12];
 #pragma unroll
     for (int e = 0; e < 12; ++e) gA[e] = 0.f;
-    if (vb && vj)
-        for (int c = 0; c < chunks; ++c) {
-            const float* p = dAp + (((long long)c * B + body) * 24 + j) * 12;
-#pragma unroll
-            for (int e = 0; e < 12; ++e) gA[e] += p[e];
-        }
+    if (vb && vj) {
+        int c = 0;
+        for (; c + 9 <= chunks; c += 9) add_dA_rows<9>(dAp + (((long long)c * B + body) * 24 + j) * 12, B * 288, gA);
+        for (; c + 4 <= chunks; c += 4) add_dA_rows<4>(dAp + (((long long)c * B + body) * 24 + j) * 12, B * 288, gA);
+        for (; c < chunks; ++c) add_dA_rows<1>(dAp + (((long long)c * B + body) * 24 + j) * 12, B * 288, gA);
+    }
     float gGR[9], gGt[3], gJ[3];
 #pragma unroll
     for (int r = 0; r < 3; ++r) {
@@ -343,14 +597,10 @@
     }
     float gbeta_direct = 0.f;
     if (vb && vj) {
-        for (int c = 0; c < chunks; ++c) {
-            const float* p = dFp + ((long long)c * B + body) * KP;
-            if (j >= 1) {
-#pragma unroll
-                for (int e = 0; e < 9; ++e) gR[e] += p[11 + (j - 1) * 9 + e];
-            }
-            if (j < 10) gbeta_direct += p[1 + j];
-        }
+        int c = 0;
+        for (; c + 9 <= chunks; c += 9) add_dF_rows<9>(dFp + ((long long)c * B + body) * KP, B * KP, j, gR, gbeta_direct);
+        for (; c + 4 <= chunks; c += 4) add_dF_rows<4>(dFp + ((long long)c * B + body) * KP, B * KP, j, gR, gbeta_direct);
+        for (; c < chunks; ++c) add_dF_rows<1>(dFp + ((long long)c * B + body) * KP, B * KP, j, gR, gbeta_direct);
         if (!AA || drot) {
 #pragma unroll
             for (int e = 0; e < 9; ++e) drot[(body * 24 + j) * 9 + e] = gR[e];
@@ -368,7 +618,7 @@
         float s = vj ? (m.j_shapedirs[(jj * 3 + 0) * 10 + l] * gJ[0] + m.j_shapedirs[(jj * 3 + 1) * 10 + l] * gJ[1] +
                         m.j_shapedirs[(jj * 3 + 2) * 10 + l] * gJ[2]) : 0.f;
 #pragma unroll
-        for (int o = 16; o > 0; o >>= 1) s += __shfl_xor(s, o, 64);
+        for (int o = 16; o > 0; o >>= 1) s += STRAPS_LANE_XOR(s, o, lane);
         const float direct = lane_get(gbeta_direct, base + l);
         if (vb && j == l) dbetas[body * 10 + l] = s + direct;
     }
@@ -405,11 +655,15 @@
     float* dAp = dFp + (long long)nch * batch * KP;
     int rc = straps_smpl_launch_pose(model, betas, rotmats, F, Amat, nullptr, batch, st);
     if (rc != STRAPS_OK) return rc;
-    const size_t lds = (size_t)(BT * AS + 4 * BT * SS) * sizeof(float);
-    STRAPS_RAISE_LDS((smpl_verts_bwd_kernel), lds, "smpl_verts_bwd_kernel");
+    const bool tab = STRAPS_TOOL_ENV_INT("STRAPS_SMPL_BWD_LDS_TABLES", 1) && model->skin_k >= 1 && model->skin_k <= TAB_KW_MAX &&
+                     model->bwd_jrt_round_max >= 1 && model->bwd_jrt_round_max <= TAB_JRT_MAX;
+    const size_t lds = (size_t)(BT * AS + 4 * BT * SS + (tab ? TAB_WORDS : 0)) * sizeof(float);
+    if (tab) STRAPS_RAISE_LDS((smpl_verts_bwd_kernel<true>), lds, "smpl_verts_bwd_kernel");
+    else STRAPS_RAISE_LDS((smpl_verts_bwd_kernel<false>), lds, "smpl_verts_bwd_kernel");
     const long long btiles = (batch + BT - 1) / BT;
     if (btiles > 65535) { straps_set_error("straps_smpl_bwd: batch %lld exceeds one launch; split it", batch); return STRAPS_EUNSUPPORTED; }
-    hipLaunchKernelGGL(smpl_verts_bwd_kernel, dim3(nch, (unsigned)btiles), dim3(256), lds, st, *model, F, Amat, dverts, djoints, dFp, dAp, batch, rpc);
+    if (tab) hipLaunchKernelGGL(smpl_verts_bwd_kernel<true>, dim3(nch, (unsigned)btiles), dim3(256), lds, st, *model, F, Amat, dverts, djoints, dFp, dAp, batch, rpc);
+    else hipLaunchKernelGGL(smpl_verts_bwd_kernel<false>, dim3(nch, (unsigned)btiles), dim3(256), lds, st, *model, F, Amat, dverts, djoints, dFp, dAp, batch, rpc);
     STRAPS_CHECK_LAUNCH("smpl_verts_bwd_kernel");
     hipLaunchKernelGGL(smpl_pose_bwd_kernel<AA>, dim3((unsigned)((batch * 32 + 255) / 256)), dim3(256), 0, st, *model, betas, rotmats, dFp, dAp,
                        djoints, dbetas, drotmats, batch, nch, aa, daa);
@@ -438,3 +692,10 @@
     return smpl_bwd_launch<true>(model, betas, rotmats, full_pose_aa, dverts, djoints, dbetas, drotmats, dfull_pose_aa, workspace, batch, chunks,
                                  stream);
 }
+
+#ifdef STRAPS_TOOLS
+extern "C" int straps_tools_smpl_bwd_phases(long long* out8) {
+    if (hipDeviceSynchronize() != hipSuccess) return STRAPS_EHIP;
+    return hipMemcpyFromSymbol(out8, HIP_SYMBOL(g_smpl_bwd_phase), 8 * sizeof(long long)) == hipSuccess ? STRAPS_OK : STRAPS_EHIP;
+}
+#endif
diff --git a/straps-3dhumanshapepose_amd/csrc/train.hip b/straps-3dhumanshapepose_amd/csrc/train.hip
--- a/straps-3dhumanshapepose_amd/csrc/train.hip
+++ b/straps-3dhumanshapepose_amd/csrc/train.hip
@@ -107,11 +107,10 @@
 
 constexpr int NVB = 1024;
 
-__global__ __launch_bounds__(256) void loss_verts_partial_kernel(const float* __restrict__ p, const float* __restrict__ t, long long n,
-                                                                 float* __restrict__ part) {
-    __shared__ float red[4];
+__device__ __forceinline__ void loss_verts_partial_block(const float* __restrict__ p, const float* __restrict__ t, long long n, float* __restrict__ part,
+                                                         float* red) {
     float s = 0.f;
-    for (long long i = (long long)blockIdx.x * 256 + threadIdx.x; i < n; i += (long long)gridDim.x * 256) {
+    for (long long i = (long long)blockIdx.x * 256 + threadIdx.x; i < n; i += (long long)NVB * 256) {
         const float d = p[i] - t[i];
         s = fmaf(d, d, s);
     }
@@ -124,36 +123,67 @@
 
 __device__ __forceinline__ bool joint_visible(float x, float y, float wh) { return !(x > wh || y > wh || x < 0.f || y < 0.f); }
 
-__global__ __launch_bounds__(256) void loss_heads_kernel(const float* __restrict__ joints, const float* __restrict__ est, int ld_est,
-                                                         const float* __restrict__ prot, const float* __restrict__ tj2d,
-                                                         const float* __restrict__ tj3d, const float* __restrict__ tshape,
-                                                         const float* __restrict__ trot, float* __restrict__ body_sums, long long B,
-                                                         float wh) {
-    const long long b = (long long)blockIdx.x * 256 + threadIdx.x;
-    if (b >= B) return;
-    const float* J = joints + b * 270;
-    const float* e = est + b * ld_est;
-    const float s = e[0], tx = e[1], ty = e[2];
+constexpr int LH_J = 0, LH_E = 272, LH_T2 = 288, LH_T3 = 324, LH_TS = 368, LH_PR = 380, LH_TR = 596, LH_N = 812;
+__device__ __forceinline__ void loss_heads_block(const float* __restrict__ joints, const float* __restrict__ est, int ld_est,
+                                                 const float* __restrict__ prot, const float* __restrict__ tj2d, const float* __restrict__ tj3d,
+                                                 const float* __restrict__ tshape, const float* __restrict__ trot, float* __restrict__ body_sums,
+                                                 long long B, float wh, float* sh_all) {
+    const int lane = threadIdx.x & 63, wave = threadIdx.x >> 6;
+    const long long b = ((long long)blockIdx.x - NVB) * 4 + wave;
+    float* sh = sh_all + wave * LH_N;
+    if (b < B) {
+        const float* e = est + b * ld_est;
+        for (int i = lane; i < 270; i += 64) sh[LH_J + i] = joints[b * 270 + i];
+        if (lane < 3) sh[LH_E + lane] = e[lane];
+        else if (lane < 13) sh[LH_E + lane] = e[147 + lane - 3];
+        if (lane < 34) sh[LH_T2 + lane] = tj2d[b * 34 + lane];
+        if (lane < 42) sh[LH_T3 + lane] = tj3d[b * 42 + lane];
+        if (lane < 10) sh[LH_TS + lane] = tshape[b * 10 + lane];
+        for (int i = lane; i < 216; i += 64) { sh[LH_PR + i] = prot[b * 216 + i]; sh[LH_TR + i] = trot[b * 216 + i]; }
+    }
+    __syncthreads();
+    if (b >= B || lane != 0) return;
+    const float* J = sh + LH_J;
+    const float s = sh[LH_E + 0], tx = sh[LH_E + 1], ty = sh[LH_E + 2];
     float sq2 = 0.f, nvis = 0.f, sq3 = 0.f, sqs = 0.f, sqr = 0.f;
     for (int k = 0; k < 17; ++k) {
-        const float lx = tj2d[(b * 17 + k) * 2 + 0], ly = tj2d[(b * 17 + k) * 2 + 1];
+        const float lx = sh[LH_T2 + k * 2 + 0], ly = sh[LH_T2 + k * 2 + 1];
         if (joint_visible(lx, ly, wh)) {
             const float* pj = J + c_coco[k] * 3;
-            const float u = s * (pj[0] + tx), v = s * (pj[1] + ty);
-            const float du = u - ((2.0f * lx) / wh - 1.0f), dv = v - ((2.0f * ly) / wh - 1.0f);
-            sq2 += du * du + dv * dv;
+            const float du = fmaf(s, pj[0] + tx, -((2.0f * lx) / wh - 1.0f)), dv = fmaf(s, pj[1] + ty, -((2.0f * ly) / wh - 1.0f));
+            sq2 = __fadd_rn(sq2, fmaf(du, du, __fmul_rn(dv, dv)));
             nvis += 1.f;
         }
     }
-    for (int k = 0; k < 14; ++k) {
+    {
+        const float* p0 = J + c_h36m14[0] * 3;
+        const float d0 = p0[0] - sh[LH_T3 + 0], d1 = p0[1] - sh[LH_T3 + 1], d2 = p0[2] - sh[LH_T3 + 2];
+        sq3 = fmaf(d2, d2, fmaf(d0, d0, __fmul_rn(d1, d1)));
+    }
+    for (int k = 1; k < 14; ++k) {
         const float* pj = J + c_h36m14[k] * 3;
-        const float* tj = tj3d + (b * 14 + k) * 3;
-        for (int c = 0; c < 3; ++c) { const float d = pj[c] - tj[c]; sq3 += d * d; }
-    }
-    for (int l = 0; l < 10; ++l) { const float d = e[147 + l] - tshape[b * 10 + l]; sqs += d * d; }
-    for (int q = 0; q < 216; ++q) { const float d = prot[b * 216 + q] - trot[b * 216 + q]; sqr += d * d; }
+        const float* tj = sh + LH_T3 + k * 3;
+        for (int c = 0; c < 3; ++c) { const float d = pj[c] - tj[c]; sq3 = fmaf(d, d, sq3); }
+    }
+    {
+        const float d0 = sh[LH_E + 3] - sh[LH_TS], d1 = sh[LH_E + 4] - sh[LH_TS + 1];
+        sqs = fmaf(d0, d0, __fmul_rn(d1, d1));
+    }
+    for (int l = 2; l < 10; ++l) { const float d = sh[LH_E + 3 + l] - sh[LH_TS + l]; sqs = fmaf(d, d, sqs); }
+#pragma unroll 8
+    for (int q = 0; q < 216; ++q) { const float d = sh[LH_PR + q] - sh[LH_TR + q]; sqr = fmaf(d, d, sqr); }
     float* o = body_sums + b * 8;
     o[0] = sq2; o[1] = nvis; o[2] = sq3; o[3] = sqs; o[4] = sqr;
+}
+
+__global__ __launch_bounds__(256) void loss_sums_kernel(const float* __restrict__ pverts, const float* __restrict__ tverts, long long nv,
+                                                        float* __restrict__ vpart, const float* __restrict__ joints, const float* __restrict__ est,
+                                                        int ld_est, const float* __restrict__ prot, const float* __restrict__ tj2d,
+                                                        const float* __restrict__ tj3d, const float* __restrict__ tshape,
+                                                        const float* __restrict__ trot, float* __restrict__ body_sums, long long B, float wh) {
+    __shared__ float sh[4 * LH_N];
+    if (blockIdx.x < NVB) loss_verts_partial_block(pverts, tverts, nv, vpart, sh);
+    else loss_heads_block(joints, est, ld_est, prot, tj2d, tj3d, tshape, trot, body_sums, B, wh, sh);
 }
 
 __global__ __launch_bounds__(256) void loss_finalize_kernel(const float* __restrict__ vpart, const float* __restrict__ body_sums,
@@ -169,10 +199,16 @@
     }
     for (int q = 0; q < 6; ++q) red[threadIdx.x][q] = a[q];
     __syncthreads();
+    __shared__ double tot[6];
+    if (threadIdx.x < 6) {
+        double tq = 0;
+#pragma unroll 16
+        for (int i = 0; i < 256; ++i) tq += red[i][threadIdx.x];
+        tot[threadIdx.x] = tq;
+    }
+    __syncthreads();
     if (threadIdx.x == 0) {
-        double t[6] = {0, 0, 0, 0, 0, 0};
-        for (int i = 0; i < 256; ++i)
-            for (int q = 0; q < 6; ++q) t[q] += red[i][q];
+        const double t[6] = {tot[0], tot[1], tot[2], tot[3], tot[4], tot[5]};
         const double nvis = t[2];
         const double n2 = j2d_count ? (double)j2d_count[0] * (double)count_scale : nvis;
         const double cnt[5] = {(double)B * 20670.0, n2 * 2.0, (double)B * 42.0, (double)B * 10.0, (double)B * 216.0};
@@ -193,20 +229,22 @@
     }
 }
 
-__global__ __launch_bounds__(256) void loss_grad_verts_kernel(const float* __restrict__ p, const float* __restrict__ t,
-                                                              const float* __restrict__ coef, float* __restrict__ g, long long n) {
-    const float c = coef[0];
-    for (long long i = (long long)blockIdx.x * 256 + threadIdx.x; i < n; i += (long long)gridDim.x * 256) g[i] = c * (p[i] - t[i]);
-}
-
-__global__ __launch_bounds__(64) STRAPS_NO_PACKED_FP32 void loss_grad_heads_kernel(const float* __restrict__ joints, const float* __restrict__ est, int ld_est,
+__global__ __launch_bounds__(256) STRAPS_NO_PACKED_FP32 void loss_grad_kernel(const float* __restrict__ pverts, const float* __restrict__ tverts,
+                                                             float* __restrict__ dverts, long long nv, int gv,
+                                                             const float* __restrict__ joints, const float* __restrict__ est, int ld_est,
                                                              const float* __restrict__ prot, const float* __restrict__ tj2d,
                                                              const float* __restrict__ tj3d, const float* __restrict__ tshape,
                                                              const float* __restrict__ trot, const float* __restrict__ coef,
                                                              float* __restrict__ djoints, float* __restrict__ dest,
                                                              float* __restrict__ drot, long long B, float wh) {
-    const long long b = blockIdx.x;
-    const int lane = threadIdx.x;
+    if ((int)blockIdx.x < gv) {
+        const float c = coef[0];
+        for (long long i = (long long)blockIdx.x * 256 + threadIdx.x; i < nv; i += (long long)gv * 256) dverts[i] = c * (pverts[i] - tverts[i]);
+        return;
+    }
+    const long long b = ((long long)blockIdx.x - gv) * 4 + (threadIdx.x >> 6);
+    const int lane = threadIdx.x & 63;
+    if (b >= B) return;
     const float* J = joints + b * 270;
     const float* e = est + b * ld_est;
     float* dJ = djoints + b * 270;
@@ -215,8 +253,10 @@
     for (int i = lane; i < 270; i += 64) dJ[i] = 0.f;
     for (int i = lane; i < ld_est; i += 64) dE[i] = (i >= 147 && i < 157) ? cs * (e[i] - tshape[b * 10 + i - 147]) : 0.f;
     for (int i = lane; i < 216; i += 64) drot[b * 216 + i] = cr * (prot[b * 216 + i] - trot[b * 216 + i]);
+    __builtin_amdgcn_fence(__ATOMIC_RELEASE, "wavefront");
     __builtin_amdgcn_s_waitcnt(0);
-    __syncthreads();
+    __builtin_amdgcn_wave_barrier();
+    __builtin_amdgcn_fence(__ATOMIC_ACQUIRE, "wavefront");
     const float s = e[0], tx = e[1], ty = e[2];
     float gs = 0.f, gtx = 0.f, gty = 0.f;
     if (lane < 17) {
@@ -239,9 +279,9 @@
     }
 #pragma unroll
     for (int o = 16; o > 0; o >>= 1) {
-        gs += __shfl_xor(gs, o, 64);
-        gtx += __shfl_xor(gtx, o, 64);
-        gty += __shfl_xor(gty, o, 64);
+        gs += STRAPS_LANE_XOR(gs, o, lane);
+        gtx += STRAPS_LANE_XOR(gtx, o, lane);
+        gty += STRAPS_LANE_XOR(gty, o, lane);
     }
     if (lane == 0) { dE[0] = gs; dE[1] = gtx; dE[2] = gty; }
 }
@@ -352,19 +392,16 @@
     float* coef = body + batch * 8;
     float* dlv = dlogvar ? dlogvar : coef + 8;
     const long long nv = batch * 20670LL;
-    hipLaunchKernelGGL(loss_verts_partial_kernel, dim3(NVB), dim3(256), 0, st, pred_verts, tgt_verts, nv, vpart);
-    STRAPS_CHECK_LAUNCH("loss_verts_partial_kernel");
-    hipLaunchKernelGGL(loss_heads_kernel, dim3((unsigned)((batch + 255) / 256)), dim3(256), 0, st, pred_joints, est, ld_est, pred_rot,
-                       tgt_joints2d, tgt_joints3d, tgt_shape, tgt_rot, body, batch, (float)img_wh);
-    STRAPS_CHECK_LAUNCH("loss_heads_kernel");
+    hipLaunchKernelGGL(loss_sums_kernel, dim3((unsigned)(NVB + (batch + 3) / 4)), dim3(256), 0, st, pred_verts, tgt_verts, nv, vpart, pred_joints, est, ld_est,
+                       pred_rot, tgt_joints2d, tgt_joints3d, tgt_shape, tgt_rot, body, batch, (float)img_wh);
+    STRAPS_CHECK_LAUNCH("loss_sums_kernel");
     hipLaunchKernelGGL(loss_finalize_kernel, dim3(1), dim3(256), 0, st, vpart, body, log_vars, loss_out, dlv, coef, batch, j2d_count_global, count_scale);
     STRAPS_CHECK_LAUNCH("loss_finalize_kernel");
     if (want_grad) {
-        hipLaunchKernelGGL(loss_grad_verts_kernel, dim3(capped_grid(nv)), dim3(256), 0, st, pred_verts, tgt_verts, coef, dverts, nv);
-        STRAPS_CHECK_LAUNCH("loss_grad_verts_kernel");
-        hipLaunchKernelGGL(loss_grad_heads_kernel, dim3((unsigned)batch), dim3(64), 0, st, pred_joints, est, ld_est, pred_rot, tgt_joints2d,
-                           tgt_joints3d, tgt_shape, tgt_rot, coef, djoints, dest, drot, batch, (float)img_wh);
-        STRAPS_CHECK_LAUNCH("loss_grad_heads_kernel");
+        const int gv = (int)capped_grid(nv);
+        hipLaunchKernelGGL(loss_grad_kernel, dim3((unsigned)(gv + (batch + 3) / 4)), dim3(256), 0, st, pred_verts, tgt_verts, dverts, nv, gv, pred_joints, est,
+                           ld_est, pred_rot, tgt_joints2d, tgt_joints3d, tgt_shape, tgt_rot, coef, djoints, dest, drot, batch, (float)img_wh);
+        STRAPS_CHECK_LAUNCH("loss_grad_kernel");
     }
     return STRAPS_OK;
 }
diff --git a/straps-3dhumanshapepose_amd/hipabi.py b/straps-3dhumanshapepose_amd/hipabi.py
--- a/straps-3dhumanshapepose_amd/hipabi.py
+++ b/straps-3dhumanshapepose_amd/hipabi.py
@@ -85,7 +85,7 @@
     _fields_ = [('blend_frag', C.c_void_p), ('j_template', C.c_void_p), ('j_shapedirs', C.c_void_p),
                 ('parents', C.c_void_p), ('depth', C.c_void_p), ('max_depth', C.c_int32), ('skin_k', C.c_int32),
                 ('skin_w', C.c_void_p), ('skin_j', C.c_void_p), ('vj_ptr', C.c_void_p), ('n_tiles', C.c_int32),
-                ('reserved0', C.c_int32), ('pick_ids', C.c_void_p), ('blend_frag_t', C.c_void_p), ('children', C.c_void_p),
+                ('bwd_jrt_round_max', C.c_int32), ('pick_ids', C.c_void_p), ('blend_frag_t', C.c_void_p), ('children', C.c_void_p),
                 ('jrt_ptr', C.c_void_p), ('jrt_code', C.c_void_p), ('jrt_w', C.c_void_p), ('dj_ptr', C.c_void_p), ('dj_code', C.c_void_p),
                 ('dj_w', C.c_void_p), ('blend_frag_h', C.c_void_p), ('blend_h_unscale', C.c_float), ('reserved1', C.c_int32), ('skin_frag_p', C.c_void_p)]
 
diff --git a/straps-3dhumanshapepose_amd/smpl.py b/straps-3dhumanshapepose_amd/smpl.py
--- a/straps-3dhumanshapepose_amd/smpl.py
+++ b/straps-3dhumanshapepose_amd/smpl.py
@@ -126,6 +126,7 @@
         'dj_ptr': dj_ptr, 'dj_code': dj_code, 'dj_w': dw.astype(np.float32),
         'blend_frag_t': frag_t.reshape(-1), 'children': children,
         'jrt_ptr': jrt_ptr, 'jrt_code': (((vs % 32) << 8) | src).astype(np.int32), 'jrt_w': ws,
+        'jrt_round_max': int(np.diff(jrt_ptr[::4]).max()),
         'blend_frag': frag.reshape(-1),
         'blend_frag_h': frag_h.reshape(-1), 'blend_h_unscale': float(2.0 ** -(sd_exp + 6)),         'skin_frag_p': skin_frag_p.reshape(-1),
         'j_template': (Jr @ vt).astype(np.float32),
@@ -150,6 +151,7 @@
         packed = pack_smpl_model(model)
         self.max_depth, self.skin_k, self.n_tiles = packed.pop('max_depth'), packed.pop('skin_k'), packed.pop('n_tiles')
         self.blend_h_unscale = packed.pop('blend_h_unscale')
+        self.jrt_round_max = packed.pop('jrt_round_max')
         precision = kwargs.pop('precision', 'fp32')
         if precision not in PRECISIONS:
             raise ValueError("SMPL: precision must be one of %s" % (sorted(PRECISIONS),))
@@ -181,6 +183,7 @@
                 setattr(s, f, getattr(self, '_k_' + f).data_ptr())
             s.max_depth, s.skin_k, s.n_tiles = self.max_depth, self.skin_k, self.n_tiles
             s.blend_h_unscale = self.blend_h_unscale
+            s.bwd_jrt_round_max = self.jrt_round_max
             self._struct, self._struct_key = s, key
         return self._struct
 
diff --git a/straps-3dhumanshapepose_amd/train_step.py b/straps-3dhumanshapepose_amd/train_step.py
--- a/straps-3dhumanshapepose_amd/train_step.py
+++ b/straps-3dhumanshapepose_amd/train_step.py
@@ -364,7 +364,7 @@
         hipabi.check(L.straps_masked_copy(C.c_void_p(est.data_ptr() + 4 * 147), EST_LD, None, 0, hipabi.ptr(pred_shape), 10, B, 10, 0, st), 'pred_shape')
         verts, joints = smpl.forward_arrays(pred_shape, R)
         eye = self._eye
-        reposed, _ = smpl.forward_arrays(pred_shape, eye, want_joints=False)
+        reposed = smpl.forward_arrays(pred_shape, eye, want_joints=False)[0] if self.metrics is not None else None
         if self._lv_index is not None:
             lv = torch.empty(5, device=d)
             hipabi.check(L.straps_gather_f32(hipabi.ptr(self._lv_params_flat), hipabi.ptr(self._lv_index), hipabi.ptr(lv), 5, st), 'log-var gather')
```

New measurement: 8318, median of 6. 1.01x the previous value.
